# prtk1729/Paligemma-MultiModal-System

Hardware: AMD Instinct MI355X
Metric: image→text tokens/sec + prefill ms, PaliGemma-3B-224 at 1/2/4/8 MI355X (higher is better)
Workload: dtype bf16; 1 GPU; PaliGemma-3B-pt-224 image->text, batch 1, prefill L=264, 128 greedy tokens (BASELINE.json configs[1]); global_batch=1, seq_len=392, parallelism=dp1, decode=hipgraph, prefill=eager

## Files before the change

include/pghip.h:

```cpp
#ifndef PGHIP_H
#define PGHIP_H
#include <stdint.h>
#include <hip/hip_runtime_api.h>

#ifdef __cplusplus
extern "C" {
#endif

int pg_abi_version(void);
int pg_source_hash(char* out, int n);

enum {
  PG_EPI_BF16 = 0,
  PG_EPI_BF16_GELU = 1,
  PG_EPI_BF16_GELU_MUL = 2,
  PG_EPI_F32 = 3,
  PG_EPI_F32_POS = 4,
  PG_EPI_BF16_VT = 5,
  PG_EPI_QKV_ROPE = 6,
  PG_EPI_F32_FIN = 7,
  PG_EPI_F32_ADD = 8,
  PG_EPI_FX_ADD = 9,
  PG_EPI_F32_RES = 10
};

typedef struct PgFusedArgs {
  int pro_mode;
  const float* resid_in;
  float* resid_out;
  const float* partials;
  int nsplit;
  const float* norm_w;
  float eps;
  const float* part_o;
  const float* part_ml;
  int asplit, head_dim, dtw, q_per_kv, kv_heads;
  const float* cos_t;
  const float* sin_t;
  const int* pos;
  int rows_per_batch;
  const int* slot_dev;
  int slot_base;
  void* kc;
  void* vtc;
  int smax;
  int q_heads;
  int* fin_cnt;
  float* fin_resid;
  float* ss_out;
  const float* ss_in;
  int ss_ld, ss_n;
  void* fin_x;
  int akeys;
  const float* a_scale;
  const float* w_scale;
  int slab_rows;
  void* kd;
  void* vd;
  unsigned* amax_out;
  const unsigned* amax_in;
  int amax_ld;
  unsigned* amax_zero;
  int amax_zero_n;
  int64_t* fx;
  uint8_t* mx_out;
  const uint8_t* mx_in;
  int* status;
} PgFusedArgs;

#define PG_W_FRAG 0x100
#define PG_FP8 0x200
#define PG_TILE_M1 0x400
#define PG_TILE_N64 0x800

int pg_gemm(const void* A, int lda, const void* W, int ldw, const float* bias, void* C, int ldc,
            int M, int N, int K, int epi, int ksplit, const float* aux, int aux_rows, void* aux_out,
            int aux_ld, int aux_n, hipStream_t stream);

int pg_gemm_finalize(const float* part, int nsplit, void* C, int ldc, int M, int N, int epi, void* aux_out,
                     int aux_ld, int aux_n, const PgFusedArgs* fused, hipStream_t stream);

int pg_gemm_fused(const void* A, int lda, const void* W, int ldw, const float* bias, void* C, int ldc,
                  int M, int N, int K, int epi, int ksplit, const PgFusedArgs* fused, hipStream_t stream);

int pg_norm_residual(float* resid, const float* partials, int nsplit, int M_part, const float* w,
                     const float* b, void* out, int ldo, float* out_f32, const int* row_map, int M_out,
                     int H, int mode, float eps, int write_resid, hipStream_t stream);

int pg_attention(const void* q, long q_rs, void* o, long o_rs, const void* k, long k_bs, long k_hs,
                 long k_rs, const void* vt, long vt_bs, long vt_hs, long vt_ds, const float* mask,
                 long mask_bs, long mask_rs, int B, int Lq, int Lkv, const int* lkv_dev, int Hq, int Hkv,
                 int D, float scale, int split_keys, int nsplit, float* part_o, float* part_ml,
                 int kcap, const void* kd, const void* vd, hipStream_t stream);
int pg_attn_combine(const float* part_o, const float* part_ml, int B, int Hq, int Hkv, int D, int nsplit,
                    void* o, long o_rs, hipStream_t stream);

int pg_attn_probs(const void* q, long q_rs, const void* k, long k_bs, long k_hs, long k_rs, const float* mask,
                  long mask_bs, long mask_rs, int B, int Lq, int Lkv, int Hq, int Hkv, int D, float scale,
                  int probs, float* out, hipStream_t stream);

#define PG_ATTN_PIPE 0x100
int pg_attn_decode(const void* q, long q_rs, void* o, long o_rs, const void* kd, const void* vd, int B, int Lkv,
                   const int* lkv_dev, int Hq, int Hkv, int D, float scale, int kcap, int nsplit, int nw, int nb,
                   float* part_o, float* part_ml, int* counters, void* q8, float* q8_scale, long q8_ld,
                   hipStream_t stream);

int pg_rope_kv_write(void* qkv, int ldq, const int* pos, int T, int L, int Hq, int Hkv, int D,
                     const float* cosT, const float* sinT, void* kc, void* vtc, int Smax, int slot_base,
                     const int* slot_dev, hipStream_t stream);

int pg_patch_im2col(const float* px, int B, int C, int H, int W, int p, void* out, int ldk, hipStream_t stream);

int pg_image_rank(const int64_t* ids, int n, long image_id, int* rank, hipStream_t stream);

int pg_embed_merge(const int64_t* ids, const int* rank, int n, const void* embed, int V, const float* feat,
                   int n_feat, int H, long image_id, long pad_id, float img_scale, float normalizer,
                   float* out, hipStream_t stream);

int pg_argmax(const float* logits, long ld, int B, int V, void* workspace, int64_t* out_ids,
              int64_t* hist, int hist_rows, int* step, int* pos, int* kv_len, hipStream_t stream);
int pg_argmax_embed(const float* logits, long ld, int B, int V, void* workspace, int64_t* out_ids,
                    int64_t* hist, int hist_rows, int* step, int* pos, int* kv_len, const void* embed, int V_embed,
                    const float* feat, int n_feat, int H, long image_id, long pad_id, float img_scale,
                    float normalizer, float* res, hipStream_t stream);

int pg_argmax_pairs(const float* logits, long ld, int B, int V, int vocab_offset, void* workspace,
                    float* pairs, hipStream_t stream);
int pg_argmax_merge(const float* pairs, int world, int B, int64_t* out_ids, int64_t* hist, int hist_rows,
                    int* step, int* pos, int* kv_len, hipStream_t stream);

int pg_topp_sample(const float* logits, long ld, int B, int V, float temperature, float top_p,
                   const float* uniforms, int64_t* out_ids, int64_t* hist, int hist_rows, int* step, int* pos,
                   int* kv_len, float* probs_out, hipStream_t stream);

int pg_image_preprocess(const uint8_t* src, int H, int W, int S, const int* hb, const int* hk, int hks,
                        const int* vb, const int* vk, int vks, int y0, int rows, const float* lut, uint8_t* tmp,
                        float* out, hipStream_t stream);
int pg_image_preprocess_modes(const uint8_t* src, int H, int W, int C, int alpha, int S, const int* hb,
                              const int* hk, int hks, const int* vb, const int* vk, int vks, int y0, int rows,
                              const float* lut, uint8_t* tmp, float* out, hipStream_t stream);
int pg_image_palette(const uint8_t* src, int H, int W, int S, const int* xtab, const int* ytab,
                     const float* pal_lut, float* out, hipStream_t stream);

int pg_synth_fill(void* out, long n, unsigned int seedmix, float a, float mean, int out_kind,
                  hipStream_t stream);

int pg_quant_fp8(const void* x, int ldx, int M, int K, void* q, int ldq, float* scale, hipStream_t stream);
int pg_norm_residual_fp8(float* resid, const float* partials, int nsplit, int M_part, const float* w,
                         const float* b, void* q, int ldq, float* scale, const int* row_map, int M_out,
                         int H, int mode, float eps, int write_resid, hipStream_t stream);
int pg_norm_residual_mx(float* resid, const float* partials, int nsplit, int M_part, const float* w, void* q,
                        int ldq, void* qs, float* ss, int ss_ld, int M, int H, int write_resid, hipStream_t stream);

int pg_xgmi_buffer_bytes(int world, long cap, long* bytes);
int pg_xgmi_alloc(long bytes, void** out);
int pg_xgmi_free(void* p);
int pg_xgmi_ipc_handle(void* p, void* handle64);
int pg_xgmi_ipc_open(const void* handle64, void** out);
int pg_xgmi_ipc_close(void* p);
int pg_allreduce_xgmi(float* data, long n, int rank, int world, void* const* peers, long cap,
                      unsigned* epochs, int* err, hipStream_t stream);
int pg_allreduce_xgmi_slabs(float* data, long n, int nslab, long slab_stride, int rank, int world,
                            void* const* peers, long cap, unsigned* epochs, int* err, hipStream_t stream);
int pg_allgather_xgmi(const float* in, long n, float* out, int rank, int world, void* const* peers, long cap,
                      unsigned* epochs, int* err, hipStream_t stream);
int pg_xgmi_rs_buffer_bytes(int world, long rs_cap, long* bytes);
int pg_allreduce_xgmi_rs(float* data, long n, int nslab, long slab_stride, int rank, int world, void* const* peers,
                         long rs_cap, int nwg, unsigned* epochs, int* err, hipStream_t stream);

#ifdef __cplusplus
}
#endif
#endif
```

paligemma-multimodal-system_amd/csrc/common.h:

```cpp
#pragma once
#include <hip/hip_runtime.h>
#include <stdint.h>

typedef uint16_t bf16_t;
typedef __attribute__((ext_vector_type(8))) __bf16 bf16x8;
typedef __attribute__((ext_vector_type(4))) float f32x4;
typedef __attribute__((ext_vector_type(2))) float f32x2;
typedef __attribute__((ext_vector_type(4))) uint32_t u32x4;
typedef __attribute__((ext_vector_type(2))) uint32_t u32x2;

#define LDS_AS __attribute__((address_space(3)))

__device__ __forceinline__ float bf2f(bf16_t v) { return __uint_as_float(((uint32_t)v) << 16); }

__device__ __forceinline__ bf16_t f2bf(float f) {
  __bf16 b = (__bf16)f;
  return __builtin_bit_cast(bf16_t, b);
}
typedef __bf16 pg_bf16x2_t __attribute__((ext_vector_type(2)));
typedef float pg_f32x2_t __attribute__((ext_vector_type(2)));
__device__ __forceinline__ uint32_t pack_bf2(float lo, float hi) {
  return __builtin_bit_cast(uint32_t, __builtin_convertvector(pg_f32x2_t{lo, hi}, pg_bf16x2_t));
}

__device__ __forceinline__ float bf_lo(uint32_t v) { return __uint_as_float(v << 16); }
__device__ __forceinline__ float bf_hi(uint32_t v) { return __uint_as_float(v & 0xffff0000u); }
__device__ __forceinline__ uint32_t pack_fp8x4(float a, float b, float c, float d) {
  int w = __builtin_amdgcn_cvt_pk_fp8_f32(fminf(fmaxf(a, -448.f), 448.f), fminf(fmaxf(b, -448.f), 448.f), 0, false);
  w = __builtin_amdgcn_cvt_pk_fp8_f32(fminf(fmaxf(c, -448.f), 448.f), fminf(fmaxf(d, -448.f), 448.f), w, true);
  return (uint32_t)w;
}

__device__ __forceinline__ float max_xor16(float v) {
  const auto r = __builtin_amdgcn_permlane16_swap(__float_as_uint(v), __float_as_uint(v), false, false);
  return fmaxf(__uint_as_float(r[0]), __uint_as_float(r[1]));
}
__device__ __forceinline__ float max_xor32(float v) {
  const auto r = __builtin_amdgcn_permlane32_swap(__float_as_uint(v), __float_as_uint(v), false, false);
  return fmaxf(__uint_as_float(r[0]), __uint_as_float(r[1]));
}
__device__ __forceinline__ float sum_xor16(float v) {
  const auto r = __builtin_amdgcn_permlane16_swap(__float_as_uint(v), __float_as_uint(v), false, false);
  return __uint_as_float(r[0]) + __uint_as_float(r[1]);
}
__device__ __forceinline__ float sum_xor32(float v) {
  const auto r = __builtin_amdgcn_permlane32_swap(__float_as_uint(v), __float_as_uint(v), false, false);
  return __uint_as_float(r[0]) + __uint_as_float(r[1]);
}

__device__ __forceinline__ float xchg_xor32(float v) {
  const auto r = __builtin_amdgcn_permlane32_swap(__float_as_uint(v), __float_as_uint(v), false, false);
  return __uint_as_float((threadIdx.x & 32) ? r[0] : r[1]);
}

__device__ __forceinline__ float gelu_tanh(float x) {
  const float u = 0.7978845608028654f * (x + 0.044715f * x * x * x);
  return x * __builtin_amdgcn_rcpf(1.0f + __builtin_amdgcn_exp2f(-2.8853900817779268f * u));
}

__device__ __forceinline__ f32x4 mfma16(const bf16x8& a, const bf16x8& b, const f32x4& c) {
  return __builtin_amdgcn_mfma_f32_16x16x32_bf16(a, b, c, 0, 0, 0);
}

typedef __attribute__((ext_vector_type(8))) int i32x8;
typedef __attribute__((ext_vector_type(4))) int i32x4;

__device__ __forceinline__ f32x4 mfma8(const bf16x8& a0, const bf16x8& a1, const bf16x8& b0, const bf16x8& b1,
                                       const f32x4& c) {
  const i32x4 x0 = __builtin_bit_cast(i32x4, a0), x1 = __builtin_bit_cast(i32x4, a1);
  const i32x4 y0 = __builtin_bit_cast(i32x4, b0), y1 = __builtin_bit_cast(i32x4, b1);
  const i32x8 a = __builtin_shufflevector(x0, x1, 0, 1, 2, 3, 4, 5, 6, 7);
  const i32x8 b = __builtin_shufflevector(y0, y1, 0, 1, 2, 3, 4, 5, 6, 7);
  return __builtin_amdgcn_mfma_scale_f32_16x16x128_f8f6f4(a, b, c, 0, 0, 0, 127, 0, 127);
}
__device__ __forceinline__ f32x4 mfma8s(const bf16x8& a0, const bf16x8& a1, const bf16x8& b0, const bf16x8& b1,
                                        const f32x4& c, int sb) {
  const i32x4 x0 = __builtin_bit_cast(i32x4, a0), x1 = __builtin_bit_cast(i32x4, a1);
  const i32x4 y0 = __builtin_bit_cast(i32x4, b0), y1 = __builtin_bit_cast(i32x4, b1);
  const i32x8 a = __builtin_shufflevector(x0, x1, 0, 1, 2, 3, 4, 5, 6, 7);
  const i32x8 b = __builtin_shufflevector(y0, y1, 0, 1, 2, 3, 4, 5, 6, 7);
  return __builtin_amdgcn_mfma_scale_f32_16x16x128_f8f6f4(a, b, c, 0, 0, 0, 127, 0, sb);
}
template <int N>
__device__ __forceinline__ void mfma_fence(f32x4 (&a)[N]) {
#ifdef PG_NO_MFMA_FENCE
  return;
#endif
  __builtin_amdgcn_sched_barrier(0);
  asm volatile("s_nop 7\n\ts_nop 7");
  __builtin_amdgcn_sched_barrier(0);
#pragma unroll
  for (int i = 0; i < N; ++i) asm volatile("" : "+v"(a[i]));
  __builtin_amdgcn_sched_barrier(0);
}
__device__ __forceinline__ int mx_exp(float amax) {
  if (!(amax > 0.f)) return 0;
  int k;
  const float f = frexpf(amax, &k);
  const int e = k - 9 + (f * 512.f > 448.f ? 1 : 0);
  return min(max(e, -127), 127);
}
__device__ __forceinline__ f32x4 mfma8(const i32x8& a, const i32x8& b, const f32x4& c) {
  return __builtin_amdgcn_mfma_scale_f32_16x16x128_f8f6f4(a, b, c, 0, 0, 0, 127, 0, 127);
}
template <int SEL>
__device__ __forceinline__ f32x4 mfma8s_sel(const bf16x8& a0, const bf16x8& a1, const bf16x8& b0, const bf16x8& b1,
                                            const f32x4& c, int sb) {
  const i32x4 x0 = __builtin_bit_cast(i32x4, a0), x1 = __builtin_bit_cast(i32x4, a1);
  const i32x4 y0 = __builtin_bit_cast(i32x4, b0), y1 = __builtin_bit_cast(i32x4, b1);
  const i32x8 a = __builtin_shufflevector(x0, x1, 0, 1, 2, 3, 4, 5, 6, 7);
  const i32x8 b = __builtin_shufflevector(y0, y1, 0, 1, 2, 3, 4, 5, 6, 7);
  return __builtin_amdgcn_mfma_scale_f32_16x16x128_f8f6f4(a, b, c, 0, 0, 0, 127, SEL, sb);
}
__device__ __forceinline__ i32x8 cat8(const bf16x8& lo, const bf16x8& hi) {
  return __builtin_shufflevector(__builtin_bit_cast(i32x4, lo), __builtin_bit_cast(i32x4, hi), 0, 1, 2, 3, 4, 5, 6, 7);
}

__device__ __forceinline__ float wave_sum(float v) {
#pragma unroll
  for (int o = 32; o > 0; o >>= 1) v += __shfl_xor(v, o, 64);
  return v;
}
__device__ __forceinline__ float wave_max(float v) {
#pragma unroll
  for (int o = 32; o > 0; o >>= 1) v = fmaxf(v, __shfl_xor(v, o, 64));
  return v;
}

__device__ __forceinline__ float block_sum(float v, float* red ) {
  const int lane = threadIdx.x & 63, w = threadIdx.x >> 6, nw = blockDim.x >> 6;
  v = wave_sum(v);
  __syncthreads();
  if (lane == 0) red[w] = v;
  __syncthreads();
  float s = 0.f;
  for (int i = 0; i < nw; ++i) s += red[i];
  return s;
}

static __device__ int pg_zero_word = 0;

#define PG_VMC(k) case k: asm volatile("s_waitcnt vmcnt(" #k ")" ::: "memory"); break;
__device__ __forceinline__ void wait_vm_n(int n) {
  switch (n) {
    PG_VMC(1) PG_VMC(2) PG_VMC(3) PG_VMC(4) PG_VMC(5) PG_VMC(6) PG_VMC(7) PG_VMC(8) PG_VMC(9) PG_VMC(10)
    PG_VMC(11) PG_VMC(12) PG_VMC(13) PG_VMC(14) PG_VMC(15) PG_VMC(16) PG_VMC(17) PG_VMC(18) PG_VMC(19) PG_VMC(20)
    PG_VMC(21) PG_VMC(22) PG_VMC(23) PG_VMC(24) PG_VMC(25) PG_VMC(26) PG_VMC(27) PG_VMC(28) PG_VMC(29) PG_VMC(30)
    PG_VMC(31) PG_VMC(32) PG_VMC(33) PG_VMC(34) PG_VMC(35) PG_VMC(36) PG_VMC(37) PG_VMC(38) PG_VMC(39) PG_VMC(40)
    default: asm volatile("s_waitcnt vmcnt(0)" ::: "memory"); break;
  }
}
#undef PG_VMC

#define PG_LAUNCH_CHECK() do { hipError_t _e = hipGetLastError(); if (_e != hipSuccess) return (int)_e; } while (0)
#define PG_REQUIRE(cond) do { if (!(cond)) return (int)hipErrorInvalidValue; } while (0)
```

paligemma-multimodal-system_amd/csrc/gemm.hip:

```cpp
#include "gemm_common.h"

static int gemm_impl(const void* A, int lda, const void* W, int ldw, const float* bias, void* C, int ldc,
                     int M, int N, int K, int epi_flags, int ksplit, const float* aux, int aux_rows, void* aux_out,
                     int aux_ld, int aux_n, const PgFusedArgs* fa, hipStream_t stream) {
  const bool frag = (epi_flags & PG_W_FRAG) != 0;
  const bool fp8 = (epi_flags & PG_FP8) != 0;
  const bool m1 = (epi_flags & PG_TILE_M1) != 0;
  const bool n64 = (epi_flags & PG_TILE_N64) != 0;
  const int epi = epi_flags & 0xFF;
  PG_REQUIRE((epi_flags & ~(0xFF | PG_W_FRAG | PG_FP8 | PG_TILE_M1 | PG_TILE_N64)) == 0 && epi <= PG_EPI_F32_RES);
  if (m1) PG_REQUIRE(!fp8 && !n64 && M >= 256 && M <= 288 && (fa == nullptr || fa->pro_mode == 0));
  if (n64) PG_REQUIRE(M > 16);
  PG_REQUIRE(M > 0 && N > 0 && K > 0 && ksplit >= 1 && W != nullptr && C != nullptr);
  PG_REQUIRE(K % 32 == 0 && ldw >= K && (N % 4) == 0);
  if (frag && !fp8) PG_REQUIRE(N % 16 == 0 && K % 64 == 0 && ldw == K &&
                       (epi == PG_EPI_BF16 || epi == PG_EPI_BF16_GELU_MUL || epi == PG_EPI_F32 ||
                        epi == PG_EPI_QKV_ROPE || epi == PG_EPI_F32_FIN || epi == PG_EPI_F32_ADD ||
                        epi == PG_EPI_FX_ADD || epi == PG_EPI_F32_RES));
  PgFusedArgs f{};
  if (fa) f = *fa;
  EpiArgs e{bias, C, ldc, M, N, aux, aux_rows, (bf16_t*)aux_out, aux_ld, aux_n, f};
  PG_REQUIRE(f.pro_mode >= 0 && f.pro_mode <= 5);
  if (f.pro_mode == 5)
    PG_REQUIRE(fp8 && frag && epi == PG_EPI_F32 && M <= 32 && f.amax_in && f.amax_ld >= 1 && A != nullptr &&
               lda >= K && lda % 8 == 0 && ((uintptr_t)A & 15) == 0 && K % 128 == 0 && (K / 128) % ksplit == 0 &&
               (K / 128 / ksplit == 8 || K / 128 / ksplit == 16));
  if (f.amax_out) PG_REQUIRE(fp8 && frag && epi == PG_EPI_BF16_GELU_MUL && M <= 32 && f.amax_ld >= 1 &&
                             ((K >> 7) + ksplit - 1) / ksplit * 128 <= 4096 && PG_GEMV8_WIDE);
  if (f.amax_zero) PG_REQUIRE(frag && f.amax_zero_n >= 0 &&
                              (fp8 ? f.amax_zero_n <= 4096
                                   : (M <= 16 && f.amax_zero_n <= 16384 && f.amax_zero_n % 4 == 0 &&
                                      ((uintptr_t)f.amax_zero & 15) == 0)));
  if (f.pro_mode == 0 || f.pro_mode == 4) PG_REQUIRE(A != nullptr && lda >= K);
  if (f.pro_mode == 4) PG_REQUIRE(ksplit == 1 && f.ss_in && f.ss_n > 0 && f.ss_ld >= f.ss_n &&
                                  ((M <= 2 && f.ss_n <= 256 && (M == 1 || f.ss_n <= 128)) ||
                                   (M > 4 && M <= 16 && f.ss_n <= 64)));
  if (f.pro_mode != 0 && f.pro_mode != 5) PG_REQUIRE(M <= 16);
  if (f.pro_mode == 1) PG_REQUIRE(ksplit == 1 && (f.resid_in || f.fx) && f.norm_w && (f.nsplit == 0 || f.partials) &&
                                  K % 4 == 0);
  if (f.pro_mode == 2)
    PG_REQUIRE(f.part_o && f.part_ml && f.head_dim > 0 && (K / ksplit) % f.head_dim == 0 && f.asplit > 0 &&
               f.q_per_kv > 0 && f.kv_heads > 0);
  if (epi == PG_EPI_QKV_ROPE) PG_REQUIRE(f.head_dim % 16 == 0 && f.cos_t && f.sin_t && f.pos && f.kc && f.vtc &&
                                         f.rows_per_batch > 0 && f.smax > 0 && ksplit == 1 &&
                                         N == (f.q_heads + 2 * f.kv_heads) * f.head_dim);
  if (f.pro_mode == 3) PG_REQUIRE(ksplit == 1 && f.resid_in && f.norm_w && f.ss_in && f.ss_n > 0 &&
                                  f.ss_ld >= f.ss_n && K % 4 == 0);
  if (epi == PG_EPI_F32_FIN) PG_REQUIRE(M <= 16 && ksplit <= 8 && (f.fin_x == nullptr || f.norm_w != nullptr) && f.fin_cnt && f.fin_resid && f.ss_out && f.ss_ld >= (N + 15) / 16 &&
                                        ldc == N);
  if (epi == PG_EPI_F32_ADD) PG_REQUIRE((M <= 16 || (fp8 && frag && M <= 32)) && (f.pro_mode == 0 || f.pro_mode == 2) &&
                                        ldc >= N);
  if (epi == PG_EPI_F32_RES) PG_REQUIRE(M > 16 && ksplit == 1 && f.pro_mode == 0 && ldc >= N && ldc % 4 == 0 &&
                                        ((uintptr_t)C & 15) == 0 && !f.mx_out);
  if (epi == PG_EPI_FX_ADD) PG_REQUIRE(M <= 16 && !fp8 && (f.pro_mode == 0 || f.pro_mode == 2) && ldc >= N &&
                                       ((uintptr_t)C & 15) == 0 && ldc % 2 == 0);
  if (f.mx_in && frag) PG_REQUIRE(fp8 && epi != PG_EPI_F32_ADD && M <= 32 && f.pro_mode == 0 && K % 128 == 0 &&
                                   A != nullptr && ((uintptr_t)f.mx_in & 15) == 0 &&
                                   (!f.ss_in || (f.ss_n > 0 && f.ss_n <= 4 && f.ss_ld >= f.ss_n && K == 1024 * f.ss_n)));
  if (f.mx_in && !frag) PG_REQUIRE(fp8 && (epi == PG_EPI_F32 || epi == PG_EPI_F32_RES) && M > 32 && f.pro_mode == 0 && K % 128 == 0 &&
                                   A != nullptr && ((uintptr_t)f.mx_in & 3) == 0 && !f.ss_in &&
                                   (size_t)M * (size_t)(K / 32) < (1ull << 32) &&
                                   (size_t)M * (size_t)lda < (1ull << 32) && (size_t)N * (size_t)ldw < (1ull << 32));
  if (f.mx_out && frag) PG_REQUIRE(fp8 && epi == PG_EPI_BF16_GELU_MUL && M <= 32 && f.pro_mode == 0 && !f.amax_out &&
                                    ksplit == 1 && (N / 2) % 128 == 0 && PG_GEMV8_WIDE && (K >> 7) * 128 <= 4096 &&
                                    (!f.mx_in || (K >> 7) == 8 || (K >> 7) == 16));
  if (f.mx_out && !frag) PG_REQUIRE(fp8 && epi == PG_EPI_BF16_GELU_MUL && M > 32 && f.pro_mode == 0 && !f.mx_in &&
                                    ksplit == 1 && N % 128 == 0 && ldc >= N / 2);
  if (f.fx) PG_REQUIRE(((uintptr_t)f.fx & 15) == 0 && (f.pro_mode == 1) != (epi == PG_EPI_F32_FIN) && !fp8 &&
                       M <= 16);
  if (ksplit > 1) PG_REQUIRE(epi == PG_EPI_F32 || epi == PG_EPI_F32_FIN || epi == PG_EPI_F32_ADD || epi == PG_EPI_FX_ADD);
  if (epi == PG_EPI_BF16_GELU_MUL) PG_REQUIRE(N % 32 == 0);
  if (epi == PG_EPI_F32_POS) PG_REQUIRE(aux != nullptr && aux_rows > 0 && bias != nullptr);
  if (epi == PG_EPI_BF16_VT) PG_REQUIRE(aux_out != nullptr && aux_n % 4 == 0);
  if (M <= 16) PG_REQUIRE(K % 64 == 0);
  else PG_REQUIRE(K % TBK == 0 && (f.pro_mode == 0 || f.pro_mode == 5) && epi != PG_EPI_F32_FIN);
  const bf16_t* a = (const bf16_t*)A;
  const bf16_t* w = (const bf16_t*)W;
  if (fp8 && frag) {
    PG_REQUIRE(M <= 32 && (f.pro_mode == 0 || f.pro_mode == 5) && (f.a_scale || f.pro_mode == 5 || f.mx_in) && f.w_scale &&
               K % 128 == 0 && N % 16 == 0 && ldw == K && lda >= K && (lda % 16 == 0 || f.pro_mode == 5) &&
               ((uintptr_t)A & 15) == 0 && ((uintptr_t)W & 15) == 0 && epi != PG_EPI_F32_FIN);
    const int rc = pg_dispatch_gemv8(epi, (const uint8_t*)A, lda, (const uint8_t*)W, K, ksplit, e, stream);
    if (rc) return rc;
    PG_LAUNCH_CHECK();
    return 0;
  }
  if (fp8) {
    PG_REQUIRE(!frag && M > 16 && f.pro_mode == 0 && (f.a_scale || f.mx_in) && f.w_scale && K % 128 == 0 && lda % 16 == 0 &&
               ldw % 16 == 0 && ((uintptr_t)A & 15) == 0 && ((uintptr_t)W & 15) == 0);
    const int rc = pg_dispatch_tile(epi, false, true, a, lda / 2, w, ldw / 2, K / 2, ksplit, e, stream, false, n64);
    if (rc) return rc;
    PG_LAUNCH_CHECK();
    return 0;
  }
  const int rc = M <= 16 ? pg_dispatch_gemv(epi, frag, a, lda, w, ldw, K, ksplit, e, stream)
                         : pg_dispatch_tile(epi, frag, false, a, lda, w, ldw, K, ksplit, e, stream, m1, n64);
  if (rc) return rc;
  PG_LAUNCH_CHECK();
  return 0;
}

extern "C" int pg_gemm(const void* A, int lda, const void* W, int ldw, const float* bias, void* C, int ldc,
                       int M, int N, int K, int epi, int ksplit, const float* aux, int aux_rows, void* aux_out,
                       int aux_ld, int aux_n, hipStream_t stream) {
  return gemm_impl(A, lda, W, ldw, bias, C, ldc, M, N, K, epi, ksplit, aux, aux_rows, aux_out, aux_ld, aux_n,
                   nullptr, stream);
}

extern "C" int pg_gemm_fused(const void* A, int lda, const void* W, int ldw, const float* bias, void* C, int ldc,
                             int M, int N, int K, int epi, int ksplit, const PgFusedArgs* fused, hipStream_t stream) {
  return gemm_impl(A, lda, W, ldw, bias, C, ldc, M, N, K, epi, ksplit, nullptr, 0, nullptr, 0, 0, fused, stream);
}
```

paligemma-multimodal-system_amd/csrc/gemm_common.h:

```cpp
#pragma once
#include <cstdlib>
#include <type_traits>

#include "attn_common.h"

#ifndef PG_G256_STAGGER
#define PG_G256_STAGGER 1
#endif
#ifndef PG_G256_F8_BUF
#define PG_G256_F8_BUF 1
#endif
#ifndef PG_G256_PREFETCH
#define PG_G256_PREFETCH 1
#endif

enum {
  PG_EPI_BF16 = 0,
  PG_EPI_BF16_GELU = 1,
  PG_EPI_BF16_GELU_MUL = 2,
  PG_EPI_F32 = 3,
  PG_EPI_F32_POS = 4,
  PG_EPI_BF16_VT = 5,
  PG_EPI_QKV_ROPE = 6,
  PG_EPI_F32_FIN = 7,
  PG_EPI_F32_ADD = 8,
  PG_EPI_FX_ADD = 9,
  PG_EPI_F32_RES = 10,
};

#define PG_FX_SCALE 0x1p32f
#define PG_FX_INV 0x1p-32f
__device__ __forceinline__ long long fx_from_f32(float v) {
  const float t = truncf(v);
  const int hi = (int)t;
  const float r = rintf((v - t) * PG_FX_SCALE);
  const float rh = truncf(r * 0x1p-16f);
  const float rl = fmaf(rh, -65536.f, r);
  return (long long)((unsigned long long)(long long)hi << 32) + ((long long)(int)rh << 16) + (long long)(int)rl;
}
__device__ __forceinline__ long long fx_from_f32_checked(float v, int* status) {
  if (__builtin_expect(!(fabsf(v) < 0x1p31f), 0)) {
    if (status) atomicOr(status, 1);
    return v > 0.f ? (1LL << 62) : (v < 0.f ? -(1LL << 62) : 0LL);
  }
  return fx_from_f32(v);
}
__device__ __forceinline__ float fx_to_f32(long long q) {
  return fmaf((float)(unsigned)(unsigned long long)q, PG_FX_INV, (float)(int)(q >> 32));
}
typedef long long i64x2 __attribute__((ext_vector_type(2)));
__device__ __forceinline__ f32x4 fx_load4(const long long* p) {
  const i64x2 a = *(const i64x2*)p, b = *(const i64x2*)(p + 2);
  return f32x4{fx_to_f32(a[0]), fx_to_f32(a[1]), fx_to_f32(b[0]), fx_to_f32(b[1])};
}

struct PgFusedArgs {
  int pro_mode;
  const float* resid_in;
  float* resid_out;
  const float* partials;
  int nsplit;
  const float* norm_w;
  float eps;
  const float* part_o;
  const float* part_ml;
  int asplit, head_dim, dtw, q_per_kv, kv_heads;
  const float* cos_t;
  const float* sin_t;
  const int* pos;
  int rows_per_batch;
  const int* slot_dev;
  int slot_base;
  bf16_t* kc;
  bf16_t* vtc;
  int smax;
  int q_heads;
  int* fin_cnt;
  float* fin_resid;
  float* ss_out;
  const float* ss_in;
  int ss_ld, ss_n;
  bf16_t* fin_x;
  int akeys;
  const float* a_scale;
  const float* w_scale;
  int slab_rows;
  bf16_t* kd;
  bf16_t* vd;
  unsigned* amax_out;
  const unsigned* amax_in;
  int amax_ld;
  unsigned* amax_zero;
  int amax_zero_n;
  long long* fx;
  uint8_t* mx_out;
  const uint8_t* mx_in;
  int* status;
};

__device__ __forceinline__ f32x4 load4_guard(const float* __restrict__ p, int n0, int N) {
  if (n0 + 3 < N) return *(const f32x4*)(p + n0);
  f32x4 v = {0.f, 0.f, 0.f, 0.f};
#pragma unroll
  for (int j = 0; j < 4; ++j) if (n0 + j < N) v[j] = p[n0 + j];
  return v;
}

#define PG_W_FRAG 0x100
#define PG_TILE_M1 0x400
#define PG_TILE_N64 0x800
#define PG_FP8 0x200

#ifndef PG_GEMV8_WIDE
#define PG_GEMV8_WIDE 1
#endif

#define TBN 128
#define TBK 64

struct EpiArgs {
  const float* bias;
  void* C;
  int ldc;
  int M, N;
  const float* aux;
  int aux_rows;
  bf16_t* aux_out;
  int aux_ld;
  int aux_n;
  PgFusedArgs f;
};

__device__ __forceinline__ void scale_acc(const EpiArgs& e, int m, int n0, f32x4& v) {
  if (m >= e.M || n0 >= e.N) return;
  v *= (e.f.mx_in ? 1.0f : e.f.a_scale[m]) * load4_guard(e.f.w_scale, n0, e.N);
}

struct Fp8RowLoads {
  float v[4];
};
__device__ __forceinline__ Fp8RowLoads fp8_row_load(const EpiArgs& e, int m) {
  Fp8RowLoads r;
  m = min(m, e.M - 1);
  if (!e.f.mx_in) {
    r.v[0] = e.f.a_scale[m];
  } else if (e.f.ss_in) {
    const float* p = e.f.ss_in + (size_t)m * e.f.ss_ld;
#pragma unroll
    for (int i = 0; i < 4; ++i) r.v[i] = p[min(i, e.f.ss_n - 1)];
  }
  return r;
}
__device__ __forceinline__ float fp8_row_finish(const EpiArgs& e, const Fp8RowLoads& r) {
  if (!e.f.mx_in) return r.v[0];
  if (!e.f.ss_in) return 1.0f;
  float s = 0.f;
#pragma unroll
  for (int i = 0; i < 4; ++i) s += i < e.f.ss_n ? r.v[i] : 0.f;
  return rsqrtf(s / (1024.0f * (float)e.f.ss_n) + e.f.eps);
}
__device__ __forceinline__ float fp8_row_factor(const EpiArgs& e, int m) { return fp8_row_finish(e, fp8_row_load(e, m)); }
__device__ __forceinline__ void scale_acc_rf(const EpiArgs& e, int m, int n0, f32x4& v, float rf) {
  if (m >= e.M || n0 >= e.N) return;
  v *= rf * load4_guard(e.f.w_scale, n0, e.N);
}

__device__ __forceinline__ int rope_freq_index(const PgFusedArgs& f, int n0, bool* roped) {
  const int D = f.head_dim, within = n0 % D, jj0 = within & 15;
  *roped = n0 / D < f.q_heads + f.kv_heads;
  return 8 * (within >> 4) + (jj0 & 7);
}
__device__ __forceinline__ void epi_qkv_rope4_core(const EpiArgs& e, int m, int n0, f32x4 v, f32x4 pr, f32x4 cs,
                                                   f32x4 sn, int slot0) {
  if (m >= e.M || n0 >= e.N) return;
  const PgFusedArgs& f = e.f;
  const int D = f.head_dim, half = D >> 1;
  const int blk = n0 / D, within = n0 % D;
  const int t = within >> 4, jj0 = within & 15;
  const bool second = jj0 >= 8;
  const int ii = 8 * t + (jj0 & 7);
  const int d0 = second ? half + ii : ii;
  const int b = m / f.rows_per_batch, i = m % f.rows_per_batch;
  const int slot = slot0 + i;
  const bool in_cache = slot < f.smax;
  const int Hq = f.q_heads, Hkv = f.kv_heads;
  const int KV = Hkv * D;
  if (blk < Hq + Hkv) {
    f32x4 y;
#pragma unroll
    for (int j = 0; j < 4; ++j) {
      y[j] = second ? v[j] * cs[j] + pr[j] * sn[j] : v[j] * cs[j] - pr[j] * sn[j];
    }
    u32x2 pk;
    pk[0] = pack_bf2(y[0], y[1]);
    pk[1] = pack_bf2(y[2], y[3]);
    if (blk < Hq) {
      *(u32x2*)((bf16_t*)e.C + (size_t)m * e.ldc + blk * D + d0) = pk;
    } else if (in_cache) {
      *(u32x2*)(f.kc + ((size_t)b * f.smax + slot) * KV + (blk - Hq) * D + d0) = pk;
      if (f.kd)
        *(u32x2*)(f.kd + ((size_t)b * Hkv + (blk - Hq)) * f.smax * D + dec_koff(slot, d0, D)) = pk;
    }
  } else {
    const int c0 = (blk - Hq - Hkv) * D + d0;
    if (in_cache) {
#pragma unroll
      for (int j = 0; j < 4; ++j) f.vtc[((size_t)b * KV + c0 + j) * f.smax + slot] = f2bf(v[j]);
      if (f.vd) {
        bf16_t* vd = f.vd + ((size_t)b * Hkv + (blk - Hq - Hkv)) * f.smax * D;
#pragma unroll
        for (int j = 0; j < 4; ++j) vd[dec_voff(slot, d0 + j, D)] = f2bf(v[j]);
      }
    }
  }
}

__device__ __forceinline__ void epi_qkv_rope4_pr(const EpiArgs& e, int m, int n0, f32x4 v, f32x4 pr) {
  if (m >= e.M || n0 >= e.N) return;
  const PgFusedArgs& f = e.f;
  bool roped;
  const int ii = rope_freq_index(f, n0, &roped);
  f32x4 cs = {1.f, 1.f, 1.f, 1.f}, sn = {0.f, 0.f, 0.f, 0.f};
  if (roped) {
    const int p = f.pos[m];
    const float* cp = f.cos_t + (long)p * (f.head_dim >> 1) + ii;
    const float* sp = f.sin_t + (long)p * (f.head_dim >> 1) + ii;
#pragma unroll
    for (int j = 0; j < 4; ++j) {
      cs[j] = cp[j];
      sn[j] = sp[j];
    }
  }
  epi_qkv_rope4_core(e, m, n0, v, pr, cs, sn, f.slot_base + (f.slot_dev ? *f.slot_dev : 0));
}

__device__ __forceinline__ void epi_qkv_rope4(const EpiArgs& e, int m, int n0, f32x4 v) {
  if (e.bias && n0 < e.N) v += load4_guard(e.bias, n0, e.N);
  f32x4 pr;
#pragma unroll
  for (int j = 0; j < 4; ++j) pr[j] = xchg_xor32(v[j]);
  epi_qkv_rope4_pr(e, m, n0, v, pr);
}

__device__ __forceinline__ f32x4 res_load4(const EpiArgs& e, int m, int n0) {
  f32x4 r = {0.f, 0.f, 0.f, 0.f};
  if (m >= e.M || n0 >= e.N) return r;
  const float* C = (const float*)e.C + (size_t)m * e.ldc;
  if (n0 + 3 < e.N) return *(const f32x4*)(C + n0);
#pragma unroll
  for (int j = 0; j < 4; ++j) if (n0 + j < e.N) r[j] = C[n0 + j];
  return r;
}
__device__ __forceinline__ void res_store4(const EpiArgs& e, int m, int n0, f32x4 v, f32x4 r) {
  if (m >= e.M || n0 >= e.N) return;
  if (e.bias) v += load4_guard(e.bias, n0, e.N);
  float* C = (float*)e.C + (size_t)m * e.ldc;
  const f32x4 o = r + v;
  if (n0 + 3 < e.N) {
    *(f32x4*)(C + n0) = o;
  } else {
#pragma unroll
    for (int j = 0; j < 4; ++j) if (n0 + j < e.N) C[n0 + j] = o[j];
  }
}

template <int EPI>
__device__ __forceinline__ void epi_store4(const EpiArgs& e, int m, int n0, f32x4 v, int z) {
  if (m >= e.M || n0 >= e.N) return;
  if (e.bias && (EPI != PG_EPI_F32 || z == 0)) v += load4_guard(e.bias, n0, e.N);
  if constexpr (EPI == PG_EPI_F32) {
    const size_t srows = e.f.slab_rows > 0 ? (size_t)e.f.slab_rows : (size_t)e.M;
    float* C = (float*)e.C + ((size_t)z * srows + m) * e.ldc;
    if (n0 + 3 < e.N) {
      *(f32x4*)(C + n0) = v;
    } else {
#pragma unroll
      for (int j = 0; j < 4; ++j) if (n0 + j < e.N) C[n0 + j] = v[j];
    }
  } else if constexpr (EPI == PG_EPI_F32_RES) {
    float* C = (float*)e.C + (size_t)m * e.ldc;
    if (n0 + 3 < e.N) {
      *(f32x4*)(C + n0) = *(const f32x4*)(C + n0) + v;
    } else {
#pragma unroll
      for (int j = 0; j < 4; ++j) if (n0 + j < e.N) C[n0 + j] = C[n0 + j] + v[j];
    }
  } else if constexpr (EPI == PG_EPI_F32_POS) {
    float* C = (float*)e.C + (size_t)m * e.ldc;
    v += load4_guard(e.aux + (size_t)(m % e.aux_rows) * e.ldc, n0, e.N);
    if (n0 + 3 < e.N) {
      *(f32x4*)(C + n0) = v;
    } else {
#pragma unroll
      for (int j = 0; j < 4; ++j) if (n0 + j < e.N) C[n0 + j] = v[j];
    }
  } else {
    if constexpr (EPI == PG_EPI_BF16_GELU) {
#pragma unroll
      for (int j = 0; j < 4; ++j) v[j] = gelu_tanh(v[j]);
    }
    if constexpr (EPI == PG_EPI_BF16_VT) {
      if (n0 >= e.aux_n) {
#pragma unroll
        for (int j = 0; j < 4; ++j)
          if (n0 + j < e.N) e.aux_out[(size_t)(n0 + j - e.aux_n) * e.aux_ld + m] = f2bf(v[j]);
        return;
      }
    }
    bf16_t* C = (bf16_t*)e.C + (size_t)m * e.ldc;
    if (n0 + 3 < e.N) {
      u32x2 p;
      p[0] = pack_bf2(v[0], v[1]);
      p[1] = pack_bf2(v[2], v[3]);
      *(u32x2*)(C + n0) = p;
    } else {
#pragma unroll
      for (int j = 0; j < 4; ++j) if (n0 + j < e.N) C[n0 + j] = f2bf(v[j]);
    }
  }
}

__device__ __forceinline__ void epi_add4(const EpiArgs& e, int m, int n0, f32x4 v, int z) {
  if (m >= e.M || n0 >= e.N) return;
  if (e.bias && z == 0) v += load4_guard(e.bias, n0, e.N);
  float* dst = (float*)e.C + (size_t)m * e.ldc + n0;
#pragma unroll
  for (int j = 0; j < 4; ++j)
    if (n0 + j < e.N) unsafeAtomicAdd(dst + j, v[j]);
}

__device__ __forceinline__ void epi_gelu_mul4(const EpiArgs& e, int m, int gb, int q, f32x4 g, f32x4 u) {
  if (m >= e.M) return;
  const int oc = (gb >> 1) + q;
  if (oc + 3 >= (e.N >> 1)) return;
  u32x2 p;
  p[0] = pack_bf2(gelu_tanh(g[0]) * u[0], gelu_tanh(g[1]) * u[1]);
  p[1] = pack_bf2(gelu_tanh(g[2]) * u[2], gelu_tanh(g[3]) * u[3]);
  *(u32x2*)((bf16_t*)e.C + (size_t)m * e.ldc + oc) = p;
}

__device__ __forceinline__ float epi_gelu_mul4_amax(const EpiArgs& e, int m, int gb, int q, f32x4 g, f32x4 u) {
  if (m >= e.M) return 0.f;
  const int oc = (gb >> 1) + q;
  if (oc + 3 >= (e.N >> 1)) return 0.f;
  u32x2 p;
  p[0] = pack_bf2(gelu_tanh(g[0]) * u[0], gelu_tanh(g[1]) * u[1]);
  p[1] = pack_bf2(gelu_tanh(g[2]) * u[2], gelu_tanh(g[3]) * u[3]);
  *(u32x2*)((bf16_t*)e.C + (size_t)m * e.ldc + oc) = p;
  return fmaxf(fmaxf(fabsf(bf_lo(p[0])), fabsf(bf_hi(p[0]))), fmaxf(fabsf(bf_lo(p[1])), fabsf(bf_hi(p[1]))));
}

__device__ __forceinline__ void amax_clear(const EpiArgs& e) {
  if (e.f.amax_zero && blockIdx.x == 0 && blockIdx.y == 0)
    for (int i = threadIdx.x; i < e.f.amax_zero_n; i += blockDim.x) e.f.amax_zero[i] = 0u;
}

int pg_dispatch_tile(int epi, bool frag, bool f8, const bf16_t* A, int lda, const bf16_t* W, int ldw, int K, int ksplit,
                     const EpiArgs& e, hipStream_t st, bool m1, bool n64);
int pg_dispatch_gemv(int epi, bool frag, const bf16_t* A, int lda, const bf16_t* W, int ldw, int K, int ksplit,
                     const EpiArgs& e, hipStream_t st);
int pg_dispatch_gemv8(int epi, const uint8_t* X, int ldx, const uint8_t* W, int K, int ksplit, const EpiArgs& e,
                      hipStream_t st);
```

paligemma-multimodal-system_amd/csrc/gemm_gemv.hip:

```cpp
#include "gemm_common.h"

#define XPAD 8

#ifndef PG_GEMV_PREW
#define PG_GEMV_PREW 1
#endif
#ifndef PG_GEMV_NT
#define PG_GEMV_NT 0
#endif
#ifndef PG_GEMV_CONTIG
#define PG_GEMV_CONTIG 0
#endif
#ifndef PG_GEMV_QKV_NT1
#define PG_GEMV_QKV_NT1 1
#endif
#ifndef PG_GEMV_D2
#define PG_GEMV_D2 4
#endif
#ifndef PG_GEMV_LM_NT
#define PG_GEMV_LM_NT 2
#endif
#ifndef PG_GEMV_LM_D
#define PG_GEMV_LM_D 6
#endif
// ... 336 lines not shown
    } else {
      const int off = (c0 + wave + j * 4) * CH + LANE_OFF;
#pragma unroll
      for (int t = 0; t < NT; ++t)
#pragma unroll
        for (int s = 0; s < U; ++s) {
#if PG_GEMV_NT
          wv[t][s] = __builtin_nontemporal_load((const u32x4*)(wrow[t] + off + S_STRIDE * s));
#else
          wv[t][s] = *(const u32x4*)(wrow[t] + off + S_STRIDE * s);
#endif
        }
    }
  };
  auto loadx = [&](int j, u32x4 (&xv)[U]) {
    const int koff = (wave + j * 4) * CH + LANE_OFF;
    if constexpr ((PRO == 0 || PRO == 4) && !PG_GEMV_XLDS) {
#pragma unroll
      for (int s = 0; s < U; ++s)
        xv[s] = *(const u32x4*)(xrow + c0 * CH + koff + S_STRIDE * s);
    } else {
#pragma unroll
      for (int s = 0; s < U; ++s) xv[s] = *(const u32x4*)(xlds + koff + S_STRIDE * s);
    }
  };
  constexpr bool STAGED = (PRO != 0 && PRO != 4) || PG_GEMV_XLDS;
  const bool early = PRO == 1 && (PG_GEMV_PRO_EARLY == 1 || (PG_GEMV_PRO_EARLY == 2 && EPI == PG_EPI_QKV_ROPE)) &&
                     M == 1 && (K >> 2) <= 512 && e.f.nsplit == 0 &&
                     e.f.resid_out == nullptr;
  Pro1Row p1;
  if constexpr (PRO == 1 && PG_GEMV_PRO_EARLY) {
    if (early) pro1_row_load(e.f, K, p1);
    __builtin_amdgcn_sched_barrier(0);
  }
  constexpr bool prew = STAGED && PG_GEMV_PREW;
  if (prew) {
#pragma unroll
    for (int d = 0; d < DEPTH; ++d)
      if (CPW > 0 ? d < CPW : d < mine) loadw(d, wb[d]);
  }
  if constexpr (STAGED) {
    float* scratch = (float*)(dyn_smem + (((size_t)M * (Kr + XPAD) * 2 + 15) & ~(size_t)15));
    if (PRO == 1 && PG_GEMV_PRO_EARLY && early)
      pro1_row_finish(e.f, K, p1, xs, scratch);
    else
      gemv_prologue<PRO>(e, M, K, c0 * CH, nch * CH, xs, scratch, A, lda, gi);
  }
#pragma unroll
  for (int d = 0; d < DEPTH; ++d)
    if (CPW > 0 ? d < CPW : d < mine) {
      if (!prew) loadw(d, wb[d]);
      loadx(d, xb[d]);
    }
  f32x4 fin_r[NT], fin_w[NT];
  i64x2 fin_fa[NT], fin_fb[NT];
  if constexpr (EPI == PG_EPI_F32_FIN) {
#pragma unroll
    for (int t = 0; t < NT; ++t) {
      const int n0 = min((tile0 + t) * 16, e.N - 16) + 4 * g;
      const size_t ro = (size_t)(r < M ? r : M - 1) * e.N + n0;
      fin_r[t] = *(const f32x4*)(e.f.fin_resid + ro);
      const long long* p = e.f.fx ? e.f.fx + ro : (const long long*)e.f.fin_resid;
      fin_fa[t] = *(const i64x2*)p;
      fin_fb[t] = *(const i64x2*)(p + 2);
      fin_w[t] = *(const f32x4*)((e.f.norm_w ? e.f.norm_w : e.f.fin_resid) + n0);
    }
  }
  f32x4 rope_cs[NT], rope_sn[NT];
  if constexpr (EPI == PG_EPI_QKV_ROPE) {
#pragma unroll
    for (int t = 0; t < NT; ++t) {
      bool roped;
      const int ii = rope_freq_index(e.f, min((tile0 + t) * 16, e.N - 16) + 4 * g, &roped);
      const long off = (long)rope_p * (e.f.head_dim >> 1) + ii;
      rope_cs[t] = *(const f32x4*)(e.f.cos_t + off);
      rope_sn[t] = *(const f32x4*)(e.f.sin_t + off);
    }
  }
  if constexpr (CPW > 0) {
    __builtin_amdgcn_sched_barrier(0);
#pragma unroll
    for (int j = 0; j < CPW; ++j) {
      const int d = j % DEPTH;
#pragma unroll
      for (int s = 0; s < U; ++s) {
        const bf16x8 xv = __builtin_bit_cast(bf16x8, xb[d][s]);
#pragma unroll
        for (int t = 0; t < NT; ++t) acc[t] = mfma16(__builtin_bit_cast(bf16x8, wb[d][t][s]), xv, acc[t]);
      }
      if (j + DEPTH < CPW) {
        loadw(j + DEPTH, wb[d]);
        loadx(j + DEPTH, xb[d]);
      }
      __builtin_amdgcn_sched_barrier(0);
    }
  } else {
    for (int base = 0; base < mine; base += DEPTH) {
#pragma unroll
      for (int d = 0; d < DEPTH; ++d) {
        const int j = base + d;
        if (j < mine) {
#pragma unroll
          for (int s = 0; s < U; ++s) {
            const bf16x8 xv = __builtin_bit_cast(bf16x8, xb[d][s]);
#pragma unroll
            for (int t = 0; t < NT; ++t) acc[t] = mfma16(__builtin_bit_cast(bf16x8, wb[d][t][s]), xv, acc[t]);
          }
          if (j + DEPTH < mine) {
            loadw(j + DEPTH, wb[d]);
            loadx(j + DEPTH, xb[d]);
          }
        }
      }
    }
  }

  __shared__ f32x4 red[4][NT][64];
#pragma unroll
  for (int t = 0; t < NT; ++t) red[wave][t][lane] = acc[t];
  __syncthreads();
  if (e.f.amax_zero && gi.bx == 0 && gi.by == 0)
    for (int i = 4 * (int)threadIdx.x; i < e.f.amax_zero_n; i += 1024) *(u32x4*)(e.f.amax_zero + i) = u32x4{0u, 0u, 0u, 0u};
  if (wave != 0) return;
#pragma unroll
  for (int t = 0; t < NT; ++t) acc[t] = red[0][t][lane] + red[1][t][lane] + red[2][t][lane] + red[3][t][lane];
  const int m = r;
  const int q = 4 * g;
  if constexpr (PRO == 3) {
    const float* scratch = (const float*)(dyn_smem + (((size_t)M * (Kr + XPAD) * 2 + 15) & ~(size_t)15));
    const float rs = scratch[64 + (m < M ? m : 0)];
#pragma unroll
    for (int t = 0; t < NT; ++t) acc[t] *= rs;
  }
  if constexpr (PRO == 4) {
    float ss = 0.f;
    if (SS16 && M > 2) {
#pragma unroll
      for (int k = 0; k < SSL; ++k) ss += g + 4 * k < e.f.ss_n ? ssv[k] : 0.f;
    } else {
      const int lpr = M == 1 ? 64 : 32;
#pragma unroll
      for (int k = 0; k < 4; ++k) ss += lane % lpr + k * lpr < e.f.ss_n ? ssv[k] : 0.f;
    }
    if (SS16 && M > 2) {
      ss = sum_xor16(ss);
      ss = sum_xor32(ss);
    } else {
      const int lpr = M == 1 ? 64 : 32;
      for (int o = 1; o < lpr; o <<= 1) ss += __shfl_xor(ss, o, 64);
      ss = __shfl(ss, (m < M ? m : 0) * lpr, 64);
    }
    const float rs = rsqrtf(ss / (float)K + e.f.eps);
#pragma unroll
    for (int t = 0; t < NT; ++t) acc[t] *= rs;
  }
  if constexpr (EPI == PG_EPI_F32_FIN) {
    const PgFusedArgs& f = e.f;
    typedef __attribute__((address_space(1))) unsigned long long gu64;
    constexpr int SE = NT >= 2 ? NT / 2 : 1;
    auto finish = [&](int t, int n0, f32x4 v, float& ssl) {
      *(f32x4*)(f.fin_resid + (size_t)m * e.N + n0) = v;
      ssl += v[0] * v[0] + v[1] * v[1] + v[2] * v[2] + v[3] * v[3];
      if (f.fin_x) {
        const f32x4 w = fin_w[t];
        u32x2 pk;
        pk[0] = pack_bf2(v[0] * (1.0f + w[0]), v[1] * (1.0f + w[1]));
        pk[1] = pack_bf2(v[2] * (1.0f + w[2]), v[3] * (1.0f + w[3]));
        *(u32x2*)(f.fin_x + (size_t)m * e.N + n0) = pk;
      }
    };
    auto fin_base = [&](int t) {
      return f.fx ? f32x4{fx_to_f32(fin_fa[t][0]), fx_to_f32(fin_fa[t][1]), fx_to_f32(fin_fb[t][0]),
                          fx_to_f32(fin_fb[t][1])}
                  : fin_r[t];
    };
    auto fx_clear = [&](int n0) {
      if (f.fx) {
        long long* p = f.fx + (size_t)m * e.N + n0;
        *(i64x2*)p = i64x2{0, 0};
        *(i64x2*)(p + 2) = i64x2{0, 0};
      }
    };
    auto put_ss = [&](float (&ssl)[SE]) {
#pragma unroll
      for (int p = 0; p < SE; ++p) {
        const float v = sum_xor32(sum_xor16(ssl[p]));
        if (g == 0 && m < M) f.ss_out[(size_t)m * f.ss_ld + gi.bx * SE + p] = v;
      }
    };
    if (gi.ny == 1) {
      float ssl[SE];
#pragma unroll
      for (int p = 0; p < SE; ++p) ssl[p] = 0.f;
#pragma unroll
      for (int t = 0; t < NT; ++t) {
        const int n0 = (tile0 + t) * 16 + q;
        if (m < M && n0 < e.N) {
          f32x4 v = acc[t];
          if (e.bias) v += load4_guard(e.bias, n0, e.N);
          finish(t, n0, fin_base(t) + v, ssl[t / 2 < SE ? t / 2 : 0]);
          fx_clear(n0);
        }
      }
      put_ss(ssl);
      return;
    }
#pragma unroll
    for (int t = 0; t < NT; ++t) {
      const int n0 = (tile0 + t) * 16 + q;
      if (m < M && n0 < e.N) {
        f32x4 v = acc[t];
        if (e.bias && z == 0) v += load4_guard(e.bias, n0, e.N);
        gu64* dst = (gu64*)((float*)e.C + ((size_t)z * M + m) * e.ldc + n0);
        __hip_atomic_store(dst, __builtin_bit_cast(unsigned long long, u32x2{__float_as_uint(v[0]),
                           __float_as_uint(v[1])}), __ATOMIC_RELAXED, __HIP_MEMORY_SCOPE_AGENT);
        __hip_atomic_store(dst + 1, __builtin_bit_cast(unsigned long long, u32x2{__float_as_uint(v[2]),
                           __float_as_uint(v[3])}), __ATOMIC_RELAXED, __HIP_MEMORY_SCOPE_AGENT);
      }
    }
    asm volatile("s_waitcnt vmcnt(0)" ::: "memory");
    int old = 0;
    if (lane == 0) old = __hip_atomic_fetch_add(f.fin_cnt + gi.bx, 1, __ATOMIC_RELAXED, __HIP_MEMORY_SCOPE_AGENT);
    old = __shfl(old, 0, 64);
    if (old != gi.ny - 1) return;
    __builtin_amdgcn_fence(__ATOMIC_ACQUIRE, "wavefront");
    float ssl[SE];
#pragma unroll
    for (int p = 0; p < SE; ++p) ssl[p] = 0.f;
#pragma unroll
    for (int t = 0; t < NT; ++t) {
      const int n0 = (tile0 + t) * 16 + q;
      if (m < M && n0 < e.N) {
        f32x4 v = fin_base(t);
        const int Z = gi.ny;
        u32x2 sa[8], sb[8];
#pragma unroll
        for (int zz = 0; zz < 8; ++zz) {
          gu64* src = (gu64*)((float*)e.C + ((size_t)(zz < Z ? zz : Z - 1) * M + m) * e.ldc + n0);
          sa[zz] = __builtin_bit_cast(u32x2, __hip_atomic_load(src, __ATOMIC_RELAXED, __HIP_MEMORY_SCOPE_AGENT));
          sb[zz] = __builtin_bit_cast(u32x2, __hip_atomic_load(src + 1, __ATOMIC_RELAXED, __HIP_MEMORY_SCOPE_AGENT));
        }
#pragma unroll
        for (int zz = 0; zz < 8; ++zz) {
          const f32x4 sv = {__uint_as_float(sa[zz][0]), __uint_as_float(sa[zz][1]), __uint_as_float(sb[zz][0]),
                            __uint_as_float(sb[zz][1])};
          v += zz < Z ? sv : f32x4{0.f, 0.f, 0.f, 0.f};
        }
        finish(t, n0, v, ssl[t / 2 < SE ? t / 2 : 0]);
        fx_clear(n0);
      }
    }
    put_ss(ssl);
    if (lane == 0) __hip_atomic_store(f.fin_cnt + gi.bx, 0, __ATOMIC_RELAXED, __HIP_MEMORY_SCOPE_AGENT);
    return;
  }
  if constexpr (EPI == PG_EPI_F32_ADD) {
    if (m < M) {
#pragma unroll
      for (int t = 0; t < NT; ++t) {
        const int n0 = (tile0 + t) * 16 + q;
        if (n0 < e.N) {
          f32x4 v = acc[t];
          if (e.bias && z == 0) v += load4_guard(e.bias, n0, e.N);
          float* dst = (float*)e.C + (size_t)m * e.ldc + n0;
#pragma unroll
          for (int j = 0; j < 4; ++j) unsafeAtomicAdd(dst + j, v[j]);
        }
      }
    }
    return;
  }
  if constexpr (EPI == PG_EPI_FX_ADD) {
    if (m < M) {
#pragma unroll
      for (int t = 0; t < NT; ++t) {
        const int n0 = (tile0 + t) * 16 + q;
        if (n0 < e.N) {
          f32x4 v = acc[t];
          if (e.bias && z == 0) v += load4_guard(e.bias, n0, e.N);
          if (e.f.resid_in && z == 0) v += load4_guard(e.f.resid_in + (size_t)m * e.N, n0, e.N);
          unsigned long long* dst = (unsigned long long*)e.C + (size_t)m * e.ldc + n0;
#pragma unroll
          for (int j = 0; j < 4; ++j) atomicAdd(dst + j, (unsigned long long)fx_from_f32_checked(v[j], e.f.status));
        }
      }
    }
    return;
  }
  if constexpr (EPI == PG_EPI_BF16_GELU_MUL) {
#pragma unroll
    for (int t = 0; t < NT; t += 2) epi_gelu_mul4(e, m, (tile0 + t) * 16, q, acc[t], acc[t + 1]);
  } else if constexpr (EPI == PG_EPI_QKV_ROPE) {
#pragma unroll
    for (int t = 0; t < NT; ++t) {
      f32x4 v = acc[t];
      const int n0 = (tile0 + t) * 16 + q;
      if (e.bias && n0 < e.N) v += load4_guard(e.bias, n0, e.N);
      f32x4 pr;
#pragma unroll
      for (int j = 0; j < 4; ++j) pr[j] = xchg_xor32(v[j]);
      epi_qkv_rope4_core(e, m, n0, v, pr, rope_cs[t], rope_sn[t], e.f.slot_base + rope_slot_raw);
    }
  } else {
#pragma unroll
    for (int t = 0; t < NT; ++t) epi_store4<EPI>(e, m, (tile0 + t) * 16 + q, acc[t], z);
  }
}

template <int EPI, int NT, int U, int DEPTH, int PRO, bool FRAG, int CPW = 0>
__global__ __launch_bounds__(256) void gemv_kernel(const bf16_t* __restrict__ A, int lda,
                                                   const bf16_t* __restrict__ W, int ldw, int K, EpiArgs e) {
  gemv_body<EPI, NT, U, DEPTH, PRO, FRAG, CPW>(A, lda, W, ldw, K, e,
                                               GemvIdx{(int)blockIdx.x, (int)blockIdx.y, (int)gridDim.x, (int)gridDim.y});
}

template <int EPI, int NT, int DEPTH, int PRO, bool FRAG>
static void launch_gemv_cpw(dim3 grid, size_t lds, hipStream_t st, const bf16_t* A, int lda, const bf16_t* W, int ldw,
                            int K, int ksplit, const EpiArgs& e) {
  const int nch = K / 64;
  const int cpw = (nch % ksplit == 0 && (nch / ksplit) % 4 == 0) ? nch / ksplit / 4 : 0;
  switch (PG_GEMV_CPW ? cpw : 0) {
    case 4: hipLaunchKernelGGL((gemv_kernel<EPI, NT, 2, DEPTH, PRO, FRAG, 4>), grid, dim3(256), lds, st, A, lda, W, ldw, K, e); break;
    case 8: hipLaunchKernelGGL((gemv_kernel<EPI, NT, 2, DEPTH, PRO, FRAG, 8>), grid, dim3(256), lds, st, A, lda, W, ldw, K, e); break;
    case 16: hipLaunchKernelGGL((gemv_kernel<EPI, NT, 2, DEPTH, PRO, FRAG, 16>), grid, dim3(256), lds, st, A, lda, W, ldw, K, e); break;
    default: hipLaunchKernelGGL((gemv_kernel<EPI, NT, 2, DEPTH, PRO, FRAG, 0>), grid, dim3(256), lds, st, A, lda, W, ldw, K, e); break;
  }
}

template <int EPI, int PRO, bool FRAG>
static void launch_gemv_pro(const bf16_t* A, int lda, const bf16_t* W, int ldw, int K, int ksplit, const EpiArgs& e,
                            hipStream_t st) {
  const int ntiles = (e.N + 15) / 16;
  const int CH = 64;
  const int per_z = (K / CH + ksplit - 1) / ksplit;
  size_t lds = 0;
  if ((PRO != 0 && PRO != 4) || PG_GEMV_XLDS) {
    lds = (size_t)e.M * (per_z * CH + XPAD) * 2;
    lds = (lds + 15) & ~(size_t)15;
    if (PRO == 1) lds += 64 * sizeof(float);
    if (PRO == 3) lds += 80 * sizeof(float);
  }
  if constexpr (PG_GEMV_QKV_NT1 && EPI == PG_EPI_QKV_ROPE) {
    if (e.M > 4) {
      launch_gemv_cpw<EPI, 1, PG_GEMV_D2, PRO, FRAG>(dim3(ntiles, ksplit), lds, st, A, lda, W, ldw, K, ksplit, e);
      return;
    }
  }
  if constexpr (PG_GEMV_LM_NT == 2 && EPI == PG_EPI_F32) {
    if (e.M <= 4 && ntiles >= 8192 && ksplit == 1) {
      launch_gemv_cpw<EPI, 2, PG_GEMV_LM_D, PRO, FRAG>(dim3((ntiles + 1) / 2, 1), lds, st, A, lda, W, ldw, K, 1, e);
      return;
    }
  }
  if constexpr (PG_GEMV_FIN_NT == 4 && EPI == PG_EPI_F32_FIN) {
    if (e.M > 4 && ntiles % 4 == 0) {
      launch_gemv_cpw<EPI, 4, PG_GEMV_D2, PRO, FRAG>(dim3(ntiles / 4, ksplit), lds, st, A, lda, W, ldw, K, ksplit, e);
      return;
    }
  }
  if (EPI == PG_EPI_BF16_GELU_MUL || e.M > 4) {
    launch_gemv_cpw<EPI, 2, PG_GEMV_D2, PRO, FRAG>(dim3((ntiles + 1) / 2, ksplit), lds, st, A, lda, W, ldw, K, ksplit, e);
  } else {
    launch_gemv_cpw<EPI, 1, PG_GEMV_D1, PRO, FRAG>(dim3(ntiles, ksplit), lds, st, A, lda, W, ldw, K, ksplit, e);
  }
}

template <int EPI, bool FRAG>
static void launch_gemv(const bf16_t* A, int lda, const bf16_t* W, int ldw, int K, int ksplit, const EpiArgs& e,
                        hipStream_t st) {
  if constexpr (EPI == PG_EPI_F32_ADD || EPI == PG_EPI_FX_ADD) {
    if (e.f.pro_mode == 2)
      launch_gemv_pro<EPI, 2, FRAG>(A, lda, W, ldw, K, ksplit, e, st);
    else
      launch_gemv_pro<EPI, 0, FRAG>(A, lda, W, ldw, K, ksplit, e, st);
    return;
  }
  switch (e.f.pro_mode) {
    case 1: launch_gemv_pro<EPI, 1, FRAG>(A, lda, W, ldw, K, ksplit, e, st); break;
    case 2: launch_gemv_pro<EPI, 2, FRAG>(A, lda, W, ldw, K, ksplit, e, st); break;
    case 3: launch_gemv_pro<EPI, 3, FRAG>(A, lda, W, ldw, K, ksplit, e, st); break;
    case 4: launch_gemv_pro<EPI, 4, FRAG>(A, lda, W, ldw, K, ksplit, e, st); break;
    default: launch_gemv_pro<EPI, 0, FRAG>(A, lda, W, ldw, K, ksplit, e, st); break;
  }
}

int pg_dispatch_gemv(int epi, bool frag, const bf16_t* A, int lda, const bf16_t* W, int ldw, int K, int ksplit,
                     const EpiArgs& e, hipStream_t st) {
#define PG_CASE(E)                                                                             \
  case E:                                                                                      \
    if (frag) launch_gemv<E, true>(A, lda, W, ldw, K, ksplit, e, st);                          \
    else launch_gemv<E, false>(A, lda, W, ldw, K, ksplit, e, st);                              \
    return 0;
#define PG_CASE_ROWMAJOR(E)                                                                    \
  case E: launch_gemv<E, false>(A, lda, W, ldw, K, ksplit, e, st); return 0;
  switch (epi) {
    PG_CASE(PG_EPI_BF16)
    PG_CASE(PG_EPI_BF16_GELU_MUL)
    PG_CASE(PG_EPI_F32)
    PG_CASE(PG_EPI_QKV_ROPE)
    PG_CASE(PG_EPI_F32_FIN)
    PG_CASE(PG_EPI_F32_ADD)
    PG_CASE(PG_EPI_FX_ADD)
    PG_CASE_ROWMAJOR(PG_EPI_BF16_GELU)
    PG_CASE_ROWMAJOR(PG_EPI_F32_POS)
    PG_CASE_ROWMAJOR(PG_EPI_BF16_VT)
    default: return (int)hipErrorInvalidValue;
  }
#undef PG_CASE
#undef PG_CASE_ROWMAJOR
}
```

paligemma-multimodal-system_amd/csrc/misc.hip:

```cpp
#include <cstdlib>

#include "common.h"

__global__ void im2col_kernel(const float* __restrict__ px, int B, int C, int H, int W, int p, int nh, int nw,
                              bf16_t* __restrict__ out, int ldk) {
  const long total = (long)B * nh * nw * ldk;
  for (long i = blockIdx.x * (long)blockDim.x + threadIdx.x; i < total; i += (long)gridDim.x * blockDim.x) {
    const int col = (int)(i % ldk);
    const long row = i / ldk;
    const int pw = (int)(row % nw);
    const int ph = (int)((row / nw) % nh);
    const int b = (int)(row / ((long)nw * nh));
    float v = 0.f;
    if (col < C * p * p) {
      const int c = col / (p * p), kh = (col / p) % p, kw = col % p;
      v = px[(((long)b * C + c) * H + ph * p + kh) * W + pw * p + kw];
    }
    out[i] = f2bf(v);
  }
}

extern "C" int pg_patch_im2col(const float* px, int B, int C, int H, int W, int p, void* out, int ldk,
                               hipStream_t stream) {
  PG_REQUIRE(px && out && B > 0 && C > 0 && p > 0 && ldk >= C * p * p && H >= p && W >= p);
  const int nh = H / p, nw = W / p;
  const long total = (long)B * nh * nw * ldk;
  const int grid = (int)min((total + 255) / 256, (long)8192);
  hipLaunchKernelGGL(im2col_kernel, dim3(grid), dim3(256), 0, stream, px, B, C, H, W, p, nh, nw, (bf16_t*)out, ldk);
  PG_LAUNCH_CHECK();
  return 0;
}

__global__ __launch_bounds__(1024) void image_rank_kernel(const int64_t* __restrict__ ids, int n, int64_t image_id,
                                                          int* __restrict__ rank) {
  __shared__ int part[1024];
  const int t = threadIdx.x;
  const int per = (n + 1023) / 1024;
  const int s = min(n, t * per), e = min(n, s + per);
  int cnt = 0;
  for (int i = s; i < e; ++i) cnt += ids[i] == image_id;
  part[t] = cnt;
  __syncthreads();
  for (int off = 1; off < 1024; off <<= 1) {
    int v = t >= off ? part[t - off] : 0;
    __syncthreads();
    part[t] += v;
    __syncthreads();
  }
  int run = part[t] - cnt;
  for (int i = s; i < e; ++i) {
    rank[i] = run;
    run += ids[i] == image_id;
  }
}

extern "C" int pg_image_rank(const int64_t* ids, int n, long image_id, int* rank, hipStream_t stream) {
  PG_REQUIRE(ids && rank && n > 0);
  hipLaunchKernelGGL(image_rank_kernel, dim3(1), dim3(1024), 0, stream, ids, n, (int64_t)image_id, rank);
  PG_LAUNCH_CHECK();
  return 0;
}

__device__ __forceinline__ void embed_row(float* __restrict__ o, int64_t id, int rk, int t, int nt,
                                          const bf16_t* __restrict__ embed, int V, const float* __restrict__ feat,
                                          int n_feat, int H, int64_t image_id, int64_t pad_id, float img_scale,
                                          float normalizer) {
  if (id == pad_id) {
    for (int c = t * 4; c < H; c += 4 * nt) *(f32x4*)(o + c) = f32x4{0.f, 0.f, 0.f, 0.f};
    return;
  }
  if (id == image_id) {
    const bool ok = rk < n_feat;
    const float* f = feat + (long)(ok ? rk : 0) * H;
    for (int c = t * 4; c < H; c += 4 * nt) {
      f32x4 v = ok ? *(const f32x4*)(f + c) : f32x4{0.f, 0.f, 0.f, 0.f};
#pragma unroll
      for (int j = 0; j < 4; ++j) v[j] = (v[j] * img_scale) * normalizer;
      *(f32x4*)(o + c) = v;
    }
    return;
  }
  const int64_t tid = id < 0 ? 0 : (id >= V ? V - 1 : id);
  const bf16_t* e = embed + tid * (long)H;
  for (int c = t * 4; c < H; c += 4 * nt) {
    const u32x2 w = *(const u32x2*)(e + c);
    f32x4 v;
    v[0] = bf2f((bf16_t)(w[0] & 0xFFFF)) * normalizer;
    v[1] = bf2f((bf16_t)(w[0] >> 16)) * normalizer;
    v[2] = bf2f((bf16_t)(w[1] & 0xFFFF)) * normalizer;
    v[3] = bf2f((bf16_t)(w[1] >> 16)) * normalizer;
    *(f32x4*)(o + c) = v;
  }
}

__global__ __launch_bounds__(256) void embed_merge_kernel(const int64_t* __restrict__ ids, const int* __restrict__ rank,
                                                          int n, const bf16_t* __restrict__ embed, int V,
                                                          const float* __restrict__ feat, int n_feat, int H,
                                                          int64_t image_id, int64_t pad_id, float img_scale,
                                                          float normalizer, float* __restrict__ out) {
  const int row = blockIdx.x;
  const int64_t id = ids[row];
  int rk = 0;
  if (id == image_id) {
    if (rank) {
      rk = rank[row];
    } else {
      for (int i = 0; i < row; ++i) rk += ids[i] == image_id;
    }
  }
  embed_row(out + (long)row * H, id, rk, threadIdx.x, blockDim.x, embed, V, feat, n_feat, H, image_id, pad_id,
            img_scale, normalizer);
}

extern "C" int pg_embed_merge(const int64_t* ids, const int* rank, int n, const void* embed, int V, const float* feat,
                              int n_feat, int H, long image_id, long pad_id, float img_scale, float normalizer,
                              float* out, hipStream_t stream) {
  PG_REQUIRE(ids && embed && out && n > 0 && V > 0 && H > 0 && H % 4 == 0 && (n_feat == 0 || feat));
  hipLaunchKernelGGL(embed_merge_kernel, dim3(n), dim3(256), 0, stream, ids, rank, n, (const bf16_t*)embed, V, feat,
                     n_feat, H, (int64_t)image_id, (int64_t)pad_id, img_scale, normalizer, out);
  PG_LAUNCH_CHECK();
  return 0;
}

__global__ __launch_bounds__(256) void rope_kv_kernel(bf16_t* __restrict__ qkv, int ldq, const int* __restrict__ pos,
                                                      int L, int Hq, int Hkv, int D, const float* __restrict__ cosT,
                                                      const float* __restrict__ sinT, bf16_t* __restrict__ kc,
                                                      bf16_t* __restrict__ vtc, int Smax, int slot_base,
                                                      const int* __restrict__ slot_dev) {
  const int t = blockIdx.x;
  const int b = t / L, i = t % L;
  const int slot = slot_base + (slot_dev ? *slot_dev : 0) + i;
  const int p = pos[t];
  const int half = D / 2;
  const float* cs = cosT + (long)p * half;
  const float* sn = sinT + (long)p * half;
  bf16_t* row = qkv + (long)t * ldq;
  const int KV = Hkv * D;
  for (int idx = threadIdx.x; idx < (Hq + Hkv) * half; idx += blockDim.x) {
    const int h = idx / half, j = idx % half;
    bf16_t* x = row + h * D;
    const float x1 = bf2f(x[j]), x2 = bf2f(x[j + half]);
    const float c = cs[j], s = sn[j];
    const float y1 = x1 * c - x2 * s;
    const float y2 = x2 * c + x1 * s;
    if (h < Hq) {
      x[j] = f2bf(y1);
      x[j + half] = f2bf(y2);
    } else {
      const int hk = h - Hq;
      bf16_t* kr = kc + ((long)b * Smax + slot) * KV + hk * D;
      kr[j] = f2bf(y1);
      kr[j + half] = f2bf(y2);
    }
  }
  const bf16_t* v = row + (Hq + Hkv) * D;
  for (int cidx = threadIdx.x; cidx < KV; cidx += blockDim.x)
    vtc[((long)b * KV + cidx) * Smax + slot] = v[cidx];
}

extern "C" int pg_rope_kv_write(void* qkv, int ldq, const int* pos, int T, int L, int Hq, int Hkv, int D,
                                const float* cosT, const float* sinT, void* kc, void* vtc, int Smax, int slot_base,
                                const int* slot_dev, hipStream_t stream) {
  PG_REQUIRE(qkv && pos && cosT && sinT && kc && vtc && T > 0 && L > 0 && T % L == 0 && D % 2 == 0);
  hipLaunchKernelGGL(rope_kv_kernel, dim3(T), dim3(256), 0, stream, (bf16_t*)qkv, ldq, pos, L, Hq, Hkv, D, cosT, sinT,
                     (bf16_t*)kc, (bf16_t*)vtc, Smax, slot_base, slot_dev);
  PG_LAUNCH_CHECK();
  return 0;
}

#define AM_CHUNKS 64
__device__ __forceinline__ void am_better(float& bv, int& bi, float v, int i) {
  if (v > bv || (v == bv && i < bi)) { bv = v; bi = i; }
}
__device__ __forceinline__ void am_block(float& bv, int& bi, float* sv, int* si) {
  const int lane = threadIdx.x & 63, w = threadIdx.x >> 6;
#pragma unroll
  for (int o = 32; o > 0; o >>= 1) {
    float ov = __shfl_xor(bv, o, 64);
    int oi = __shfl_xor(bi, o, 64);
    am_better(bv, bi, ov, oi);
  }
  if (lane == 0) { sv[w] = bv; si[w] = bi; }
  __syncthreads();
  bv = sv[0]; bi = si[0];
  for (int i = 1; i < (int)(blockDim.x >> 6); ++i) am_better(bv, bi, sv[i], si[i]);
}

__global__ __launch_bounds__(256) void argmax_partial_kernel(const float* __restrict__ x, long ld, int V,
                                                             float* __restrict__ pv, int* __restrict__ pi) {
  __shared__ float sv[4];
  __shared__ int si[4];
  const int b = blockIdx.y, ch = blockIdx.x;
  const int per = ((V + AM_CHUNKS - 1) / AM_CHUNKS + 3) & ~3;
  const int s = ch * per, e = min(V, s + per);
  const float* row = x + (long)b * ld;
  float bv = -INFINITY;
  int bi = 0x7FFFFFFF;
  for (int i = s + threadIdx.x * 4; i < e; i += 1024) {
    if (i + 3 < e) {
      const f32x4 v = *(const f32x4*)(row + i);
#pragma unroll
      for (int j = 0; j < 4; ++j) am_better(bv, bi, v[j], i + j);
    } else {
      for (int j = 0; j < 4 && i + j < e; ++j) am_better(bv, bi, row[i + j], i + j);
    }
  }
  am_block(bv, bi, sv, si);
  if (threadIdx.x == 0) { pv[b * AM_CHUNKS + ch] = bv; pi[b * AM_CHUNKS + ch] = bi; }
}

__global__ __launch_bounds__(1024) void argmax_final_kernel(const float* __restrict__ pv, const int* __restrict__ pi,
                                                            int B, int64_t* __restrict__ out_ids, int64_t* __restrict__ hist,
                                                            int hist_rows, int* __restrict__ step, int* __restrict__ pos,
                                                            int* __restrict__ kv_len) {
  const int lane = threadIdx.x & 63, wave = threadIdx.x >> 6, nw = blockDim.x >> 6;
  const int st = step ? *step : 0;
  __syncthreads();
  for (int b = wave; b < B; b += nw) {
    float bv = pv[b * AM_CHUNKS + lane];
    int bi = pi[b * AM_CHUNKS + lane];
#pragma unroll
    for (int o = 32; o > 0; o >>= 1) {
      float ov = __shfl_xor(bv, o, 64);
      int oi = __shfl_xor(bi, o, 64);
      am_better(bv, bi, ov, oi);
    }
    if (lane == 0) {
      out_ids[b] = bi;
      if (hist && st < hist_rows) hist[(long)st * B + b] = bi;
      if (pos) pos[b] += 1;
    }
  }
  if (threadIdx.x == 0) {
    if (kv_len) *kv_len += 1;
    if (step) *step = st + 1;
  }
}

#define AM_EMB_MAX_B 1024
struct AmEmbArgs {
  const bf16_t* embed;
  int V, n_feat, H;
  const float* feat;
  int64_t image_id, pad_id;
  float img_scale, normalizer;
  float* res;
};
__global__ __launch_bounds__(1024) void argmax_final_embed_kernel(const float* __restrict__ pv, const int* __restrict__ pi,
                                                                  int B, int64_t* __restrict__ out_ids,
                                                                  int64_t* __restrict__ hist, int hist_rows,
                                                                  int* __restrict__ step, int* __restrict__ pos,
                                                                  int* __restrict__ kv_len, AmEmbArgs ea) {
  __shared__ int win[AM_EMB_MAX_B];
  const int lane = threadIdx.x & 63, wave = threadIdx.x >> 6, nw = blockDim.x >> 6;
  const int st = step ? *step : 0;
  for (int b = wave; b < B; b += nw) {
    float bv = pv[b * AM_CHUNKS + lane];
    int bi = pi[b * AM_CHUNKS + lane];
#pragma unroll
    for (int o = 32; o > 0; o >>= 1) {
      float ov = __shfl_xor(bv, o, 64);
      int oi = __shfl_xor(bi, o, 64);
      am_better(bv, bi, ov, oi);
    }
    if (lane == 0) {
      win[b] = bi;
      out_ids[b] = bi;
      if (hist && st < hist_rows) hist[(long)st * B + b] = bi;
      if (pos) pos[b] += 1;
    }
  }
  __syncthreads();
  if (threadIdx.x == 0) {
    if (kv_len) *kv_len += 1;
    if (step) *step = st + 1;
  }
  for (int b = wave; b < B; b += nw) {
    const int64_t id = win[b];
    int rk = 0;
    if (id == ea.image_id)
      for (int i = 0; i < b; ++i) rk += win[i] == ea.image_id;
    embed_row(ea.res + (long)b * ea.H, id, rk, lane, 64, ea.embed, ea.V, ea.feat, ea.n_feat, ea.H, ea.image_id,
              ea.pad_id, ea.img_scale, ea.normalizer);
  }
}

static inline int am_waves(int B) { return B < 1 ? 1 : (B > 16 ? 16 : B); }

__global__ __launch_bounds__(1024) void argmax_pairs_kernel(const float* __restrict__ pv, const int* __restrict__ pi,
                                                            int B, int vocab_offset, float* __restrict__ pairs) {
  const int lane = threadIdx.x & 63, wave = threadIdx.x >> 6, nw = blockDim.x >> 6;
  for (int b = wave; b < B; b += nw) {
    float bv = pv[b * AM_CHUNKS + lane];
    int bi = pi[b * AM_CHUNKS + lane];
#pragma unroll
    for (int o = 32; o > 0; o >>= 1) {
      float ov = __shfl_xor(bv, o, 64);
      int oi = __shfl_xor(bi, o, 64);
      am_better(bv, bi, ov, oi);
    }
    if (lane == 0) { pairs[2 * b] = bv; pairs[2 * b + 1] = (float)(bi + vocab_offset); }
  }
}

__global__ void argmax_merge_kernel(const float* __restrict__ pairs, int world, int B, int64_t* __restrict__ out_ids,
                                    int64_t* __restrict__ hist, int hist_rows, int* __restrict__ step, int* __restrict__ pos,
                                    int* __restrict__ kv_len) {
  if (threadIdx.x != 0) return;
  const int st = step ? *step : 0;
  for (int b = 0; b < B; ++b) {
    float bv = -INFINITY;
    int bi = 0x7FFFFFFF;
    for (int r = 0; r < world; ++r) am_better(bv, bi, pairs[(r * B + b) * 2], (int)pairs[(r * B + b) * 2 + 1]);
    out_ids[b] = bi;
    if (hist && st < hist_rows) hist[(long)st * B + b] = bi;
    if (pos) pos[b] += 1;
  }
  if (kv_len) *kv_len += 1;
  if (step) *step = st + 1;
}

extern "C" int pg_argmax_pairs(const float* logits, long ld, int B, int V, int vocab_offset, void* workspace,
                               float* pairs, hipStream_t stream) {
  PG_REQUIRE(logits && workspace && pairs && B > 0 && V > 0 && ld % 4 == 0 && vocab_offset >= 0 &&
             vocab_offset + V < (1 << 24));
  float* pv = (float*)workspace;
  int* pi = (int*)(pv + B * AM_CHUNKS);
  hipLaunchKernelGGL(argmax_partial_kernel, dim3(AM_CHUNKS, B), dim3(256), 0, stream, logits, ld, V, pv, pi);
  hipLaunchKernelGGL(argmax_pairs_kernel, dim3(1), dim3(64 * am_waves(B)), 0, stream, pv, pi, B, vocab_offset, pairs);
  PG_LAUNCH_CHECK();
  return 0;
}

extern "C" int pg_argmax_merge(const float* pairs, int world, int B, int64_t* out_ids, int64_t* hist, int hist_rows,
                               int* step, int* pos, int* kv_len, hipStream_t stream) {
  PG_REQUIRE(pairs && out_ids && world > 0 && B > 0 && (hist == nullptr || hist_rows > 0));
  hipLaunchKernelGGL(argmax_merge_kernel, dim3(1), dim3(64), 0, stream, pairs, world, B, out_ids, hist, hist_rows,
                     step, pos, kv_len);
  PG_LAUNCH_CHECK();
  return 0;
}

extern "C" int pg_argmax(const float* logits, long ld, int B, int V, void* workspace, int64_t* out_ids,
                         int64_t* hist, int hist_rows, int* step, int* pos, int* kv_len, hipStream_t stream) {
  PG_REQUIRE(logits && workspace && out_ids && B > 0 && V > 0 && ld % 4 == 0 && (hist == nullptr || hist_rows > 0));
  float* pv = (float*)workspace;
  int* pi = (int*)(pv + B * AM_CHUNKS);
  hipLaunchKernelGGL(argmax_partial_kernel, dim3(AM_CHUNKS, B), dim3(256), 0, stream, logits, ld, V, pv, pi);
  hipLaunchKernelGGL(argmax_final_kernel, dim3(1), dim3(64 * am_waves(B)), 0, stream, pv, pi, B, out_ids, hist, hist_rows, step, pos,
                     kv_len);
  PG_LAUNCH_CHECK();
  return 0;
}

extern "C" int pg_argmax_embed(const float* logits, long ld, int B, int V, void* workspace, int64_t* out_ids,
                               int64_t* hist, int hist_rows, int* step, int* pos, int* kv_len, const void* embed,
                               int V_embed, const float* feat, int n_feat, int H, long image_id, long pad_id,
                               float img_scale, float normalizer, float* res, hipStream_t stream) {
  PG_REQUIRE(logits && workspace && out_ids && B > 0 && B <= AM_EMB_MAX_B && V > 0 && ld % 4 == 0 &&
             (hist == nullptr || hist_rows > 0));
  PG_REQUIRE(embed != nullptr && res != nullptr && V_embed > 0 && H > 0 && H % 4 == 0 && (n_feat == 0 || feat));
  float* pv = (float*)workspace;
  int* pi = (int*)(pv + B * AM_CHUNKS);
  const AmEmbArgs ea{(const bf16_t*)embed, V_embed, n_feat, H, feat, (int64_t)image_id, (int64_t)pad_id,
                     img_scale, normalizer, res};
  hipLaunchKernelGGL(argmax_partial_kernel, dim3(AM_CHUNKS, B), dim3(256), 0, stream, logits, ld, V, pv, pi);
  hipLaunchKernelGGL(argmax_final_embed_kernel, dim3(1), dim3(64 * am_waves(B)), 0, stream, pv, pi, B, out_ids, hist,
                     hist_rows, step, pos, kv_len, ea);
  PG_LAUNCH_CHECK();
  return 0;
}

__global__ __launch_bounds__(1024) void topp_kernel(const float* __restrict__ logits, long ld, int V, float inv_temp,
                                                    float top_p, const float* __restrict__ uniforms,
                                                    int64_t* __restrict__ out_ids, int64_t* __restrict__ hist, int hist_rows,
                                                    int* __restrict__ step, int* __restrict__ pos, int B,
                                                    int* __restrict__ kv_len, float* __restrict__ probs_out) {
  __shared__ float red[16];
  __shared__ float hist_mass[256];
  __shared__ float scan[1024];
  __shared__ int sel;
  __shared__ float sel_above;
  const int b = blockIdx.x;
  const float* x = logits + (long)b * ld;
  const int tid = threadIdx.x;
  float mx = -INFINITY;
  for (int i = tid; i < V; i += 1024) mx = fmaxf(mx, x[i] * inv_temp);
  mx = wave_max(mx);
  if ((tid & 63) == 0) red[tid >> 6] = mx;
  __syncthreads();
  mx = red[0];
  for (int i = 1; i < 16; ++i) mx = fmaxf(mx, red[i]);
  __syncthreads();
  float z = 0.f;
  for (int i = tid; i < V; i += 1024) z += __expf(x[i] * inv_temp - mx);
  z = block_sum(z, red);
  const float target = top_p * z;
  uint32_t prefix = 0;
  float above = 0.f;
  for (int digit = 3; digit >= 0; --digit) {
    const int shift = digit * 8;
    const uint32_t hi_mask = digit == 3 ? 0u : (0xFFFFFFFFu << (shift + 8));
    for (int i = tid; i < 256; i += 1024) hist_mass[i] = 0.f;
    __syncthreads();
    for (int i = tid; i < V; i += 1024) {
      const float e = __expf(x[i] * inv_temp - mx);
      const uint32_t u = __float_as_uint(e);
      if ((u & hi_mask) == (prefix & hi_mask)) atomicAdd(&hist_mass[(u >> shift) & 255], e);
    }
    __syncthreads();
    if (tid == 0) {
      float acc = above;
      int k = 255;
      for (; k >= 0; --k) {
        if (acc + hist_mass[k] > target && hist_mass[k] > 0.f) break;
        acc += hist_mass[k];
      }
      if (k < 0) {
        acc = above;
        for (k = 0; k < 256 && hist_mass[k] == 0.f; ++k) {}
        for (int j = 255; j > k; --j) acc += hist_mass[j];
      }
      sel = k;
      sel_above = acc;
    }
    __syncthreads();
    prefix |= ((uint32_t)sel) << shift;
    above = sel_above;
    __syncthreads();
  }
  const float t0 = __uint_as_float(prefix);
  const int per = (V + 1023) / 1024;
  const int s = min(V, tid * per), e = min(V, s + per);
  float mine = 0.f;
  for (int i = s; i < e; ++i) {
    const float v = __expf(x[i] * inv_temp - mx);
    if (v >= t0) mine += v;
  }
  scan[tid] = mine;
  __syncthreads();
  for (int off = 1; off < 1024; off <<= 1) {
    float v = tid >= off ? scan[tid - off] : 0.f;
    __syncthreads();
    scan[tid] += v;
    __syncthreads();
  }
  const float kept = scan[1023];
  if (probs_out) {
    for (int i = s; i < e; ++i) {
      const float v = __expf(x[i] * inv_temp - mx);
      probs_out[(long)b * V + i] = v >= t0 ? v / kept : 0.f;
    }
  }
  const long srow = step ? (long)min(*step, hist_rows - 1) : 0;
  const float u = uniforms[srow * B + b] * kept;
  const float lo = scan[tid] - mine;
  __shared__ int chosen;
  if (tid == 0) chosen = -1;
  __syncthreads();
  if (mine > 0.f && u >= lo && u < scan[tid]) {
    float run = lo;
    int pick = -1, last = -1;
    for (int i = s; i < e; ++i) {
      const float v = __expf(x[i] * inv_temp - mx);
      if (v >= t0) {
        last = i;
        run += v;
        if (run > u) { pick = i; break; }
      }
    }
    atomicMax(&chosen, pick >= 0 ? pick : last);
  }
  __syncthreads();
  if (tid == 0) {
    int c = chosen;
    if (c < 0) {
      for (int i = V - 1; i >= 0; --i) if (__expf(x[i] * inv_temp - mx) >= t0) { c = i; break; }
    }
    out_ids[b] = c;
    if (hist && (!step || *step < hist_rows)) hist[srow * B + b] = c;
    if (pos) pos[b] += 1;
  }
}

__global__ void advance_kernel(int* step, int* kv_len) {
  if (kv_len) *kv_len += 1;
  if (step) *step += 1;
}

extern "C" int pg_topp_sample(const float* logits, long ld, int B, int V, float temperature, float top_p,
                              const float* uniforms, int64_t* out_ids, int64_t* hist, int hist_rows, int* step, int* pos,
                              int* kv_len, float* probs_out, hipStream_t stream) {
  PG_REQUIRE(logits && uniforms && out_ids && B > 0 && V > 0 && temperature > 0.f && hist_rows > 0);
  hipLaunchKernelGGL(topp_kernel, dim3(B), dim3(1024), 0, stream, logits, ld, V, 1.0f / temperature, top_p, uniforms,
                     out_ids, hist, hist_rows, step, pos, B, kv_len, probs_out);
  hipLaunchKernelGGL(advance_kernel, dim3(1), dim3(1), 0, stream, step, kv_len);
  PG_LAUNCH_CHECK();
  return 0;
}

__device__ __forceinline__ uint32_t fmix32(uint32_t h) {
  h ^= h >> 16; h *= 0x85EBCA6Bu; h ^= h >> 13; h *= 0xC2B2AE35u; h ^= h >> 16;
  return h;
}
__device__ __forceinline__ uint32_t bf16_rne_bits(float v) {
  const uint32_t u = __float_as_uint(v);
  return (u + 0x7FFFu + ((u >> 16) & 1u)) >> 16;
}
__global__ void synth_kernel(void* out, long n, uint32_t seedmix, float a, float mean, int out_kind) {
  for (long i = blockIdx.x * (long)blockDim.x + threadIdx.x; i < n; i += (long)gridDim.x * blockDim.x) {
    const uint32_t h = fmix32((uint32_t)i * 0x9E3779B1u + seedmix);
    float v = __fmul_rn((float)(h >> 8), 5.9604644775390625e-08f);
    v = __fsub_rn(__fmul_rn(v, 2.0f), 1.0f);
    v = __fmul_rn(v, a);
    if (mean != 0.0f) v = __fadd_rn(v, mean);
    const uint32_t bits = bf16_rne_bits(v);
    if (out_kind == 0) ((bf16_t*)out)[i] = (bf16_t)bits;
    else ((float*)out)[i] = __uint_as_float(bits << 16);
  }
}

extern "C" int pg_synth_fill(void* out, long n, unsigned int seedmix, float a, float mean, int out_kind,
                             hipStream_t stream) {
  PG_REQUIRE(out && n > 0 && n <= 0xFFFFFFFFl && (out_kind == 0 || out_kind == 1));
  const int grid = (int)min((n + 255) / 256, (long)16384);
  hipLaunchKernelGGL(synth_kernel, dim3(grid), dim3(256), 0, stream, out, n, (uint32_t)seedmix, a, mean, out_kind);
  PG_LAUNCH_CHECK();
  return 0;
}

extern "C" int pg_abi_version(void) { return 13; }

#ifndef PG_SOURCE_HASH
#define PG_SOURCE_HASH "unknown"
#endif
__attribute__((used)) static const char pg_source_hash_str[] = "PGHIP_SOURCE_HASH=" PG_SOURCE_HASH;
extern "C" int pg_source_hash(char* out, int n) {
  const char* h = pg_source_hash_str + 18;
  PG_REQUIRE(n <= 0 || out != nullptr);
  int i = 0;
  for (; h[i] && i + 1 < n; ++i) out[i] = h[i];
  if (n > 0) out[i] = 0;
  return h[i] ? (int)hipErrorInvalidValue : 0;
}

__device__ __forceinline__ uint8_t clip8_22(int acc) {
  const int v = acc >> 22;
  return (uint8_t)(v < 0 ? 0 : (v > 255 ? 255 : v));
}

__global__ __launch_bounds__(256) void resize_h_kernel(const uint8_t* __restrict__ src, int W, int y0, int rows,
                                                       int S, const int* __restrict__ hb, const int* __restrict__ hk,
                                                       int hks, uint8_t* __restrict__ tmp) {
  const long total = (long)rows * S * 3;
  for (long i = blockIdx.x * (long)blockDim.x + threadIdx.x; i < total; i += (long)gridDim.x * blockDim.x) {
    const int c = (int)(i % 3), xx = (int)((i / 3) % S);
    const long r = i / (3L * S);
    const int xmin = hb[2 * xx], n = hb[2 * xx + 1];
    const int* k = hk + (long)xx * hks;
    const uint8_t* p = src + ((long)(y0 + r) * W + xmin) * 3 + c;
    int acc = 1 << 21;
    for (int x = 0; x < n; ++x) acc += (int)p[3 * x] * k[x];
    tmp[i] = clip8_22(acc);
  }
}

__global__ __launch_bounds__(256) void resize_v_kernel(const uint8_t* __restrict__ in, int Win, int yshift, int S,
                                                       const int* __restrict__ vb, const int* __restrict__ vk,
                                                       int vks, const float* __restrict__ lut,
                                                       float* __restrict__ out) {
  const long total = 3L * S * S;
  for (long i = blockIdx.x * (long)blockDim.x + threadIdx.x; i < total; i += (long)gridDim.x * blockDim.x) {
    const int xx = (int)(i % S), yy = (int)((i / S) % S), c = (int)(i / ((long)S * S));
    int v;
    if (vb) {
      const int ymin = vb[2 * yy] - yshift, n = vb[2 * yy + 1];
      const int* k = vk + (long)yy * vks;
      const uint8_t* p = in + ((long)ymin * Win + xx) * 3 + c;
      int acc = 1 << 21;
      for (int y = 0; y < n; ++y) acc += (int)p[(long)y * Win * 3] * k[y];
      v = clip8_22(acc);
    } else {
      v = in[((long)yy * Win + xx) * 3 + c];
    }
    out[i] = lut[v];
  }
}

extern "C" int pg_image_preprocess(const uint8_t* src, int H, int W, int S, const int* hb, const int* hk, int hks,
                                   const int* vb, const int* vk, int vks, int y0, int rows, const float* lut,
                                   uint8_t* tmp, float* out, hipStream_t stream) {
  PG_REQUIRE(H > 0 && W > 0 && S > 0 && lut && out && src);
  PG_REQUIRE(hb ? (hk && hks > 0 && tmp && rows > 0 && y0 >= 0 && y0 + rows <= H) : W == S);
  PG_REQUIRE(vb ? (vk && vks > 0) : (hb ? rows == S : H == S));
  const uint8_t* in = src;
  int win = W, yshift = 0;
  if (hb) {
    const long n = (long)rows * S * 3;
    hipLaunchKernelGGL(resize_h_kernel, dim3((int)min((n + 255) / 256, 4096L)), dim3(256), 0, stream, src, W, y0,
                       rows, S, hb, hk, hks, tmp);
    in = tmp;
    win = S;
    yshift = y0;
  }
  const long n = 3L * S * S;
  hipLaunchKernelGGL(resize_v_kernel, dim3((int)min((n + 255) / 256, 4096L)), dim3(256), 0, stream, in, win, yshift,
                     S, vb, vk, vks, lut, out);
  PG_LAUNCH_CHECK();
  return 0;
}

__device__ __forceinline__ int clip8_22_px(int acc) {
  const int hi = (256 << 22) - 1;
  return (int)((uint32_t)(acc < 0 ? 0 : (acc > hi ? hi : acc)) >> 22);
}

template <int C>
__device__ __forceinline__ void load_px(const uint8_t* __restrict__ p, int (&v)[C]) {
  if constexpr (C == 4) {
    const uint32_t w = *reinterpret_cast<const uint32_t*>(p);
    v[0] = (int)(w & 255u), v[1] = (int)((w >> 8) & 255u), v[2] = (int)((w >> 16) & 255u), v[3] = (int)(w >> 24);
  } else if constexpr (C == 2) {
    const uint32_t w = *reinterpret_cast<const uint16_t*>(p);
    v[0] = (int)(w & 255u), v[1] = (int)(w >> 8);
  } else {
#pragma unroll
    for (int c = 0; c < C; ++c) v[c] = p[c];
  }
}

template <int C>
__device__ __forceinline__ void store_px(uint8_t* __restrict__ p, const int (&v)[C]) {
  if constexpr (C == 4) {
    *reinterpret_cast<uint32_t*>(p) =
        (uint32_t)v[0] | ((uint32_t)v[1] << 8) | ((uint32_t)v[2] << 16) | ((uint32_t)v[3] << 24);
  } else if constexpr (C == 2) {
    *reinterpret_cast<uint16_t*>(p) = (uint16_t)(v[0] | (v[1] << 8));
  } else {
#pragma unroll
    for (int c = 0; c < C; ++c) p[c] = (uint8_t)v[c];
  }
}

template <int C>
__device__ __forceinline__ void premultiply_px(int (&v)[C]) {
#pragma unroll
  for (int c = 0; c < C - 1; ++c) {
    const int t = v[c] * v[C - 1] + 128;
    v[c] = ((t >> 8) + t) >> 8;
  }
}

template <int C, bool ALPHA>
__global__ __launch_bounds__(256) void resize_h_px_kernel(const uint8_t* __restrict__ src, int W, int y0, int rows,
                                                          int S, const int* __restrict__ hb,
                                                          const int* __restrict__ hk, int hks,
                                                          uint8_t* __restrict__ tmp) {
  const long total = (long)rows * S;
  for (long i = blockIdx.x * (long)blockDim.x + threadIdx.x; i < total; i += (long)gridDim.x * blockDim.x) {
    const int xx = (int)(i % S);
    const long r = i / S;
    const int xmin = hb[2 * xx], n = hb[2 * xx + 1];
    const int* k = hk + (long)xx * hks;
    const uint8_t* p = src + ((long)(y0 + r) * W + xmin) * C;
    int acc[C];
#pragma unroll
    for (int c = 0; c < C; ++c) acc[c] = 1 << 21;
    for (int x = 0; x < n; ++x) {
      int v[C];
      load_px<C>(p + (long)x * C, v);
      if constexpr (ALPHA) premultiply_px<C>(v);
      const int kx = k[x];
#pragma unroll
      for (int c = 0; c < C; ++c) acc[c] += v[c] * kx;
    }
// ... 115 lines not shown
```

paligemma-multimodal-system_amd/pghip/_lib.py:

```python
from __future__ import annotations

import ctypes as C
import os

_HERE = os.path.dirname(os.path.abspath(__file__))
LIB_PATH = os.environ.get("PGHIP_LIB") or os.path.join(_HERE, "libpghip.so")

vp, i32, i64, f32, u32 = C.c_void_p, C.c_int, C.c_long, C.c_float, C.c_uint

class PgFusedArgs(C.Structure):
    _fields_ = [("pro_mode", C.c_int), ("resid_in", C.c_void_p), ("resid_out", C.c_void_p),
                ("partials", C.c_void_p), ("nsplit", C.c_int), ("norm_w", C.c_void_p), ("eps", C.c_float),
                ("part_o", C.c_void_p), ("part_ml", C.c_void_p), ("asplit", C.c_int), ("head_dim", C.c_int),
                ("dtw", C.c_int), ("q_per_kv", C.c_int), ("kv_heads", C.c_int), ("cos_t", C.c_void_p),
                ("sin_t", C.c_void_p), ("pos", C.c_void_p), ("rows_per_batch", C.c_int), ("slot_dev", C.c_void_p),
                ("slot_base", C.c_int), ("kc", C.c_void_p), ("vtc", C.c_void_p), ("smax", C.c_int),
                ("q_heads", C.c_int), ("fin_cnt", C.c_void_p), ("fin_resid", C.c_void_p), ("ss_out", C.c_void_p),
                ("ss_in", C.c_void_p), ("ss_ld", C.c_int), ("ss_n", C.c_int), ("fin_x", C.c_void_p),
                ("akeys", C.c_int), ("a_scale", C.c_void_p), ("w_scale", C.c_void_p),
                ("slab_rows", C.c_int), ("kd", C.c_void_p), ("vd", C.c_void_p),
                ("amax_out", C.c_void_p), ("amax_in", C.c_void_p), ("amax_ld", C.c_int), ("amax_zero", C.c_void_p),
                ("amax_zero_n", C.c_int), ("fx", C.c_void_p),
                ("mx_out", C.c_void_p), ("mx_in", C.c_void_p), ("status", C.c_void_p)]


SIGNATURES = {
    "pg_abi_version": [],
    "pg_source_hash": [C.c_char_p, i32],
    "pg_gemm": [vp, i32, vp, i32, vp, vp, i32, i32, i32, i32, i32, i32, vp, i32, vp, i32, i32, vp],
    "pg_gemm_fused": [vp, i32, vp, i32, vp, vp, i32, i32, i32, i32, i32, i32, C.POINTER(PgFusedArgs), vp],
    "pg_gemm_finalize": [vp, i32, vp, i32, i32, i32, i32, vp, i32, i32, C.POINTER(PgFusedArgs), vp],
    "pg_norm_residual": [vp, vp, i32, i32, vp, vp, vp, i32, vp, vp, i32, i32, i32, f32, i32, vp],
    "pg_attention": [vp, i64, vp, i64, vp, i64, i64, i64, vp, i64, i64, i64, vp, i64, i64,
                     i32, i32, i32, vp, i32, i32, i32, f32, i32, i32, vp, vp, i32, vp, vp, vp],
    "pg_attn_combine": [vp, vp, i32, i32, i32, i32, i32, vp, i64, vp],
    "pg_attn_probs": [vp, i64, vp, i64, i64, i64, vp, i64, i64, i32, i32, i32, i32, i32, i32, f32, i32, vp, vp],
    "pg_attn_decode": [vp, i64, vp, i64, vp, vp, i32, i32, vp, i32, i32, i32, f32, i32, i32, i32, i32, vp, vp, vp,
                       vp, vp, i64, vp],
    "pg_rope_kv_write": [vp, i32, vp, i32, i32, i32, i32, i32, vp, vp, vp, vp, i32, i32, vp, vp],
    "pg_patch_im2col": [vp, i32, i32, i32, i32, i32, vp, i32, vp],
    "pg_image_rank": [vp, i32, i64, vp, vp],
    "pg_embed_merge": [vp, vp, i32, vp, i32, vp, i32, i32, i64, i64, f32, f32, vp, vp],
    "pg_argmax": [vp, i64, i32, i32, vp, vp, vp, i32, vp, vp, vp, vp],
    "pg_argmax_embed": [vp, i64, i32, i32, vp, vp, vp, i32, vp, vp, vp, vp, i32, vp, i32, i32, i64, i64, f32, f32, vp,
                        vp],
    "pg_argmax_pairs": [vp, i64, i32, i32, i32, vp, vp, vp],
    "pg_argmax_merge": [vp, i32, i32, vp, vp, i32, vp, vp, vp, vp],
    "pg_topp_sample": [vp, i64, i32, i32, f32, f32, vp, vp, vp, i32, vp, vp, vp, vp, vp],
    "pg_image_preprocess": [vp, i32, i32, i32, vp, vp, i32, vp, vp, i32, i32, i32, vp, vp, vp, vp],
    "pg_image_preprocess_modes": [vp, i32, i32, i32, i32, i32, vp, vp, i32, vp, vp, i32, i32, i32, vp, vp, vp, vp],
    "pg_image_palette": [vp, i32, i32, i32, vp, vp, vp, vp, vp],
    "pg_synth_fill": [vp, i64, u32, f32, f32, i32, vp],
    "pg_quant_fp8": [vp, i32, i32, i32, vp, i32, vp, vp],
    "pg_norm_residual_fp8": [vp, vp, i32, i32, vp, vp, vp, i32, vp, vp, i32, i32, i32, f32, i32, vp],
    "pg_norm_residual_mx": [vp, vp, i32, i32, vp, vp, i32, vp, vp, i32, i32, i32, i32, vp],
    "pg_xgmi_buffer_bytes": [i32, i64, C.POINTER(C.c_long)],
    "pg_xgmi_alloc": [i64, C.POINTER(C.c_void_p)],
    "pg_xgmi_free": [vp],
    "pg_xgmi_ipc_handle": [vp, C.c_char_p],
    "pg_xgmi_ipc_open": [C.c_char_p, C.POINTER(C.c_void_p)],
    "pg_xgmi_ipc_close": [vp],
    "pg_allreduce_xgmi": [vp, i64, i32, i32, C.POINTER(C.c_void_p), i64, vp, vp, vp],
    "pg_allreduce_xgmi_slabs": [vp, i64, i32, i64, i32, i32, C.POINTER(C.c_void_p), i64, vp, vp, vp],
    "pg_allgather_xgmi": [vp, i64, vp, i32, i32, C.POINTER(C.c_void_p), i64, vp, vp, vp],
    "pg_xgmi_rs_buffer_bytes": [i32, i64, C.POINTER(C.c_long)],
    "pg_allreduce_xgmi_rs": [vp, i64, i32, i64, i32, i32, C.POINTER(C.c_void_p), i64, i32, vp, vp, vp],
}

_lib = None
_hip = None


class PgHipError(RuntimeError):
    pass


ABI_VERSION = 13


def source_hash(lib=None) -> str:
    lib = load() if lib is None else lib
    buf = C.create_string_buffer(80)
    if lib.pg_source_hash(buf, 80) != 0:
        raise PgHipError("pg_source_hash: buffer too small")
    return buf.value.decode()


def load(path: str = LIB_PATH) -> C.CDLL:
    global _lib
    if _lib is not None:
        return _lib
    if not os.path.exists(path):
        raise PgHipError(f"libpghip.so not found at {path}: build it with `python -m pghip.build` "
                         "(or __graft_entry__.build()); there is no CPU fallback.")
    lib = C.CDLL(path, mode=C.RTLD_GLOBAL)
    for name, argtypes in SIGNATURES.items():
        fn = getattr(lib, name)
        fn.argtypes = argtypes
        fn.restype = C.c_int
    if lib.pg_abi_version() != ABI_VERSION:
        raise PgHipError(f"{path}: ABI {lib.pg_abi_version()}, this package expects {ABI_VERSION}; rebuild it")
    if not os.environ.get("PGHIP_LIB"):
        from . import build
        if os.path.isdir(build.CSRC):
            want, got = build.source_hash(), source_hash(lib)
            if want != got:
                raise PgHipError(f"{path} was built from other sources (hash {got[:16]}, tree {want[:16]}): "
                                 "rebuild it with `python -m pghip.build`")
    _lib = lib
    return lib


def _err_string(code: int) -> str:
    global _hip
    try:
        if _hip is None:
            _hip = C.CDLL("libamdhip64.so.7")
            _hip.hipGetErrorString.restype = C.c_char_p
            _hip.hipGetErrorString.argtypes = [C.c_int]
        return _hip.hipGetErrorString(code).decode()
    except Exception:
        return "?"


def call(name: str, *args) -> None:
    rc = getattr(load(), name)(*args)
    if rc != 0:
        raise PgHipError(f"{name} failed: hip error {rc} ({_err_string(rc)})")
```

paligemma-multimodal-system_amd/pghip/engine.py:

```python
from __future__ import annotations

import math
import os
from types import SimpleNamespace
from typing import Optional

import torch

from . import ops
from .tp import CaptureUnsupported, SoloComm
from .weights import PackedWeights


def _rup(x: int, m: int) -> int:
    return (x + m - 1) // m * m


def rope_tables(dim: int, n_pos: int, base: float, device):
    inv = 1.0 / (base ** (torch.arange(0, dim, 2, dtype=torch.int64).float() / dim))
    pos = torch.arange(n_pos, dtype=torch.int64).float()
    freqs = inv[None, :] * pos[:, None]
    return freqs.cos().to(device).contiguous(), freqs.sin().to(device).contiguous()


class KVStore:

    def __init__(self, layers: int, B: int, Smax: int, kv_dim: int, device, kv_heads: int = 1):
        if kv_dim % kv_heads:
            raise ValueError(f"kv_dim {kv_dim} does not split into {kv_heads} kv heads")
        self.B, self.Smax, self.kv_dim, self.kv_heads = B, Smax, kv_dim, kv_heads
        self.k = torch.zeros(layers, B, Smax, kv_dim, dtype=torch.bfloat16, device=device)
        self.vt = torch.zeros(layers, B, kv_dim, Smax, dtype=torch.bfloat16, device=device)
        self.kd = torch.zeros(layers, B * Smax * kv_dim, dtype=torch.bfloat16, device=device)
        self.vd = torch.zeros(layers, B * Smax * kv_dim, dtype=torch.bfloat16, device=device)
        self.length = 0

    def copy_prefix_from(self, old: "KVStore", n: int):
        nl = old.k.shape[0]
        self.k[:nl, :, :n] = old.k[:, :, :n]
        self.vt[:nl, :, :, :n] = old.vt[:, :, :, :n]
        if (old.B, old.kv_dim, old.kv_heads) != (self.B, self.kv_dim, self.kv_heads):
            raise ValueError("copy_prefix_from: the stores differ in batch or kv-head layout")
        nb = -(-n // 32) * 32
        hk, hd = self.kv_heads, self.kv_dim // self.kv_heads
        for t_new, t_old in ((self.kd, old.kd), (self.vd, old.vd)):
            t_new.view(-1, self.B, hk, self.Smax, hd)[:nl, :, :, :nb] = t_old.view(nl, old.B, hk, old.Smax, hd)[:, :, :, :nb]


class PaliGemmaEngine:
    DECODE_SPLIT_O = 2
    DECODE_SPLIT_O_SMALL = 2
    DECODE_SPLIT_O_FIN16, DECODE_SPLIT_DOWN_FIN16 = 1, 4
    DECODE_SPLIT_DOWN = 8
    DECODE_SPLIT_KEYS = 32
    DECODE_SPLIT_KEYS_SMALL = int(os.environ.get("PG_SK_SMALL", "32"))
    PREFILL_ROWMAJOR_MIN_M = int(os.environ.get("PG_ROWMAJOR_MIN_M", "256"))
    ROW_BLOCKS = os.environ.get("PG_ROW_BLOCKS", "1") != "0"
    TAIL_SPLIT = os.environ.get("PG_TAIL_SPLIT", "1") != "0"
    HEAD_KSPLIT = os.environ.get("PG_HEAD_KSPLIT", "1") != "0"
    ROW_BLOCKS_GU = os.environ.get("PG_ROW_BLOCKS_GU", "1") != "0"
    TILE_M1 = os.environ.get("PG_TILE_M1", "1") != "0"
    TILE_M1_SPLIT = {"gu": 1, "down": int(os.environ.get("PG_M1_DOWN", "16"))}
    FUSE_MAX_B = 2
    DECODE_SPLIT_TARGET = 1024
    FIN_MIN_B = 5
    USE_FIN = True
    VISION_DP = os.environ.get("PG_VISION_DP", "1") != "0"
    AR_CHUNK_ROWS = int(os.environ.get("PG_AR_CHUNK_ROWS", "4096"))
    CHAIN_EMBED = os.environ.get("PG_CHAIN_EMBED", "1") != "0"
    MX_H = os.environ.get("PG_MX_H", "1") != "0"
    MX_NORM = os.environ.get("PG_MX_NORM", "1") != "0"
    MX_PREFILL = os.environ.get("PG_MX_PREFILL", "1") != "0"
    PREFILL_RES = os.environ.get("PG_PREFILL_RES", "1") != "0"
    PREFILL_RES_MIN_M = int(os.environ.get("PG_PREFILL_RES_MIN_M", "65536"))

    DECODE_FUSED_ATTN = os.environ.get("PG_DECODE_FUSED", "1") != "0"
    FUSED_MIN_ROUNDS = int(os.environ.get("PG_FUSED_MIN_ROUNDS", "2"))
    ATTN_FP8_OUT = os.environ.get("PG_ATTN_FP8_OUT", "1") != "0"
    DECODE_ADD = os.environ.get("PG_DECODE_ADD", "fx")
    FP8_GEMV = os.environ.get("PG_FP8_GEMV", "1") != "0"

    def __init__(self, cfg: dict, weights: PackedWeights, device="cuda", comm=None):
        self.cfg = cfg
        self.w = weights
        self.comm = comm if comm is not None else SoloComm()
        self.fp8 = bool(getattr(weights, "fp8", False))
        self.tp = getattr(weights, "tp_world", 1)
        if self.comm.world != self.tp:
            raise ValueError(f"weights packed for tp_world={self.tp}, communicator has world {self.comm.world}")
        self.split_o = self.DECODE_SPLIT_O if self.tp == 1 else 1
        self.split_down = self.DECODE_SPLIT_DOWN if self.tp == 1 else max(1, self.DECODE_SPLIT_DOWN // self.tp)
        env_o, env_d = os.environ.get("PG_SPLIT_O"), os.environ.get("PG_SPLIT_DOWN")
        if env_o:
            self.split_o = int(env_o)
        if env_d:
            self.split_down = int(env_d)
        self._split_fixed = (bool(env_o), bool(env_d))
        self._validate_splits()
        self.device = torch.device(device)
        self.image_token_id = cfg.get("image_token_index", 256000)
        pad = cfg.get("pad_token_id")
        self.pad_id = -1 if pad is None else pad
        self.n_img = weights.n_img
        self._rope = None
        self._rope_n = 0
        self._ws = {}
        self.graphs = {}

    def _validate_splits(self):
        w = self.w
        if not hasattr(w, "heads"):
            return
        checks = [("o_proj (PG_SPLIT_O)", self.split_o, w.heads * w.head_dim, 8),
                  ("o_proj at batch <= 2", self.DECODE_SPLIT_O_SMALL, w.heads * w.head_dim, 8),
                  ("down_proj (PG_SPLIT_DOWN)", self.split_down, w.inter, 8)]
        if self.TILE_M1:
            checks.append(("batch-1 prefill down_proj (PG_M1_DOWN)", self.TILE_M1_SPLIT["down"], 64 * 64, 64))
        for what, ks, K, hi in checks:
            if not 1 <= ks <= hi:
                raise ValueError(f"split-K {ks} for {what}: needs 1 <= split <= {hi} (K = {K})")

    def _buf(self, name, shape, dtype):
        t = self._ws.get(name)
        n = math.prod(shape)
        if t is None or t.numel() < n or t.dtype != dtype:
            t = torch.empty(max(n, 1), dtype=dtype, device=self.device)
            self._ws[name] = t
        return t[:n].view(*shape)

    def rope(self, n_pos: int):
        if self._rope is None or self._rope_n < n_pos:
            n = _rup(max(n_pos, 1024), 1024)
            self._rope = rope_tables(self.w.head_dim, n, self.w.rope_theta, self.device)
            self._rope_n = n
        return self._rope

    def new_cache(self, B: int, Smax: int) -> KVStore:
        w = self.w
        return KVStore(w.t_layers, B, _rup(Smax, 64), w.kv_heads * w.head_dim, self.device, kv_heads=w.kv_heads)

    def vision(self, pixel_values: torch.Tensor, want_hidden: bool = False, taps: Optional[list] = None,
               _split_batch: Optional[int] = None):
        w = self.w
        px = pixel_values.to(device=self.device, dtype=torch.float32).contiguous()
        B = px.shape[0]
        if (_split_batch is None and self.tp > 1 and self.VISION_DP and B >= self.tp and B % self.tp == 0
                and not want_hidden and taps is None and w.proj_w is not None):
            Bl = B // self.tp
            mine = self.vision(px[self.comm.rank * Bl:(self.comm.rank + 1) * Bl], _split_batch=B)
            feats = torch.empty(B * w.n_img, w.proj_dim, dtype=torch.float32, device=self.device)
            self.comm.all_gather(feats, mine)
            return feats
        N, hv, nh, hd = w.n_img, w.v_hidden, w.v_heads, w.v_head_dim
        M = B * N
        patches = self._buf("v_patches", (M, w.patch_k), torch.bfloat16)
        ops.patch_im2col(px, w.patch, patches)
        resid = self._buf("v_resid", (M, hv), torch.float32)
        ops.gemm(patches, w.patch_w, resid, epi=ops.EPI_F32_POS, bias=w.patch_b, aux=w.pos_emb, aux_rows=N)
        if taps is not None:
            taps.append(resid.clone())
        xn = self._buf("v_xn", (M, hv), torch.bfloat16)
        qkv = self._buf("v_qkv", (M, 3 * hv), torch.bfloat16)
        vt = self._buf("v_vt", (hv, M + 32), torch.bfloat16)
        attn = self._buf("v_attn", (M, hv), torch.bfloat16)
        h = self._buf("v_h", (M, w.v_inter), torch.bfloat16)
        Bs = _split_batch or B
        s_o = ops.gemm_ksplit(Bs * N, hv, hv)
        s_2 = ops.gemm_ksplit(Bs * N, hv, w.v_inter)
        ks_v = self._key_split_args("v", Bs, N, N, nh, nh, hd)
        part = self._buf("v_part", (max(s_o, s_2), M, hv), torch.float32)
        res = self.PREFILL_RES and M >= max(17, self.PREFILL_RES_MIN_M)
        res_o, res_2 = res and s_o == 1, res and s_2 == 1
        ns = 0
        for L in w.vl:
            ops.norm_residual(resid, L["ln1_w"], b=L["ln1_b"], mode=ops.NORM_LAYER, eps=w.v_eps, partials=part,
                              nsplit=ns, out=xn, write_resid=ns > 0)
            ops.gemm(xn, L["qkv_w"], qkv, epi=ops.EPI_BF16_VT, bias=L["qkv_b"], aux_out=vt, aux_ld=M + 32,
                     aux_n=2 * hv, split_m=Bs * N)
            ops.attention(qkv, 3 * hv, attn, hv, qkv[:, hv:], N * 3 * hv, hd, 3 * hv, vt, N, hd * (M + 32), M + 32,
                          B=B, Lq=N, Lkv=N, Hq=nh, Hkv=nh, D=hd, scale=1.0 / (hd ** 0.5), **ks_v)
            if res_o:
                ops.gemm(attn, L["o_w"], resid, epi=ops.EPI_F32_RES, bias=L["o_b"])
            else:
                ops.gemm(attn, L["o_w"], part, epi=ops.EPI_F32, bias=L["o_b"], ksplit=s_o)
            ops.norm_residual(resid, L["ln2_w"], b=L["ln2_b"], mode=ops.NORM_LAYER, eps=w.v_eps, partials=part,
                              nsplit=0 if res_o else s_o, out=xn, write_resid=not res_o)
            ops.gemm(xn, L["fc1_w"], h, epi=ops.EPI_BF16_GELU, bias=L["fc1_b"], split_m=Bs * N)
            if res_2:
                ops.gemm(h, L["fc2_w"], resid, epi=ops.EPI_F32_RES, bias=L["fc2_b"])
                ns = 0
            else:
                ops.gemm(h, L["fc2_w"], part, epi=ops.EPI_F32, bias=L["fc2_b"], ksplit=s_2)
                ns = s_2
            if taps is not None:
                taps.append((resid + part[:ns].sum(0)).clone())
        hid = torch.empty(M, hv, dtype=torch.float32, device=self.device) if want_hidden else None
        ops.norm_residual(resid, w.post_w, b=w.post_b, mode=ops.NORM_LAYER, eps=w.v_eps, partials=part, nsplit=ns,
                          out=xn, out_f32=hid)
        feats = torch.empty(M, max(w.proj_dim, 1), dtype=torch.float32, device=self.device)
        if w.proj_w is None:
            return (None, hid) if want_hidden else None
        ops.gemm(xn, w.proj_w, feats, epi=ops.EPI_F32)
        return (feats, hid) if want_hidden else feats

    def _embed_kw(self) -> dict:
        return dict(image_id=self.image_token_id, pad_id=self.pad_id, img_scale=float(self.w.proj_dim ** -0.5),
                    normalizer=float(self.w.hidden ** 0.5))

    def embed_merge(self, input_ids: torch.Tensor, feats: torch.Tensor, out: torch.Tensor, rank=None):
        ids = input_ids.reshape(-1)
        n = ids.numel()
        if rank is None and n > 64:
            rank = self._buf("rank", (n,), torch.int32)
            ops.image_rank(ids, self.image_token_id, rank)
        ops.embed_merge(ids, rank, self.w.embed, feats, feats.shape[0] if feats is not None else 0, out,
                        **self._embed_kw())

    def gemma_prefill(self, x_resid: torch.Tensor, positions: torch.Tensor, cache: KVStore, B: int, L: int,
                      logits_rows: Optional[torch.Tensor] = None, mask: Optional[torch.Tensor] = None,
                      want_hidden: bool = False, want_logits: bool = True, taps: Optional[list] = None):
        w = self.w
        T = B * L
        H, I, nh, nkv, hd = w.hidden, w.inter, w.heads, w.kv_heads, w.head_dim
        cos_t, sin_t = self.rope(L + 2)
        xn = self._buf("t_xn", (T, H), torch.bfloat16)
        qb = self._buf("t_q", (T, nh * hd), torch.bfloat16)
        attn = self._buf("t_attn", (T, nh * hd), torch.bfloat16)
        h = self._buf("t_h", (T, I), torch.bfloat16)
        s_o = self._ksplit(T, H, nh * hd) if T > 16 else self.DECODE_SPLIT_O
        s_d = self._ksplit(T, H, I) if T > 16 else self.DECODE_SPLIT_DOWN
        part = self._buf("t_part", (max(s_o, s_d), T, H), torch.float32)
        pos = positions.to(device=self.device, dtype=torch.int32).reshape(-1).contiguous()
        ks_t = self._key_split_args("t", B, L, L, nh, nkv, hd) if mask is None else {}
        ns = 0
        if taps is not None:
            taps.append(x_resid.clone())
        kvd = nkv * hd
        for i, Lw in enumerate(w.tl):
            xin = self._norm(x_resid, Lw["in_w"], part, ns, xn, T)
            fa = ops.fused_args(head_dim=hd, cos_t=cos_t, sin_t=sin_t, pos=pos, rows_per_batch=L, slot_base=0,
                                kc=cache.k[i], vtc=cache.vt[i], smax=cache.Smax, q_heads=nh, kv_heads=nkv,
                                kd=cache.kd[i], vd=cache.vd[i])
            self._lin(xin, Lw, "qkv", qb, ops.EPI_QKV_ROPE, T, fa=fa)
            ops.attention(qb, nh * hd, attn, attn.stride(0), cache.k[i], cache.Smax * kvd, hd, kvd,
                          cache.vt[i], kvd * cache.Smax, hd * cache.Smax, cache.Smax,
                          B=B, Lq=L, Lkv=L, Hq=nh, Hkv=nkv, D=hd, scale=1.0 / math.sqrt(hd),
                          mask=mask, mask_bs=(mask.stride(0) if mask is not None else 0),
                          mask_rs=(mask.stride(-2) if mask is not None else 0), **ks_t)
            n_o = self._row_parallel(attn, Lw, "o", part, T, s_o, resid=x_resid)
            xin = self._norm(x_resid, Lw["post_w"], part, n_o, xn, T)
            if self._mx_prefill(T):
                h8 = self._buf("t_h8", (T, I), torch.uint8)
                hs = self._buf("t_hs", (T, I // 32), torch.uint8)
                x8, xs = xin
                ops.gemm8(x8, xs, Lw["gu_w8"], Lw["gu_s8"], h8, epi=ops.EPI_BF16_GELU_MUL, M=T, mx_out=hs)
                ns = self._row_parallel(("mx", h8, hs), Lw, "down", part, T, s_d, resid=x_resid)
            else:
                self._lin(xin, Lw, "gu", h, ops.EPI_BF16_GELU_MUL, T)
                ns = self._row_parallel(h, Lw, "down", part, T, s_d, resid=x_resid)
            if taps is not None:
                taps.append((x_resid + part[:ns].sum(0)).clone())
        cache.length = L
        rows = logits_rows.numel() if logits_rows is not None else T
        xf = self._buf("t_xf", (rows, H), torch.bfloat16)
        hid = torch.empty(rows, H, dtype=torch.float32, device=self.device) if want_hidden else None
        ops.norm_residual(x_resid, w.final_w, mode=ops.NORM_RMS, partials=part, nsplit=ns, out=xf, out_f32=hid,
                          row_map=logits_rows, write_resid=False)
        logits = self.lm_head(xf, rows, fresh=True) if want_logits else None
        return logits, hid

    def _key_split_args(self, tag: str, B: int, Lq: int, Lkv: int, Hq: int, Hkv: int, D: int) -> dict:
        nks = ops.prefill_key_splits(B, Lq, Lkv, Hq, Hkv)
        if nks <= 1:
            return {}
        no, nml = ops.prefill_split_workspace(B, Lq, Hq, Hkv, D, nks)
        return dict(nsplit=nks, part_o=self._buf(f"pf_po_{tag}", (no,), torch.float32),
                    part_ml=self._buf(f"pf_pml_{tag}", (nml,), torch.float32))

    def _fp8_rows(self, M: int) -> bool:
        return self.fp8 and M > 16

    def _mx_prefill(self, M: int) -> bool:
        L0 = self.w.tl[0]
        chunks_ok = self.tp == 1 or M < 2 * self.AR_CHUNK_ROWS or self.AR_CHUNK_ROWS >= 64
        return (self.MX_PREFILL and self._fp8_rows(M) and M > 32 and "gu_w8" in L0 and "down_w8" in L0
                and self.w.inter % 128 == 0 and chunks_ok)

    def _mx_decode(self, B: int) -> tuple:
        w = self.w
        L0 = w.tl[0]
        mx_h = (self.FP8_GEMV and self._fp8_rows(B) and B <= 32 and self.MX_H and "gu_w8f" in L0
                and "down_w8f" in L0 and w.inter % 128 == 0 and w.hidden <= 4096)
        mx_n = (mx_h and self.MX_NORM and "qkv_w8f" in L0 and w.hidden % 1024 == 0
                and getattr(w, "lm_w8f", None) is not None)
        return mx_h, mx_n

    def _ksplit(self, M: int, N: int, K: int) -> int:
        if self._fp8_rows(M):
            return ops.gemm_ksplit(M, N, K // 2)
        m1 = self._tile_m1(M, "down" if K == self.w.inter else "o")
        if m1:
            return m1
        Mh = M // 256 * 256
        if self.ROW_BLOCKS and self.HEAD_KSPLIT and 0 < Mh < M:
            s = ops.gemm_ksplit(Mh, N, K)
            if self._row_head(M, N, s):
                return s
        return ops.gemm_ksplit(M, N, K)

    def _tile_m1(self, M: int, name: str) -> int:
        if (not self.TILE_M1 or self.fp8 or self.tp != 1 or not 256 <= M <= 288
                or M < self.PREFILL_ROWMAJOR_MIN_M):
            return 0
        ks = self.TILE_M1_SPLIT.get(name, 0)
        K = self.w.inter if name == "down" else self.w.hidden
        return ks if ks * 64 <= K else 0

    def _lin(self, x: torch.Tensor, Lw: dict, name: str, out: torch.Tensor, epi: int, M: int, ksplit: int = 1,
             fa=None):
        if isinstance(x, tuple) and x[0] == "mx":
            return ops.gemm8(x[1], None, Lw[name + "_w8"], Lw[name + "_s8"], out, epi=epi, M=M, ksplit=ksplit, fa=fa,
                             mx_in=x[2])
        if not isinstance(x, tuple) and self._fp8_rows(M):
            x8, xs = self._x8(M, x.shape[1])
            ops.quant_fp8(x, x8, xs, M=M)
            x = (x8, xs)
        if isinstance(x, tuple):
            x8, xs = x
            if self.FP8_GEMV and M <= 32 and name + "_w8f" in Lw:
                return ops.gemm8(x8, xs, Lw[name + "_w8f"], Lw[name + "_s8"], out, epi=epi, M=M, ksplit=ksplit,
                                 fa=fa, frag=True)
            return ops.gemm8(x8, xs, Lw[name + "_w8"], Lw[name + "_s8"], out, epi=epi, M=M, ksplit=ksplit, fa=fa)
        W, flag = Lw[name + "_w"], self.w.wflag
        if M >= self.PREFILL_ROWMAJOR_MIN_M and name + "_wr" in Lw:
            W, flag = Lw[name + "_wr"], 0
            if fa is None and self._tile_m1(M, name) == ksplit:
                return ops.gemm(x, W, out, epi=epi | ops.TILE_M1, ksplit=ksplit)
        if fa is not None:
            return ops.gemm_fused(x, W, out, fa, epi=epi | flag, M=M)
        if epi == ops.EPI_F32 and self.ROW_BLOCKS:
            Mh = self._row_head(M, W.shape[0], ksplit)
            if Mh:
                return self._lin_row_blocks(x, W, out, epi | flag, M, Mh, ksplit)
        if epi == ops.EPI_BF16_GELU_MUL and self.ROW_BLOCKS and self.ROW_BLOCKS_GU:
            Mh = self._row_head(M, W.shape[0], 1)
            if Mh:
                ops.gemm(x[:Mh], W, out[:Mh], epi=epi | flag)
                return ops.gemm(x[Mh:M], W, out[Mh:M], epi=epi | flag)
        return ops.gemm(x, W, out, epi=epi | flag, ksplit=ksplit)

    def _lin_row_blocks(self, x: torch.Tensor, W: torch.Tensor, out: torch.Tensor, epi: int, M: int, Mh: int,
                        ksplit: int):
        fr = ops.fused_args(slab_rows=M)
        ops.gemm_fused(x[:Mh], W, out, fr, epi=epi, M=Mh, ksplit=ksplit, ldc=out.stride(-2))
        N, K, Mt = W.shape[0], W.shape[1], M - Mh
        st = max(ksplit, ops.split_for(math.ceil(Mt / 64) * math.ceil(N / 128), K // 64, max_split=8))
        if st > ksplit and self.TAIL_SPLIT:
            tp = self._buf("row_tail", (st, Mt, N), torch.float32)
            ops.gemm(x[Mh:M], W, tp, epi=epi, ksplit=st)
            ops.slab_sum(tp, out[0, Mh:M])
            if ksplit > 1:
                out[1:ksplit, Mh:M].zero_()
            return out
        tail = out.view(-1)[Mh * out.stride(-2):]
        return ops.gemm_fused(x[Mh:M], W, tail, fr, epi=epi, M=Mt, ksplit=ksplit, ldc=out.stride(-2))

    def _x8(self, M: int, K: int) -> tuple:
        return self._buf(f"x8_{K}", (M, K), torch.uint8), self._buf(f"xs_{K}", (M,), torch.float32)

    @staticmethod
    def _row_head(M: int, N: int, ksplit: int, cus: int = ops.CUS) -> int:
        Mh = M // 256 * 256
        tn = (N + 255) // 256
        if Mh == M or Mh == 0 or (M + 255) // 256 * tn * ksplit < cus:
            return 0
        rounds = lambda tiles: (tiles + cus - 1) // cus
        return Mh if rounds(Mh // 256 * tn * ksplit) < rounds((M + 255) // 256 * tn * ksplit) else 0

    def _norm(self, resid: torch.Tensor, norm_w: torch.Tensor, part, nsplit: int, xn: torch.Tensor, M: int):
        if self._fp8_rows(M):
            x8, xs = self._x8(M, resid.shape[-1])
            return ops.norm_residual_fp8(resid, norm_w, x8, xs, mode=ops.NORM_RMS, partials=part, nsplit=nsplit,
                                         write_resid=nsplit > 0)
        ops.norm_residual(resid, norm_w, mode=ops.NORM_RMS, partials=part, nsplit=nsplit, out=xn,
                          write_resid=nsplit > 0)
        return xn

    def _allreduce_slabs(self, part: torch.Tensor, ns: int) -> int:
        if self.tp == 1:
            return ns
        return self.comm.all_reduce_slabs(part[:ns], ns)

    def _row_parallel(self, x: torch.Tensor, Lw: dict, name: str, part: torch.Tensor, T: int, ks: int,
                      resid: Optional[torch.Tensor] = None) -> int:
        if self.tp == 1:
            row_blocks = (not self._fp8_rows(T) and self.ROW_BLOCKS and
                          self._row_head(T, self.w.hidden, 1) > 0)
            if (resid is not None and self.PREFILL_RES and ks == 1 and T >= max(17, self.PREFILL_RES_MIN_M)
                    and not row_blocks):
                self._lin(x, Lw, name, resid, ops.EPI_F32_RES, T)
                return 0
            self._lin(x, Lw, name, part, ops.EPI_F32, T, ksplit=ks)
            return ks
        C = -(-T // self.AR_CHUNK_ROWS) if T >= 2 * self.AR_CHUNK_ROWS else 1
        if C <= 1:
            self._lin(x, Lw, name, part, ops.EPI_F32, T, ksplit=ks)
            return self.comm.all_reduce_slabs(part[:ks], ks)
        bounds = [T * c // C for c in range(C + 1)]
        works = []
        for r0, r1 in zip(bounds[:-1], bounds[1:]):
            xc = ("mx", x[1][r0:r1], x[2][r0:r1]) if isinstance(x, tuple) else x[r0:r1]
            self._lin(xc, Lw, name, part[0, r0:r1], ops.EPI_F32, r1 - r0, ksplit=1)
            works.append(self.comm.all_reduce_async(part[0, r0:r1]))
        for wk in works:
            wk.wait()
        return 1

    def lm_head(self, xf: torch.Tensor, rows: int, fresh: bool = False, name: str = "lm"):
        w = self.w
        alloc = (lambda shape: torch.empty(*shape, dtype=torch.float32, device=self.device)) if fresh else \
            (lambda shape: self._buf(name, shape, torch.float32))
        if self.tp == 1:
            logits = alloc((rows, w.vocab_local_pad))
            self._lm_gemm(xf, rows, logits)
            return logits[:, :w.vocab]
        vl, vlp = w.vocab_local, w.vocab_local_pad
        loc = self._buf(name + "_loc", (rows, vlp), torch.float32)
        self._lm_gemm(xf, rows, loc)
        g = self._buf(name + "_gather", (self.tp, rows, vlp), torch.float32)
        self.comm.all_gather(g, loc)
        out = alloc((rows, w.vocab))
        out.view(rows, self.tp, vl).copy_(g[:, :, :vl].permute(1, 0, 2))
        return out

    def _lm_gemm(self, xf: torch.Tensor, rows: int, out: torch.Tensor):
        w = self.w
        if isinstance(xf, tuple):
            _, x8, xs, ss = xf
            return ops.gemm8(x8, None, w.lm_w8f, w.lm_s8, out, epi=ops.EPI_F32, M=rows, bias=w.lm_bias, frag=True,
                             mx_in=xs, ss_in=ss)
        if self.FP8_GEMV and self._fp8_rows(rows) and rows <= 32 and getattr(w, "lm_w8f", None) is not None:
            x8, xs = self._x8(rows, xf.shape[1])
            ops.quant_fp8(xf, x8, xs, M=rows)
            return ops.gemm8(x8, xs, w.lm_w8f, w.lm_s8, out, epi=ops.EPI_F32, M=rows, bias=w.lm_bias, frag=True)
        return ops.gemm(xf, w.lm_w, out, epi=ops.EPI_F32 | w.wflag, bias=w.lm_bias)

    def _chain_ok(self, sampler) -> bool:
        return self.CHAIN_EMBED and self.tp == 1 and sampler is not None and not sampler.get("do_sample")

    def decode_state(self, B: int, cache: KVStore, positions_next: torch.Tensor, max_steps: int, sampler=None):
        st = {
            "ids": torch.zeros(B, dtype=torch.int64, device=self.device),
            "pos": positions_next.to(device=self.device, dtype=torch.int32).reshape(B).contiguous().clone(),
            "kv_len": torch.full((1,), cache.length, dtype=torch.int32, device=self.device),
            "step": torch.zeros(1, dtype=torch.int32, device=self.device),
            "hist": torch.zeros(max_steps + 1, B, dtype=torch.int64, device=self.device),
            "ws": torch.empty(B * 64 * 2, dtype=torch.float32, device=self.device),
            "chain": self._chain_ok(sampler),
        }
        return st

    def _decode_route(self, B: int) -> str:
        fin_rows = B <= self.FUSE_MAX_B or self.FIN_MIN_B <= B <= 16
        if self.tp == 1 and self.USE_FIN and fin_rows and not self._fp8_rows(B):
            return "fin"
        return "unfused" if B > self.FUSE_MAX_B else "fused"

    def _decode_splits(self, B: int, route: str) -> tuple:
        so, sd = self.split_o, self.split_down
        fixed_o, fixed_d = self._split_fixed
        if route == "fin" and B > self.FUSE_MAX_B:
            so = so if fixed_o else self.DECODE_SPLIT_O_FIN16
            sd = sd if fixed_d else self.DECODE_SPLIT_DOWN_FIN16
        elif self.tp == 1 and B <= self.FUSE_MAX_B and not fixed_o:
            so = self.DECODE_SPLIT_O_SMALL
        return so, sd

    def _decode_ws(self, B: int, cache: KVStore) -> SimpleNamespace:
        w = self.w
        H, nh, nkv, hd = w.hidden, w.heads, w.kv_heads, w.head_dim
        route = self._decode_route(B)
        so, sd = self._decode_splits(B, route)
        cos_t, sin_t = self.rope(cache.Smax + 2)
        SK = self._split_keys(B, cache.Smax)
        nsplit = _rup((cache.Smax + SK - 1) // SK, 4)
        dt = (hd + 15) // 16 * 16
        ns_ws = max(nsplit, ops.decode_plan(B, nkv, cache.Smax)[0]) if B > self.FUSE_MAX_B else nsplit
        return SimpleNamespace(
            B=B, route=route, so=so, sd=sd, SK=SK, nsplit=nsplit, dt=dt, cos_t=cos_t, sin_t=sin_t,
            res_a=self._buf("d_res_a", (B, H), torch.float32),
            res_b=self._buf("d_res_b", (B, H), torch.float32),
            xn=self._buf("d_xn", (B, H), torch.bfloat16),
            qb=self._buf("d_q", (B, nh * hd), torch.bfloat16),
            h=self._buf("d_h", (B, w.inter), torch.bfloat16),
            part=self._buf("d_part", (max(so, sd), B, H), torch.float32),
            part_o=self._buf("d_po", (B * nkv * ns_ws * 16 * dt,), torch.float32),
            part_ml=self._buf("d_pml", (B * nkv * ns_ws * 16 * 2,), torch.float32))

    def decode_step(self, st: dict, cache: KVStore, feats: Optional[torch.Tensor], sampler: dict):
        w = self.w
        B = st["ids"].numel()
        ws = self._decode_ws(B, cache)
        chain = bool(st.get("chain")) and self._chain_ok(sampler)
        if not chain:
            ops.embed_merge(st["ids"], None, w.embed, feats, feats.shape[0] if feats is not None else 0, ws.res_a,
                            **self._embed_kw())
        if ws.route == "fin":
            xq, ss, tiles, n_ss = self._decode_layers_fin(st, cache, ws)
            logits = self._buf("d_logits", (B, w.vocab_local_pad), torch.float32)
            fa = ops.fused_args(pro_mode=ops.PRO_X_RSTD, ss_in=ss, ss_ld=tiles, ss_n=n_ss, eps=1e-6)
            ops.gemm_fused(xq, w.lm_w, logits, fa, epi=ops.EPI_F32 | w.wflag, M=B, bias=w.lm_bias)
            logits = logits[:, :w.vocab]
        else:
            layers = self._decode_layers_fused if ws.route == "fused" else self._decode_layers_unfused
            ns = layers(st, cache, ws)
            xn = ws.xn
            if ws.route == "unfused" and self._mx_decode(B)[1]:
                H = w.hidden
                xn = ("mx",) + ops.norm_residual_mx(ws.res_a, w.final_w, self._buf("d_x8n", (B, H), torch.uint8),
                                                    self._buf("d_xsn", (B * H // 32,), torch.uint8),
                                                    self._buf("d_ssn", (B, H // 1024), torch.float32),
                                                    partials=ws.part, nsplit=ns, write_resid=False)
            else:
                ops.norm_residual(ws.res_a, w.final_w, mode=ops.NORM_RMS, partials=ws.part, nsplit=ns, out=xn,
                                  write_resid=False)
            if self.tp > 1 and sampler is not None and not sampler.get("do_sample"):
                return self._tp_greedy(xn, st)
            logits = self.lm_head(xn, B, name="d_logits")
        if sampler is not None:
            self.sample(logits, st, sampler, advance=True, feats=feats)
        return logits

    def _tp_greedy(self, xn, st: dict) -> torch.Tensor:
        w = self.w
        B = st["ids"].numel()
        loc = self._buf("d_logits_loc", (B, w.vocab_local_pad), torch.float32)
        self._lm_gemm(xn, B, loc)
        loc = loc[:, :w.vocab_local]
        Bp = B + (B & 1)
        mine = self._buf("d_pairs_loc", (Bp, 2), torch.float32)
        ops.argmax_pairs(loc, st["ws"], mine, vocab_offset=w.vocab_offset)
        pairs = self._buf("d_pairs", (self.tp, Bp, 2), torch.float32)
        self.comm.all_gather(pairs, mine)
        if Bp != B:
            pairs = self._buf("d_pairs_b", (self.tp, B, 2), torch.float32).copy_(pairs[:, :B])
        ops.argmax_merge(pairs, st["ids"], world=self.tp, hist=st["hist"], step=st["step"], pos=st["pos"],
                         kv_len=st["kv_len"])
        return loc

    def _rope_kw(self, i: int, st: dict, cache: KVStore, ws) -> dict:
        w = self.w
        return dict(head_dim=w.head_dim, cos_t=ws.cos_t, sin_t=ws.sin_t, pos=st["pos"], rows_per_batch=1,
                    slot_dev=st["kv_len"], slot_base=0, kc=cache.k[i], vtc=cache.vt[i], smax=cache.Smax,
                    q_heads=w.heads, kv_heads=w.kv_heads, kd=cache.kd[i], vd=cache.vd[i])

    def _attn_split(self, i: int, st: dict, cache: KVStore, ws):
        w = self.w
        nh, nkv, hd = w.heads, w.kv_heads, w.head_dim
        kvd = nkv * hd
        ops.attention(ws.qb, nh * hd, None, nh * hd, cache.k[i], cache.Smax * kvd, hd, kvd,
                      cache.vt[i], kvd * cache.Smax, hd * cache.Smax, cache.Smax,
                      B=ws.B, Lq=1, Lkv=1, lkv_dev=st["kv_len"], Hq=nh, Hkv=nkv, D=hd,
                      scale=1.0 / math.sqrt(hd), split_keys=ws.SK, nsplit=ws.nsplit, part_o=ws.part_o,
                      part_ml=ws.part_ml, kcap=cache.Smax, kd=cache.kd[i], vd=cache.vd[i])

    def _combine_kw(self, st: dict, ws) -> dict:
        w = self.w
        return dict(pro_mode=ops.PRO_ATTN_COMBINE, part_o=ws.part_o, part_ml=ws.part_ml, asplit=ws.nsplit,
                    head_dim=w.head_dim, dtw=ws.dt, q_per_kv=w.heads // w.kv_heads, kv_heads=w.kv_heads,
                    slot_dev=st["kv_len"], akeys=ws.SK)

    def _decode_attn_merged(self, i: int, st: dict, cache: KVStore, ws, want_fp8: bool = False):
        w = self.w
        B = ws.B
        nh, nkv, hd = w.heads, w.kv_heads, w.head_dim
        attn = self._buf("d_attn", (B, nh * hd), torch.bfloat16)
        plan = ops.decode_plan(B, nkv, cache.Smax)
        if self.DECODE_FUSED_ATTN and hd in (32, 256) and cache.Smax >= 64 and plan[2] >= self.FUSED_MIN_ROUNDS:
            x8 = None
            if want_fp8 and self.ATTN_FP8_OUT and ops.attn_decode_q8_ok(nh, nkv, hd, plan[1]):
                x8 = self._x8(B, nh * hd)
            ops.attn_decode(ws.qb, nh * hd, attn, nh * hd, cache.kd[i], cache.vd[i],
                            B=B, Lkv=1, lkv_dev=st["kv_len"], Hq=nh, Hkv=nkv, D=hd, scale=1.0 / math.sqrt(hd),
                            kcap=cache.Smax, part_o=ws.part_o, part_ml=ws.part_ml,
                            counters=self._zeros("d_dec_cnt", (B * nkv,), torch.int32), plan=plan,
                            q8=x8[0] if x8 else None, q8_scale=x8[1] if x8 else None)
            return x8 or attn
        self._attn_split(i, st, cache, ws)
        ops.attn_combine(ws.part_o, ws.part_ml, attn, nh * hd, B=B, Hq=nh, Hkv=nkv, D=hd, nsplit=ws.nsplit)
        return attn

    def fx_status(self) -> torch.Tensor:
        return self._zeros("d_fx_status", (1,), torch.int32)

    def check_numerics(self):
        t = self._ws.get("d_fx_status")
        if t is not None and int(t.item()):
            t.zero_()
            raise FloatingPointError("decode residual: a non-finite or out-of-range (|v| >= 2^31) value reached the "
                                     "fixed-point accumulator; the generated tokens are invalid")

    def _zeros(self, name, shape, dtype):
        t = self._ws.get(name)
        if t is None or tuple(t.shape) != tuple(shape) or t.dtype != dtype:
            t = torch.zeros(*shape, dtype=dtype, device=self.device)
            self._ws[name] = t
        return t

    def _decode_layers_fused(self, st: dict, cache: KVStore, ws) -> int:
        w = self.w
        B, res_a, res_b, part = ws.B, ws.res_a, ws.res_b, ws.part
        ns = 0
        for i, Lw in enumerate(w.tl):
            fa = ops.fused_args(pro_mode=ops.PRO_RMSNORM, resid_in=res_a, resid_out=res_b, partials=part, nsplit=ns,
                                norm_w=Lw["in_w"], eps=1e-6, **self._rope_kw(i, st, cache, ws))
            ops.gemm_fused(None, Lw["qkv_w"], ws.qb, fa, epi=ops.EPI_QKV_ROPE | w.wflag, M=B)
            self._attn_split(i, st, cache, ws)
            fa = ops.fused_args(**self._combine_kw(st, ws))
            ops.gemm_fused(None, Lw["o_w"], part, fa, epi=ops.EPI_F32 | w.wflag, M=B, ksplit=ws.so)
            n_o = self._allreduce_slabs(part, ws.so)
            fa = ops.fused_args(pro_mode=ops.PRO_RMSNORM, resid_in=res_b, resid_out=res_a, partials=part, nsplit=n_o,
                                norm_w=Lw["post_w"], eps=1e-6)
            ops.gemm_fused(None, Lw["gu_w"], ws.h, fa, epi=ops.EPI_BF16_GELU_MUL | w.wflag, M=B)
            ops.gemm(ws.h, Lw["down_w"], part, epi=ops.EPI_F32 | w.wflag, ksplit=ws.sd)
            ns = self._allreduce_slabs(part, ws.sd)
        return ns

    def _decode_layers_fin(self, st: dict, cache: KVStore, ws):
        w = self.w
        B, res, part = ws.B, ws.res_a, ws.part
        H = w.hidden
        tiles = (H + 15) // 16
        merge_in_gemv = B <= self.FUSE_MAX_B
        fx = self._zeros("d_fx", (B, H), torch.int64) if merge_in_gemv and self.DECODE_ADD == "fx" else None
        f = SimpleNamespace(
            tiles=tiles,
            n_ss=tiles if B <= 4 else (tiles + 1) // 2,
            cnt=self._zeros("d_fin_cnt", (tiles,), torch.int32),
            ss_o=self._buf("d_ss_o", (B, tiles), torch.float32),
            ss_d=self._buf("d_ss_d", (B, tiles), torch.float32),
            xq=self._buf("d_xq", (B, H), torch.bfloat16),
            add_down=merge_in_gemv and self.DECODE_ADD in ("down", "both", "fx"),
            add_o=merge_in_gemv and self.DECODE_ADD in ("both", "fx"),
            fx=fx,
            fx_st=self.fx_status() if fx is not None else None,
            add_epi=ops.EPI_FX_ADD if fx is not None else ops.EPI_F32_ADD,
            add_dst=fx if fx is not None else res)
        fin_o = dict(fin_cnt=f.cnt, fin_resid=res, ss_out=f.ss_o, ss_ld=tiles, fin_x=f.xq)
        for i, Lw in enumerate(w.tl):
            rope = self._rope_kw(i, st, cache, ws)
            if i == 0 or f.add_down:
                fa = ops.fused_args(pro_mode=ops.PRO_RMSNORM, resid_in=res if (i == 0 or fx is None) else None,
                                    fx=fx if i > 0 else None, nsplit=0, norm_w=Lw["in_w"], eps=1e-6, **rope)
                if i == 0 and fx is not None:
                    fa.amax_zero, fa.amax_zero_n = fx.data_ptr(), fx.numel() * 2
                ops.gemm_fused(None, Lw["qkv_w"], ws.qb, fa, epi=ops.EPI_QKV_ROPE | w.wflag, M=B)
            else:
                fa = ops.fused_args(pro_mode=ops.PRO_X_RSTD, ss_in=f.ss_d, ss_ld=tiles, ss_n=f.n_ss, eps=1e-6, **rope)
                ops.gemm_fused(f.xq, Lw["qkv_w"], ws.qb, fa, epi=ops.EPI_QKV_ROPE | w.wflag, M=B)
            if not merge_in_gemv:
                attn = self._decode_attn_merged(i, st, cache, ws)
                fa = ops.fused_args(norm_w=Lw["post_w"], **fin_o)
                ops.gemm_fused(attn, Lw["o_w"], part, fa, epi=ops.EPI_F32_FIN | w.wflag, M=B, ksplit=ws.so)
            else:
                self._attn_split(i, st, cache, ws)
                if f.add_o:
                    fa = ops.fused_args(resid_in=res if (fx is not None and i == 0) else None, status=f.fx_st,
                                        **self._combine_kw(st, ws))
                    ops.gemm_fused(None, Lw["o_w"], f.add_dst, fa, epi=f.add_epi | w.wflag, M=B, ksplit=ws.so)
                else:
                    fa = ops.fused_args(norm_w=Lw["post_w"], **fin_o, **self._combine_kw(st, ws))
                    ops.gemm_fused(None, Lw["o_w"], part, fa, epi=ops.EPI_F32_FIN | w.wflag, M=B, ksplit=ws.so)
            self._mlp_fin(i, ws, f)
        return f.xq, f.ss_d, tiles, f.n_ss

    def _mlp_fin(self, i: int, ws, f):
        w = self.w
        Lw, last = w.tl[i], i + 1 == len(w.tl)
        B, res, fx = ws.B, ws.res_a, f.fx
        if f.add_o:
            fa = ops.fused_args(pro_mode=ops.PRO_RMSNORM, resid_in=res if fx is None else None, fx=fx, nsplit=0,
                                norm_w=Lw["post_w"], eps=1e-6)
            ops.gemm_fused(None, Lw["gu_w"], ws.h, fa, epi=ops.EPI_BF16_GELU_MUL | w.wflag, M=B)
        else:
            fa = ops.fused_args(pro_mode=ops.PRO_X_RSTD, ss_in=f.ss_o, ss_ld=f.tiles, ss_n=f.n_ss, eps=1e-6)
            ops.gemm_fused(f.xq, Lw["gu_w"], ws.h, fa, epi=ops.EPI_BF16_GELU_MUL | w.wflag, M=B)
        if f.add_down and not last:
            ops.gemm_fused(ws.h, Lw["down_w"], f.add_dst, ops.fused_args(status=f.fx_st), epi=f.add_epi | w.wflag,
                           M=B, ksplit=ws.sd)
            return
        nxt_w = w.final_w if last else w.tl[i + 1]["in_w"]
        fa = ops.fused_args(fin_cnt=f.cnt, fin_resid=res, ss_out=f.ss_d, ss_ld=f.tiles, fin_x=f.xq, norm_w=nxt_w, fx=fx)
        ops.gemm_fused(ws.h, Lw["down_w"], ws.part, fa, epi=ops.EPI_F32_FIN | w.wflag, M=B, ksplit=ws.sd)

    def _split_keys(self, B: int, Smax: int) -> int:
        SK = self.DECODE_SPLIT_KEYS
        if B <= self.FUSE_MAX_B:
            return self.DECODE_SPLIT_KEYS_SMALL
        blocks = (Smax + SK - 1) // SK
        mult = max(1, min(8, (B * blocks) // self.DECODE_SPLIT_TARGET))
        return SK * (1 << (mult.bit_length() - 1))

    def _decode_layers_unfused(self, st: dict, cache: KVStore, ws) -> int:
        w = self.w
        B, res, part, h = ws.B, ws.res_a, ws.part, ws.h
        I, H = w.inter, w.hidden
        mx, mxn = self._mx_decode(B)
        if mx:
            h8 = self._buf("d_h8", (B, I), torch.uint8)
            hs = self._buf("d_hs", (B * I // 32,), torch.uint8)
        if mxn:
            x8n = self._buf("d_x8n", (B, H), torch.uint8)
            xsn = self._buf("d_xsn", (B * H // 32,), torch.uint8)
            ssn = self._buf("d_ssn", (B, H // 1024), torch.float32)
        ns = 0
        for i, Lw in enumerate(w.tl):
            fa = ops.fused_args(**self._rope_kw(i, st, cache, ws))
            if mxn:
                ops.norm_residual_mx(res, Lw["in_w"], x8n, xsn, ssn, partials=part, nsplit=ns)
                ops.gemm8(x8n, None, Lw["qkv_w8f"], Lw["qkv_s8"], ws.qb, epi=ops.EPI_QKV_ROPE, M=B, fa=fa, frag=True,
                          mx_in=xsn, ss_in=ssn)
            else:
                xin = self._norm(res, Lw["in_w"], part, ns, ws.xn, B)
                self._lin(xin, Lw, "qkv", ws.qb, ops.EPI_QKV_ROPE, B, fa=fa)
            attn = self._decode_attn_merged(i, st, cache, ws, want_fp8=self._fp8_rows(B))
            self._lin(attn, Lw, "o", part, ops.EPI_F32, B, ksplit=ws.so)
            n_o = self._allreduce_slabs(part, ws.so)
            if mxn:
                ops.norm_residual_mx(res, Lw["post_w"], x8n, xsn, ssn, partials=part, nsplit=n_o)
                ops.gemm8(x8n, None, Lw["gu_w8f"], Lw["gu_s8"], h8, epi=ops.EPI_BF16_GELU_MUL, M=B, frag=True,
                          mx_in=xsn, ss_in=ssn, mx_out=hs)
            else:
                xin = self._norm(res, Lw["post_w"], part, n_o, ws.xn, B)
                if mx:
                    x8, xs = xin
                    ops.gemm8(x8, xs, Lw["gu_w8f"], Lw["gu_s8"], h8, epi=ops.EPI_BF16_GELU_MUL, M=B, frag=True,
                              mx_out=hs)
                else:
                    self._lin(xin, Lw, "gu", h, ops.EPI_BF16_GELU_MUL, B)
            if mx:
                ops.gemm8(h8, None, Lw["down_w8f"], Lw["down_s8"], part, epi=ops.EPI_F32, M=B, ksplit=ws.sd,
                          frag=True, mx_in=hs)
            else:
                self._lin(h, Lw, "down", part, ops.EPI_F32, B, ksplit=ws.sd)
            ns = self._allreduce_slabs(part, ws.sd)
        return ns

    def sample(self, logits: torch.Tensor, st: dict, sampler: dict, advance: bool,
               feats: Optional[torch.Tensor] = None):
        kw = dict(hist=st["hist"], step=st["step"])
        if advance:
            kw.update(pos=st["pos"], kv_len=st["kv_len"])
        if st.get("chain") and self._chain_ok(sampler):
            w = self.w
            B = st["ids"].numel()
            ops.argmax_embed(logits, st["ids"], st["ws"], w.embed, feats, feats.shape[0] if feats is not None else 0,
                             self._buf("d_res_a", (B, w.hidden), torch.float32), **self._embed_kw(), **kw)
        elif sampler.get("do_sample"):
            ops.topp_sample(logits, st["ids"], sampler["uniforms"], temperature=sampler["temperature"],
                            top_p=sampler["top_p"], **kw)
        else:
            ops.argmax(logits, st["ids"], st["ws"], **kw)

    def prefill_request(self, input_ids: torch.Tensor, pixel_values: torch.Tensor, attention_mask: torch.Tensor,
                        max_new_tokens: int, feats: Optional[torch.Tensor] = None):
        B, L = input_ids.shape
        if feats is None:
            feats = self.vision(pixel_values)
        cache = self.new_cache(B, L + max_new_tokens + 1)
        resid = self._buf("p_resid", (B * L, self.w.hidden), torch.float32)
        self.embed_merge(input_ids.to(self.device), feats, resid)
        am = attention_mask.to(self.device)
        pos = am.cumsum(-1).masked_fill(am == 0, 1)
        rows = (torch.arange(B, device=self.device, dtype=torch.int32) * L + (L - 1)).contiguous()
        logits, _ = self.gemma_prefill(resid, pos, cache, B, L, logits_rows=rows)
        nxt = am.sum(-1).to(torch.int32) + 1
        return cache, feats, logits, nxt

    def generate(self, input_ids, pixel_values, attention_mask, max_new_tokens: int, do_sample=False,
                 temperature=0.8, top_p=0.9, uniforms=None, stop_token: Optional[int] = 1, use_graph=True,
                 check_every: Optional[int] = None, pad_token: int = 0, return_list: bool = False):
        B = input_ids.shape[0]
        if check_every is None:
            check_every = 1 if B == 1 else 8
        cache, feats, logits, nxt = self.prefill_request(input_ids, pixel_values, attention_mask, max_new_tokens)
        sampler = dict(do_sample=do_sample, temperature=temperature, top_p=top_p)
        st = self.decode_state(B, cache, nxt, max_new_tokens, sampler=sampler)
        if do_sample:
            if uniforms is None:
                uniforms = torch.rand(max_new_tokens + 1, B)
            sampler["uniforms"] = uniforms.to(device=self.device, dtype=torch.float32).contiguous()
        self.sample(logits, st, sampler, advance=False, feats=feats)
        n = 1
        step_fn = None
        if use_graph and self.comm.capturable:
            try:
                step_fn = self._graph_step(st, cache, feats, sampler)
            except CaptureUnsupported:
                torch.cuda.synchronize()
                step_fn = None
        if step_fn is None:
            step_fn = lambda: self.decode_step(st, cache, feats, sampler)
        while n < max_new_tokens:
            if stop_token is not None and n % check_every == 0:
                if B == 1:
                    if int(st["ids"][0]) == stop_token:
                        break
                elif bool((st["hist"][:n] == stop_token).any(0).all()):
                    break
            step_fn()
            n += 1
        hist = st["hist"][:n].t().contiguous().cpu()
        self.check_numerics()
        if hasattr(self.comm, "check"):
            self.comm.check()
        if stop_token is None:
            return [r.tolist() for r in hist] if return_list else hist
        rows = []
        for r in hist.tolist():
            rows.append(r[: r.index(stop_token) + 1] if stop_token in r else r)
        if return_list:
            return rows
        if B == 1:
            return torch.tensor(rows, dtype=torch.int64)
        out = torch.full((B, max(len(r) for r in rows)), pad_token, dtype=torch.int64)
        for b, r in enumerate(rows):
            out[b, : len(r)] = torch.tensor(r, dtype=torch.int64)
        return out

    def _graph_step(self, st, cache, feats, sampler):
        torch.cuda.synchronize()
        snap = {k: st[k].clone() for k in ("ids", "pos", "kv_len", "step")}
        hist0 = st["hist"].clone()
        res0 = self._ws["d_res_a"][: st["ids"].numel() * self.w.hidden].clone() if st.get("chain") else None
        s = torch.cuda.Stream()
        s.wait_stream(torch.cuda.current_stream())
        try:
            with torch.cuda.stream(s):
                self.decode_step(st, cache, feats, sampler)
            torch.cuda.current_stream().wait_stream(s)
        finally:
            torch.cuda.synchronize()
            for k, v in snap.items():
                st[k].copy_(v)
            st["hist"].copy_(hist0)
            if res0 is not None:
                self._ws["d_res_a"][: res0.numel()].copy_(res0)
        g = torch.cuda.CUDAGraph()
        with torch.cuda.graph(g):
            self.decode_step(st, cache, feats, sampler)
        torch.cuda.synchronize()
        self.graphs["decode"] = g
        return g.replay
```

paligemma-multimodal-system_amd/pghip/ops.py:

```python
from __future__ import annotations

import math
import os
from typing import Optional

import torch

from . import _lib

EPI_BF16, EPI_BF16_GELU, EPI_BF16_GELU_MUL, EPI_F32, EPI_F32_POS, EPI_BF16_VT, EPI_QKV_ROPE, EPI_F32_FIN, \
    EPI_F32_ADD, EPI_FX_ADD, EPI_F32_RES = range(11)
FX_SCALE = 2.0 ** 32
PRO_NONE, PRO_RMSNORM, PRO_ATTN_COMBINE, PRO_RMSNORM_FIN, PRO_X_RSTD = range(5)
NORM_LAYER, NORM_RMS = 0, 1
W_FRAG = 0x100
TILE_M1 = 0x400
TILE_N64 = 0x800


def _p(t: Optional[torch.Tensor]):
    return None if t is None else t.data_ptr()


def _s() -> int:
# ... 49 lines not shown
        _lib.call("pg_gemm", _p(A), A.stride(0), _p(W), W.stride(0), _p(bias), _p(part), N, M, N, K,
                  (flags & ~0xFF) | EPI_F32, s, None, 0, None, 0, 0, _s())
        _lib.call("pg_gemm_finalize", _p(part), s, _p(out), ldc, M, N, epi, _p(aux_out), aux_ld, aux_n, None, _s())
        return out
    _lib.call("pg_gemm", _p(A), A.stride(0), _p(W), W.stride(0), _p(bias), _p(out), ldc, M, N, K, flags, ksplit,
              _p(aux), aux_rows, _p(aux_out), aux_ld, aux_n, _s())
    return out


EPI_FP8 = 0x200


def quant_fp8(x: torch.Tensor, q: Optional[torch.Tensor] = None, scale: Optional[torch.Tensor] = None,
              M: Optional[int] = None):
    _chk(x, torch.bfloat16, "x")
    M = x.shape[0] if M is None else M
    K = x.shape[1]
    if q is None:
        q = torch.empty(M, K, dtype=torch.uint8, device=x.device)
    if scale is None:
        scale = torch.empty(M, dtype=torch.float32, device=x.device)
    if q.dtype != torch.uint8 or q.stride(1) != 1 or x.stride(1) != 1 or q.shape[1] < K or scale.numel() < M:
        raise ValueError("pghip.quant_fp8: bad output buffers")
    _lib.call("pg_quant_fp8", _p(x), x.stride(0), M, K, _p(q), q.stride(0), _p(scale), _s())
    return q, scale


def gemm8(A8: torch.Tensor, a_scale: Optional[torch.Tensor], W8: torch.Tensor, w_scale: torch.Tensor,
          out: torch.Tensor, *, epi: int = EPI_BF16, M: Optional[int] = None, bias: Optional[torch.Tensor] = None,
          ksplit: int = 1, fa=None, frag: bool = False, mx_in: Optional[torch.Tensor] = None,
          mx_out: Optional[torch.Tensor] = None, ss_in: Optional[torch.Tensor] = None,
          eps: float = 1e-6) -> torch.Tensor:
    for t, n in ((A8, "A8"), (W8, "W8")):
        if t.dtype != torch.uint8 or not t.is_cuda or t.stride(1) != 1:
            raise ValueError(f"pghip.gemm8: {n} must be a row-major uint8 (e4m3) HIP tensor")
    if mx_in is None:
        _chk(a_scale, torch.float32, "a_scale")
    _chk(w_scale, torch.float32, "w_scale")
    M = A8.shape[0] if M is None else M
    N, K = W8.shape
    fa = fused_args() if fa is None else fa
    fa.a_scale = a_scale.data_ptr() if a_scale is not None else None
    fa.w_scale = w_scale.data_ptr()
    for t, n, numel in ((mx_in, "mx_in", M * K // 32), (mx_out, "mx_out", M * N // 64)):
        if t is None:
            continue
        if (t.dtype != torch.uint8 or not t.is_cuda or not t.is_contiguous() or t.numel() < numel
                or (not frag and M <= 32)):
            raise ValueError(f"pghip.gemm8: {n} must be a contiguous uint8 HIP tensor of >= {numel} E8M0 scales "
                             "(the fp8 GEMV, or the tile GEMM at M > 32)")
        setattr(fa, n, t.data_ptr())
    if ss_in is not None:
        _chk(ss_in, torch.float32, "ss_in")
        if mx_in is None or ss_in.stride(-1) != 1 or K % 1024 or not 0 < K // 1024 <= 4 or ss_in.shape[-1] < K // 1024:
            raise ValueError("pghip.gemm8: ss_in needs mx_in and fp32 [M][K/1024] sums of squares (K <= 4096)")
        fa.ss_in, fa.ss_ld, fa.ss_n, fa.eps = ss_in.data_ptr(), ss_in.stride(-2), K // 1024, float(eps)
    e = epi & 0xFF
    ldc = out.stride(-2) if out.dim() >= 2 else out.shape[-1]
    if frag:
        if M > 32:
            raise ValueError("pghip.gemm8: the fp8 GEMV takes at most 32 rows")
        _lib.call("pg_gemm_fused", _p(A8), A8.stride(0), _p(W8), W8.stride(0), _p(bias), _p(out), ldc, M, N, K,
                  e | EPI_FP8 | W_FRAG, ksplit, _lib.C.byref(fa), _s())
        return out
    s = finalize_split(M, N, K // 2) if ksplit == 1 and e in _FIN_EPIS and mx_out is None else 1
    if s > 1:
        part = torch.empty(s, M, N, dtype=torch.float32, device=out.device)
        _lib.call("pg_gemm_fused", _p(A8), A8.stride(0), _p(W8), W8.stride(0), _p(bias), _p(part), N, M, N, K,
                  EPI_F32 | EPI_FP8, s, _lib.C.byref(fa), _s())
        _lib.call("pg_gemm_finalize", _p(part), s, _p(out), ldc, M, N, e, None, 0, 0, _lib.C.byref(fa), _s())
        return out
    _lib.call("pg_gemm_fused", _p(A8), A8.stride(0), _p(W8), W8.stride(0), _p(bias), _p(out), ldc, M, N, K,
              e | EPI_FP8, ksplit, _lib.C.byref(fa), _s())
    return out


def gemm8_hx(H: torch.Tensor, amax: torch.Tensor, amax_ld: int, W8: torch.Tensor, w_scale: torch.Tensor,
             out: torch.Tensor, *, M: int, ksplit: int, bias: Optional[torch.Tensor] = None) -> torch.Tensor:
    _chk(H, torch.bfloat16, "H")
    _chk(w_scale, torch.float32, "w_scale")
    if W8.dtype != torch.uint8 or not W8.is_cuda or amax.dtype != torch.int32 or not amax.is_cuda:
        raise ValueError("pghip.gemm8_hx: W8 uint8 (fragment-packed e4m3) and amax int32 HIP tensors")
    N, K = W8.shape
    if M > 32 or (K // 128) % ksplit or (K // 128 // ksplit) not in (8, 16) or amax.numel() < M * amax_ld:
        raise ValueError("pghip.gemm8_hx: M <= 32, K / 128 / ksplit in (8, 16), amax [M * amax_ld]")
    fa = fused_args(pro_mode=5, amax_in=amax, amax_ld=amax_ld, w_scale=w_scale)
    ldc = out.stride(-2) if out.dim() >= 2 else out.shape[-1]
    _lib.call("pg_gemm_fused", _p(H), H.stride(0), _p(W8), W8.stride(0), _p(bias), _p(out), ldc, M, N, K,
              EPI_F32 | EPI_FP8 | W_FRAG, ksplit, _lib.C.byref(fa), _s())
    return out


def fused_args(**kw) -> "_lib.PgFusedArgs":
    fa = _lib.PgFusedArgs()
    for k, v in kw.items():
        setattr(fa, k, v.data_ptr() if isinstance(v, torch.Tensor) else v)
    return fa


def gemm_fused(A: Optional[torch.Tensor], W: torch.Tensor, out: torch.Tensor, fa, *, epi: int = EPI_BF16,
               M: int, bias: Optional[torch.Tensor] = None, ksplit: int = 1, N: Optional[int] = None,
               ldc: Optional[int] = None, keep=None) -> torch.Tensor:
    _chk(W, torch.bfloat16, "W")
    _chk_frag(W, epi)
    if (epi & 0xFF) == EPI_FX_ADD:
        _chk(out, torch.int64, "out (the fixed-point accumulator)")
    N = W.shape[0] if N is None else N
    K = W.shape[1]
    if ldc is None:
        ldc = out.stride(-2) if out.dim() >= 2 else out.shape[-1]
    lda = A.stride(0) if A is not None else K
    s = finalize_split(M, N, K) if (fa.pro_mode == 0 and A is not None and ksplit == 1 and
                                    (epi & 0xFF) in _FIN_EPIS) else 1
    if s > 1:
        part = torch.empty(s, M, N, dtype=torch.float32, device=out.device)
        _lib.call("pg_gemm", _p(A), lda, _p(W), W.stride(0), _p(bias), _p(part), N, M, N, K,
                  (epi & ~0xFF) | EPI_F32, s, None, 0, None, 0, 0, _s())
        _lib.call("pg_gemm_finalize", _p(part), s, _p(out), ldc, M, N, epi & 0xFF, None, 0, 0,
                  _lib.C.byref(fa), _s())
        return out
    _lib.call("pg_gemm_fused", _p(A), lda, _p(W), W.stride(0), _p(bias), _p(out), ldc, M, N, K, epi, ksplit,
              _lib.C.byref(fa), _s())
    return out


def norm_residual(resid: torch.Tensor, w: torch.Tensor, *, b: Optional[torch.Tensor] = None,
                  mode: int = NORM_RMS, eps: float = 1e-6, partials: Optional[torch.Tensor] = None,
                  nsplit: int = 0, out: Optional[torch.Tensor] = None, out_f32: Optional[torch.Tensor] = None,
                  row_map: Optional[torch.Tensor] = None, write_resid: bool = True):
    _chk(resid, torch.float32, "resid")
    M, H = resid.shape[-2], resid.shape[-1]
    M_out = row_map.numel() if row_map is not None else M
    ldo = out.stride(-2) if out is not None else H
    _lib.call("pg_norm_residual", _p(resid), _p(partials), nsplit, M, _p(w), _p(b), _p(out), ldo, _p(out_f32),
              _p(row_map), M_out, H, mode, float(eps), int(write_resid), _s())


def norm_residual_fp8(resid: torch.Tensor, w: torch.Tensor, q: torch.Tensor, scale: torch.Tensor, *,
                      b: Optional[torch.Tensor] = None, mode: int = NORM_RMS, eps: float = 1e-6,
                      partials: Optional[torch.Tensor] = None, nsplit: int = 0, write_resid: bool = True):
    _chk(resid, torch.float32, "resid")
    M, H = resid.shape[-2], resid.shape[-1]
    if q.dtype != torch.uint8 or q.stride(-1) != 1 or q.shape[-1] < H or scale.numel() < M:
        raise ValueError("pghip.norm_residual_fp8: bad output buffers")
    _lib.call("pg_norm_residual_fp8", _p(resid), _p(partials), nsplit, M, _p(w), _p(b), _p(q), q.stride(-2),
              _p(scale), None, M, H, mode, float(eps), int(write_resid), _s())
    return q, scale


def norm_residual_mx(resid: torch.Tensor, w: torch.Tensor, q: torch.Tensor, qs: torch.Tensor, ss: torch.Tensor, *,
                     partials: Optional[torch.Tensor] = None, nsplit: int = 0, write_resid: bool = True):
    _chk(resid, torch.float32, "resid")
    _chk(w, torch.float32, "w")
    M, H = resid.shape[-2], resid.shape[-1]
    if (q.dtype != torch.uint8 or q.stride(-1) != 1 or q.shape[-1] < H or q.shape[0] < M or qs.dtype != torch.uint8
            or not qs.is_contiguous() or qs.numel() < M * H // 32 or ss.dtype != torch.float32
            or ss.stride(-1) != 1 or ss.shape[-1] < H // 1024 or ss.shape[0] < M or H % 1024):
        raise ValueError("pghip.norm_residual_mx: bad output buffers (q uint8 [M][H], qs uint8 [M*H/32], "
                         "ss fp32 [M][H/1024], H % 1024 == 0)")
    if nsplit and (partials is None or partials.dtype != torch.float32):
        raise ValueError("pghip.norm_residual_mx: fp32 partials needed for nsplit > 0")
    _lib.call("pg_norm_residual_mx", _p(resid), _p(partials), nsplit, M, _p(w), _p(q), q.stride(-2), _p(qs), _p(ss),
              ss.stride(-2), M, H, int(write_resid), _s())
    return q, qs, ss


def attention(q, q_rs, o, o_rs, k, k_bs, k_hs, k_rs, vt, vt_bs, vt_hs, vt_ds, *, B, Lq, Lkv, Hq, Hkv, D,
              scale, mask=None, mask_bs=0, mask_rs=0, lkv_dev=None, split_keys=0, nsplit=0, part_o=None,
              part_ml=None, kcap=0, kd=None, vd=None):
    _lib.call("pg_attention", _p(q), q_rs, _p(o), o_rs, _p(k), k_bs, k_hs, k_rs, _p(vt), vt_bs, vt_hs, vt_ds,
              _p(mask), mask_bs, mask_rs, B, Lq, Lkv, _p(lkv_dev), Hq, Hkv, D, float(scale), split_keys, nsplit,
              _p(part_o), _p(part_ml), int(kcap), _p(kd), _p(vd), _s())


def decode_cache_pack(k: torch.Tensor, vt: torch.Tensor, Hkv: int):
    B, S, KV = k.shape
    D = KV // Hkv
    nb = S // 32
    kd = (k.reshape(B, nb, 4, 2, 4, Hkv, D // 8, 8).permute(0, 5, 1, 3, 6, 2, 4, 7)
          .reshape(B, Hkv, S, D).contiguous())
    vd = (vt.reshape(B, Hkv, D // 16, 16, nb, 4, 8).permute(0, 1, 4, 2, 5, 3, 6)
          .reshape(B, Hkv, S, D).contiguous())
    return kd, vd


PF_KEYSPLIT = os.environ.get("PG_PF_KEYSPLIT", "1") != "0"


def prefill_key_splits(B: int, Lq: int, Lkv: int, Hq: int, Hkv: int) -> int:
    wgs = math.ceil(Lq * (Hq // Hkv) / 64) * Hkv * B
    if not PF_KEYSPLIT or wgs >= 128:
        return 1
    return max(1, min(8, 256 // wgs, math.ceil(Lkv / 64)))


def prefill_split_workspace(B: int, Lq: int, Hq: int, Hkv: int, D: int, nks: int):
    rows = B * Hkv * nks * Lq * (Hq // Hkv)
    return rows * ((D + 15) // 16 * 16), rows * 2


def attn_combine(part_o, part_ml, o, o_rs, *, B, Hq, Hkv, D, nsplit):
    _lib.call("pg_attn_combine", _p(part_o), _p(part_ml), B, Hq, Hkv, D, nsplit, _p(o), o_rs, _s())


ATTN_WEIGHTS = os.environ.get("PG_ATTN_WEIGHTS", "0") == "1"


def attn_probs(q, q_rs, k, k_bs, k_hs, k_rs, *, B, Lq, Lkv, Hq, Hkv, D, scale, mask=None, mask_bs=0, mask_rs=0,
               probs=True, out=None) -> torch.Tensor:
    if out is None:
        out = torch.empty(B, Hq, Lq, Lkv, dtype=torch.float32, device=q.device)
    if mask is not None:
        _chk(mask, torch.float32, "mask")
    _lib.call("pg_attn_probs", _p(q), q_rs, _p(k), k_bs, k_hs, k_rs, _p(mask), mask_bs, mask_rs, B, Lq, Lkv, Hq, Hkv,
              D, float(scale), int(bool(probs)), _p(out), _s())
    return out


DECODE_MAX_SPLITS = int(os.environ.get("PG_DECODE_MAX_SPLITS", "8"))


def decode_plan(B: int, Hkv: int, kcap: int):
    nblk = kcap // 32
    nw = 4 if nblk >= 4 else 2
    nsplit = max(1, min(DECODE_MAX_SPLITS, nblk // nw))
    nb = -(-nblk // (nw * nsplit))
    return nsplit, nw, nb


ATTN_PIPE = os.environ.get("PG_ATTN_PIPE", "1") != "0"
_ATTN_PIPE_FLAG = 0x100


def attn_decode(q, q_rs, o, o_rs, kd, vd, *, B, Lkv, lkv_dev, Hq, Hkv, D, scale, kcap, part_o, part_ml, counters,
                plan=None, q8=None, q8_scale=None):
    nsplit, nw, nb = plan or decode_plan(B, Hkv, kcap)
    if q8 is not None:
        _chk(q8, torch.uint8, "q8")
        _chk(q8_scale, torch.float32, "q8_scale")
        if not attn_decode_q8_ok(Hq, Hkv, D, nw) or q8.shape[0] < B or q8_scale.numel() < B:
            raise ValueError("pghip.attn_decode: fp8 row copy needs one kv head, Hq*D/8 <= 64*nw and B rows")
    if part_o.numel() < B * Hkv * nsplit * 16 * D or part_ml.numel() < B * Hkv * nsplit * 16 * 2:
        raise ValueError("pghip.attn_decode: partial workspace too small")
    if counters.dtype != torch.int32 or counters.numel() < B * Hkv:
        raise ValueError("pghip.attn_decode: counters must be int32 [B*Hkv]")
    _lib.call("pg_attn_decode", _p(q), q_rs, _p(o), o_rs, _p(kd), _p(vd), B, Lkv, _p(lkv_dev), Hq, Hkv, D,
              float(scale), kcap, nsplit, nw | (_ATTN_PIPE_FLAG if ATTN_PIPE else 0), nb, _p(part_o), _p(part_ml), _p(counters), _p(q8), _p(q8_scale),
              q8.stride(0) if q8 is not None else 0, _s())


def attn_decode_q8_ok(Hq: int, Hkv: int, D: int, nw: int) -> bool:
    return Hkv == 1 and Hq * (D // 8) <= 64 * nw


def rope_kv_write(qkv, pos, cos_t, sin_t, kc, vtc, *, T, L, Hq, Hkv, D, Smax, slot_base=0, slot_dev=None):
    _chk(qkv, torch.bfloat16, "qkv")
    _chk(pos, torch.int32, "pos")
    _lib.call("pg_rope_kv_write", _p(qkv), qkv.stride(0), _p(pos), T, L, Hq, Hkv, D, _p(cos_t), _p(sin_t), _p(kc),
              _p(vtc), Smax, slot_base, _p(slot_dev), _s())


def patch_im2col(px: torch.Tensor, patch: int, out: torch.Tensor):
    _chk(px, torch.float32, "pixel_values")
    px = px.contiguous()
    B, C, H, W = px.shape
    _lib.call("pg_patch_im2col", _p(px), B, C, H, W, patch, _p(out), out.stride(0), _s())


def image_rank(ids: torch.Tensor, image_id: int, rank: torch.Tensor):
    _chk(ids, torch.int64, "input_ids")
    _lib.call("pg_image_rank", _p(ids), ids.numel(), int(image_id), _p(rank), _s())


def embed_merge(ids, rank, embed, feat, n_feat, out, *, image_id, pad_id, img_scale, normalizer):
    _chk(ids, torch.int64, "input_ids")
    V, H = embed.shape
    _lib.call("pg_embed_merge", _p(ids), _p(rank), ids.numel(), _p(embed), V, _p(feat), n_feat, H, int(image_id),
              int(pad_id), float(img_scale), float(normalizer), _p(out), _s())


def _rows(t: Optional[torch.Tensor], B: int) -> int:
    return 0 if t is None else t.numel() // B


def argmax(logits, out_ids, workspace, *, hist=None, step=None, pos=None, kv_len=None):
    _chk(logits, torch.float32, "logits")
    B, V = logits.shape
    _lib.call("pg_argmax", _p(logits), logits.stride(0), B, V, _p(workspace), _p(out_ids), _p(hist), _rows(hist, B),
              _p(step), _p(pos), _p(kv_len), _s())


def argmax_embed(logits, out_ids, workspace, embed, feat, n_feat, res, *, image_id, pad_id, img_scale, normalizer,
                 hist=None, step=None, pos=None, kv_len=None):
    _chk(logits, torch.float32, "logits")
    _chk(res, torch.float32, "res")
    B, V = logits.shape
    Ve, H = embed.shape
    assert res.is_contiguous() and res.numel() >= B * H
    _lib.call("pg_argmax_embed", _p(logits), logits.stride(0), B, V, _p(workspace), _p(out_ids), _p(hist),
              _rows(hist, B), _p(step), _p(pos), _p(kv_len), _p(embed), Ve, _p(feat), int(n_feat), H, int(image_id),
              int(pad_id), float(img_scale), float(normalizer), _p(res), _s())


def argmax_pairs(logits, workspace, pairs, *, vocab_offset: int):
    _chk(logits, torch.float32, "logits")
    B, V = logits.shape
    _lib.call("pg_argmax_pairs", _p(logits), logits.stride(0), B, V, int(vocab_offset), _p(workspace), _p(pairs), _s())


def argmax_merge(pairs, out_ids, *, world: int, hist=None, step=None, pos=None, kv_len=None):
    B = out_ids.numel()
    _lib.call("pg_argmax_merge", _p(pairs), int(world), B, _p(out_ids), _p(hist), _rows(hist, B), _p(step), _p(pos),
              _p(kv_len), _s())


def topp_sample(logits, out_ids, uniforms, *, temperature, top_p, hist=None, step=None, pos=None, kv_len=None,
                probs_out=None):
    _chk(logits, torch.float32, "logits")
    B, V = logits.shape
    rows = _rows(uniforms, B) if hist is None else min(_rows(uniforms, B), _rows(hist, B))
    _lib.call("pg_topp_sample", _p(logits), logits.stride(0), B, V, float(temperature), float(top_p), _p(uniforms),
              _p(out_ids), _p(hist), rows, _p(step), _p(pos), _p(kv_len), _p(probs_out), _s())


def image_preprocess(src, H, W, S, hb, hk, hks, vb, vk, vks, y0, rows, lut, tmp, out):
    _chk(src, torch.uint8, "image")
    _chk(out, torch.float32, "pixel_values")
    _lib.call("pg_image_preprocess", _p(src), H, W, S, _p(hb), _p(hk), hks, _p(vb), _p(vk), vks, y0, rows, _p(lut),
              _p(tmp), _p(out), _s())


def image_preprocess_modes(src, H, W, C, alpha, S, hb, hk, hks, vb, vk, vks, y0, rows, lut, tmp, out):
    _chk(src, torch.uint8, "image")
    _chk(out, torch.float32, "pixel_values")
    _lib.call("pg_image_preprocess_modes", _p(src), H, W, C, int(bool(alpha)), S, _p(hb), _p(hk), hks, _p(vb), _p(vk),
              vks, y0, rows, _p(lut), _p(tmp), _p(out), _s())


def image_palette(src, H, W, S, xtab, ytab, pal_lut, out):
    _chk(src, torch.uint8, "image")
    _chk(out, torch.float32, "pixel_values")
    _lib.call("pg_image_palette", _p(src), H, W, S, _p(xtab), _p(ytab), _p(pal_lut), _p(out), _s())


def synth_fill(out: torch.Tensor, seedmix: int, a: float, mean: float):
    kind = 0 if out.dtype == torch.bfloat16 else 1
    if kind == 1:
        _chk(out, torch.float32, "out")
    _lib.call("pg_synth_fill", _p(out), out.numel(), seedmix & 0xFFFFFFFF, float(a), float(mean), kind, _s())


_FIN_EPIS = (EPI_BF16, EPI_BF16_GELU, EPI_BF16_GELU_MUL, EPI_BF16_VT, EPI_QKV_ROPE)
FINALIZE_SPLIT = True


def finalize_split(M: int, N: int, K: int) -> int:
    if not FINALIZE_SPLIT or M <= 16 or K % 64:
        return 1
    if math.ceil(M / 256) * math.ceil(N / 256) >= CUS:
        return 1
    tiles = math.ceil(M / 64) * math.ceil(N / 128)
    if tiles > 100:
        return 1
    s = min(2, math.ceil(CUS / tiles), (K // 64) // 6)
    return s if s >= 2 else 1


def slab_sum(part: torch.Tensor, out: torch.Tensor) -> torch.Tensor:
    _chk(part, torch.float32, "part")
    _chk(out, torch.float32, "out")
    S, M, N = part.shape
    if not part.is_contiguous() or out.shape != (M, N) or out.stride(1) != 1:
        raise ValueError("pghip.slab_sum: part must be contiguous [S][M][N] and out [M][N] with unit column stride")
    _lib.call("pg_gemm_finalize", _p(part), S, _p(out), out.stride(0), M, N, EPI_F32, None, 0, 0, None, _s())
    return out


def split_for(tiles: int, k_steps: int, target: int = 256, max_split: int = 4) -> int:
    s = max(1, min(max_split, target // max(tiles, 1), k_steps // 2))
    return s


CUS = 256


def gemm_ksplit(M: int, N: int, K: int) -> int:
    t256 = math.ceil(M / 256) * math.ceil(N / 256)
    if t256 >= CUS:
        kt = K // 64
        best, best_s = -1.0, 1
        for s in (1, 2, 3, 4):
            if s > 1 and kt // s < 8:
                break
            u = t256 * s
            eff = u / (math.ceil(u / CUS) * CUS) - 800.0 / K * (s - 1)
            if eff > best + 1e-9:
                best, best_s = eff, s
        return best_s
    s256 = math.ceil(CUS / t256)
    if s256 <= min(16, (K // 64) // 8):
        return s256
    return split_for(math.ceil(M / 64) * math.ceil(N / 128), K // 64, max_split=6)
```

Measured before the change: 942.8 tokens/s.

## Fuse per-workgroup argmax partials into LM-head GEMV epilogue for greedy decode

The LM-head GEMV epilogue now also computes a per-workgroup (value, index) argmax over its logit tiles using cross-lane permlane swaps, and writes these partials to small buffers. A new single-workgroup final kernel, optionally with the next-token embedding, reduces only those partials instead of rescanning the full vocab-sized logits. The aim is to remove the separate argmax pass over the logits array in each greedy decode step. Logits are still written in full, so the kernel now does a bit more epilogue work, and the Python side tracks tensor versions to confirm the partials still match the logits.

```diff
diff --git a/include/pghip.h b/include/pghip.h
--- a/include/pghip.h
+++ b/include/pghip.h
@@ -124,6 +124,18 @@
                     const float* feat, int n_feat, int H, long image_id, long pad_id, float img_scale,
                     float normalizer, float* res, hipStream_t stream);
 
+int pg_gemm_fused_argmax(const void* A, int lda, const void* W, int ldw, const float* bias, void* C, int ldc, int M,
+                         int N, int K, int epi, const PgFusedArgs* fused, int am_n, float* am_val, int* am_idx,
+                         int am_ld, hipStream_t stream);
+int pg_gemv_argmax_parts(int M, int N, int* n_part);
+int pg_argmax_parts(const float* am_val, const int* am_idx, int am_ld, int n_part, int B, void* workspace,
+                    int64_t* out_ids, int64_t* hist, int hist_rows, int* step, int* pos, int* kv_len,
+                    hipStream_t stream);
+int pg_argmax_parts_embed(const float* am_val, const int* am_idx, int am_ld, int n_part, int B, void* workspace,
+                          int64_t* out_ids, int64_t* hist, int hist_rows, int* step, int* pos, int* kv_len,
+                          const void* embed, int V_embed, const float* feat, int n_feat, int H, long image_id,
+                          long pad_id, float img_scale, float normalizer, float* res, hipStream_t stream);
+
 int pg_argmax_pairs(const float* logits, long ld, int B, int V, int vocab_offset, void* workspace,
                     float* pairs, hipStream_t stream);
 int pg_argmax_merge(const float* pairs, int world, int B, int64_t* out_ids, int64_t* hist, int hist_rows,
diff --git a/paligemma-multimodal-system_amd/csrc/common.h b/paligemma-multimodal-system_amd/csrc/common.h
--- a/paligemma-multimodal-system_amd/csrc/common.h
+++ b/paligemma-multimodal-system_amd/csrc/common.h
@@ -46,6 +46,23 @@
 __device__ __forceinline__ float sum_xor32(float v) {
   const auto r = __builtin_amdgcn_permlane32_swap(__float_as_uint(v), __float_as_uint(v), false, false);
   return __uint_as_float(r[0]) + __uint_as_float(r[1]);
+}
+
+__device__ __forceinline__ void am_better(float& bv, int& bi, float v, int i) {
+  if (v > bv || (v == bv && i < bi)) { bv = v; bi = i; }
+}
+
+__device__ __forceinline__ void am_xor16(float& bv, int& bi) {
+  const auto rv = __builtin_amdgcn_permlane16_swap(__float_as_uint(bv), __float_as_uint(bv), false, false);
+  const auto ri = __builtin_amdgcn_permlane16_swap((uint32_t)bi, (uint32_t)bi, false, false);
+  am_better(bv, bi, __uint_as_float(rv[0]), (int)ri[0]);
+  am_better(bv, bi, __uint_as_float(rv[1]), (int)ri[1]);
+}
+__device__ __forceinline__ void am_xor32(float& bv, int& bi) {
+  const auto rv = __builtin_amdgcn_permlane32_swap(__float_as_uint(bv), __float_as_uint(bv), false, false);
+  const auto ri = __builtin_amdgcn_permlane32_swap((uint32_t)bi, (uint32_t)bi, false, false);
+  am_better(bv, bi, __uint_as_float(rv[0]), (int)ri[0]);
+  am_better(bv, bi, __uint_as_float(rv[1]), (int)ri[1]);
 }
 
 __device__ __forceinline__ float xchg_xor32(float v) {
diff --git a/paligemma-multimodal-system_amd/csrc/gemm.hip b/paligemma-multimodal-system_amd/csrc/gemm.hip
--- a/paligemma-multimodal-system_amd/csrc/gemm.hip
+++ b/paligemma-multimodal-system_amd/csrc/gemm.hip
@@ -2,7 +2,8 @@
 
 static int gemm_impl(const void* A, int lda, const void* W, int ldw, const float* bias, void* C, int ldc,
                      int M, int N, int K, int epi_flags, int ksplit, const float* aux, int aux_rows, void* aux_out,
-                     int aux_ld, int aux_n, const PgFusedArgs* fa, hipStream_t stream) {
+                     int aux_ld, int aux_n, const PgFusedArgs* fa, hipStream_t stream, float* am_val = nullptr,
+                     int* am_idx = nullptr, int am_ld = 0, int am_n = 0) {
   const bool frag = (epi_flags & PG_W_FRAG) != 0;
   const bool fp8 = (epi_flags & PG_FP8) != 0;
   const bool m1 = (epi_flags & PG_TILE_M1) != 0;
@@ -20,6 +21,13 @@
   PgFusedArgs f{};
   if (fa) f = *fa;
   EpiArgs e{bias, C, ldc, M, N, aux, aux_rows, (bf16_t*)aux_out, aux_ld, aux_n, f};
+  if (am_val || am_idx)
+    PG_REQUIRE(am_val && am_idx && epi == PG_EPI_F32 && !fp8 && M <= 16 && ksplit == 1 && am_n > 0 && am_n <= N &&
+               am_ld >= pg_gemv_f32_wgs(M, N));
+  e.am_val = am_val;
+  e.am_idx = am_idx;
+  e.am_ld = am_ld;
+  e.am_n = am_n;
   PG_REQUIRE(f.pro_mode >= 0 && f.pro_mode <= 5);
   if (f.pro_mode == 5)
     PG_REQUIRE(fp8 && frag && epi == PG_EPI_F32 && M <= 32 && f.amax_in && f.amax_ld >= 1 && A != nullptr &&
@@ -111,3 +119,17 @@
                              int M, int N, int K, int epi, int ksplit, const PgFusedArgs* fused, hipStream_t stream) {
   return gemm_impl(A, lda, W, ldw, bias, C, ldc, M, N, K, epi, ksplit, nullptr, 0, nullptr, 0, 0, fused, stream);
 }
+
+extern "C" int pg_gemm_fused_argmax(const void* A, int lda, const void* W, int ldw, const float* bias, void* C, int ldc,
+                                    int M, int N, int K, int epi, const PgFusedArgs* fused, int am_n, float* am_val,
+                                    int* am_idx, int am_ld, hipStream_t stream) {
+  PG_REQUIRE(am_val != nullptr && am_idx != nullptr);
+  return gemm_impl(A, lda, W, ldw, bias, C, ldc, M, N, K, epi, 1, nullptr, 0, nullptr, 0, 0, fused, stream, am_val,
+                   am_idx, am_ld, am_n);
+}
+
+extern "C" int pg_gemv_argmax_parts(int M, int N, int* n_part) {
+  PG_REQUIRE(M > 0 && M <= 16 && N > 0 && n_part != nullptr);
+  *n_part = pg_gemv_f32_wgs(M, N);
+  return 0;
+}
diff --git a/paligemma-multimodal-system_amd/csrc/gemm_common.h b/paligemma-multimodal-system_amd/csrc/gemm_common.h
--- a/paligemma-multimodal-system_amd/csrc/gemm_common.h
+++ b/paligemma-multimodal-system_amd/csrc/gemm_common.h
@@ -129,6 +129,9 @@
   int aux_ld;
   int aux_n;
   PgFusedArgs f;
+  float* am_val;
+  int* am_idx;
+  int am_ld, am_n;
 };
 
 __device__ __forceinline__ void scale_acc(const EpiArgs& e, int m, int n0, f32x4& v) {
@@ -264,19 +267,23 @@
   }
 }
 
+__device__ __forceinline__ void epi_put4_f32(const EpiArgs& e, int m, int n0, f32x4 v, int z) {
+  const size_t srows = e.f.slab_rows > 0 ? (size_t)e.f.slab_rows : (size_t)e.M;
+  float* C = (float*)e.C + ((size_t)z * srows + m) * e.ldc;
+  if (n0 + 3 < e.N) {
+    *(f32x4*)(C + n0) = v;
+  } else {
+#pragma unroll
+    for (int j = 0; j < 4; ++j) if (n0 + j < e.N) C[n0 + j] = v[j];
+  }
+}
+
 template <int EPI>
 __device__ __forceinline__ void epi_store4(const EpiArgs& e, int m, int n0, f32x4 v, int z) {
   if (m >= e.M || n0 >= e.N) return;
   if (e.bias && (EPI != PG_EPI_F32 || z == 0)) v += load4_guard(e.bias, n0, e.N);
   if constexpr (EPI == PG_EPI_F32) {
-    const size_t srows = e.f.slab_rows > 0 ? (size_t)e.f.slab_rows : (size_t)e.M;
-    float* C = (float*)e.C + ((size_t)z * srows + m) * e.ldc;
-    if (n0 + 3 < e.N) {
-      *(f32x4*)(C + n0) = v;
-    } else {
-#pragma unroll
-      for (int j = 0; j < 4; ++j) if (n0 + j < e.N) C[n0 + j] = v[j];
-    }
+    epi_put4_f32(e, m, n0, v, z);
   } else if constexpr (EPI == PG_EPI_F32_RES) {
     float* C = (float*)e.C + (size_t)m * e.ldc;
     if (n0 + 3 < e.N) {
@@ -359,5 +366,6 @@
                      const EpiArgs& e, hipStream_t st, bool m1, bool n64);
 int pg_dispatch_gemv(int epi, bool frag, const bf16_t* A, int lda, const bf16_t* W, int ldw, int K, int ksplit,
                      const EpiArgs& e, hipStream_t st);
+int pg_gemv_f32_wgs(int M, int N);
 int pg_dispatch_gemv8(int epi, const uint8_t* X, int ldx, const uint8_t* W, int K, int ksplit, const EpiArgs& e,
                       hipStream_t st);
diff --git a/paligemma-multimodal-system_amd/csrc/gemm_gemv.hip b/paligemma-multimodal-system_amd/csrc/gemm_gemv.hip
--- a/paligemma-multimodal-system_amd/csrc/gemm_gemv.hip
+++ b/paligemma-multimodal-system_amd/csrc/gemm_gemv.hip
@@ -662,6 +662,31 @@
       epi_qkv_rope4_core(e, m, n0, v, pr, rope_cs[t], rope_sn[t], e.f.slot_base + rope_slot_raw);
     }
   } else {
+    if constexpr (EPI == PG_EPI_F32) {
+      if (e.am_val) {
+        float bv = -INFINITY;
+        int bi = 0x7FFFFFFF;
+#pragma unroll
+        for (int t = 0; t < NT; ++t) {
+          const int n0 = (tile0 + t) * 16 + q;
+          if (m < M && n0 < e.N) {
+            f32x4 v = acc[t];
+            if (e.bias) v += load4_guard(e.bias, n0, e.N);
+            epi_put4_f32(e, m, n0, v, 0);
+#pragma unroll
+            for (int j = 0; j < 4; ++j)
+              if (n0 + j < e.am_n) am_better(bv, bi, v[j], n0 + j);
+          }
+        }
+        am_xor16(bv, bi);
+        am_xor32(bv, bi);
+        if (g == 0 && m < M) {
+          e.am_val[(size_t)m * e.am_ld + gi.bx] = bv;
+          e.am_idx[(size_t)m * e.am_ld + gi.bx] = bi;
+        }
+        return;
+      }
+    }
 #pragma unroll
     for (int t = 0; t < NT; ++t) epi_store4<EPI>(e, m, (tile0 + t) * 16 + q, acc[t], z);
   }
@@ -685,6 +710,14 @@
     case 16: hipLaunchKernelGGL((gemv_kernel<EPI, NT, 2, DEPTH, PRO, FRAG, 16>), grid, dim3(256), lds, st, A, lda, W, ldw, K, e); break;
     default: hipLaunchKernelGGL((gemv_kernel<EPI, NT, 2, DEPTH, PRO, FRAG, 0>), grid, dim3(256), lds, st, A, lda, W, ldw, K, e); break;
   }
+}
+
+static inline bool gemv_lm_two_tiles(int M, int ntiles, int ksplit) {
+  return PG_GEMV_LM_NT == 2 && M <= 4 && ntiles >= 8192 && ksplit == 1;
+}
+int pg_gemv_f32_wgs(int M, int N) {
+  const int ntiles = (N + 15) / 16;
+  return (M > 4 || gemv_lm_two_tiles(M, ntiles, 1)) ? (ntiles + 1) / 2 : ntiles;
 }
 
 template <int EPI, int PRO, bool FRAG>
@@ -707,7 +740,7 @@
     }
   }
   if constexpr (PG_GEMV_LM_NT == 2 && EPI == PG_EPI_F32) {
-    if (e.M <= 4 && ntiles >= 8192 && ksplit == 1) {
+    if (gemv_lm_two_tiles(e.M, ntiles, ksplit)) {
       launch_gemv_cpw<EPI, 2, PG_GEMV_LM_D, PRO, FRAG>(dim3((ntiles + 1) / 2, 1), lds, st, A, lda, W, ldw, K, 1, e);
       return;
     }
diff --git a/paligemma-multimodal-system_amd/csrc/misc.hip b/paligemma-multimodal-system_amd/csrc/misc.hip
--- a/paligemma-multimodal-system_amd/csrc/misc.hip
+++ b/paligemma-multimodal-system_amd/csrc/misc.hip
@@ -169,9 +169,6 @@
 }
 
 #define AM_CHUNKS 64
-__device__ __forceinline__ void am_better(float& bv, int& bi, float v, int i) {
-  if (v > bv || (v == bv && i < bi)) { bv = v; bi = i; }
-}
 __device__ __forceinline__ void am_block(float& bv, int& bi, float* sv, int* si) {
   const int lane = threadIdx.x & 63, w = threadIdx.x >> 6;
 #pragma unroll
@@ -371,6 +368,162 @@
   return 0;
 }
 
+typedef __attribute__((ext_vector_type(4))) int i32x4;
+template <int UN>
+__global__ __launch_bounds__(1024) void argmax_parts_final_kernel(const float* __restrict__ pv, const int* __restrict__ pi,
+                                                                  int ld, int n_part, int B, int tshift,
+                                                                  int64_t* __restrict__ out_ids,
+                                                                  int64_t* __restrict__ hist, int hist_rows,
+                                                                  int* __restrict__ step, int* __restrict__ pos,
+                                                                  int* __restrict__ kv_len, AmEmbArgs ea) {
+  __shared__ float sv[16];
+  __shared__ int si[16];
+  __shared__ int win[16];
+  const int T = 1 << tshift;
+  const int b = threadIdx.x >> tshift, tr = threadIdx.x & (T - 1);
+  const int lane = threadIdx.x & 63, wave = threadIdx.x >> 6;
+  const int st = step ? *step : 0;
+  float bv = -INFINITY;
+  int bi = 0x7FFFFFFF;
+  if (b < B) {
+    const float* rv = pv + (long)b * ld;
+    const int* ri = pi + (long)b * ld;
+    const int last = (n_part - 1) & ~3;
+    for (int i0 = tr * 4; i0 < n_part; i0 += T * 4 * UN) {
+      f32x4 v[UN];
+      i32x4 ix[UN];
+#pragma unroll
+      for (int u = 0; u < UN; ++u) {
+        const int i = min(i0 + u * T * 4, last);
+        v[u] = *(const f32x4*)(rv + i);
+        ix[u] = *(const i32x4*)(ri + i);
+      }
+      __builtin_amdgcn_sched_barrier(0);
+#pragma unroll
+      for (int u = 0; u < UN; ++u) {
+        const int i = i0 + u * T * 4;
+#pragma unroll
+        for (int j = 0; j < 4; ++j)
+          if (i + j < n_part) am_better(bv, bi, v[u][j], ix[u][j]);
+      }
+    }
+  }
+#pragma unroll
+  for (int o = 32; o > 0; o >>= 1) {
+    float ov = __shfl_xor(bv, o, 64);
+    int oi = __shfl_xor(bi, o, 64);
+    am_better(bv, bi, ov, oi);
+  }
+  if (lane == 0) { sv[wave] = bv; si[wave] = bi; }
+  __syncthreads();
+  if (threadIdx.x < B) {
+    const int wpr = T >> 6, row = threadIdx.x;
+    bv = sv[row * wpr];
+    bi = si[row * wpr];
+    for (int i = 1; i < wpr; ++i) am_better(bv, bi, sv[row * wpr + i], si[row * wpr + i]);
+    win[row] = bi;
+    out_ids[row] = bi;
+    if (hist && st < hist_rows) hist[(long)st * B + row] = bi;
+    if (pos) pos[row] += 1;
+  }
+  if (threadIdx.x == 0) {
+    if (kv_len) *kv_len += 1;
+    if (step) *step = st + 1;
+  }
+  if (ea.res == nullptr) return;
+  __syncthreads();
+  if (b < B) {
+    const int64_t id = win[b];
+    int rk = 0;
+    if (id == ea.image_id)
+      for (int i = 0; i < b; ++i) rk += win[i] == ea.image_id;
+    embed_row(ea.res + (long)b * ea.H, id, rk, tr, T, ea.embed, ea.V, ea.feat, ea.n_feat, ea.H, ea.image_id, ea.pad_id,
+              ea.img_scale, ea.normalizer);
+  }
+}
+
+__global__ __launch_bounds__(64) void argmax_parts_chunk_kernel(const float* __restrict__ am_val,
+                                                                const int* __restrict__ am_idx, int ld, int n_part,
+                                                                float* __restrict__ pv, int* __restrict__ pi) {
+  const int b = blockIdx.y, ch = blockIdx.x, lane = threadIdx.x;
+  const int per = ((n_part + AM_CHUNKS - 1) / AM_CHUNKS + 3) & ~3;
+  const int s = ch * per, e = min(n_part, s + per);
+  const float* rv = am_val + (long)b * ld;
+  const int* ri = am_idx + (long)b * ld;
+  float bv = -INFINITY;
+  int bi = 0x7FFFFFFF;
+  for (int i = s + lane * 4; i < e; i += 256) {
+    const f32x4 v = *(const f32x4*)(rv + i);
+    const i32x4 ix = *(const i32x4*)(ri + i);
+#pragma unroll
+    for (int j = 0; j < 4; ++j)
+      if (i + j < e) am_better(bv, bi, v[j], ix[j]);
+  }
+#pragma unroll
+  for (int o = 32; o > 0; o >>= 1) {
+    float ov = __shfl_xor(bv, o, 64);
+    int oi = __shfl_xor(bi, o, 64);
+    am_better(bv, bi, ov, oi);
+  }
+  if (lane == 0) { pv[b * AM_CHUNKS + ch] = bv; pi[b * AM_CHUNKS + ch] = bi; }
+}
+
+#define AMP_ONE_WG_MAX_B 4
+static int argmax_parts_launch(const float* am_val, const int* am_idx, int am_ld, int n_part, int B, void* workspace,
+                               int64_t* out_ids, int64_t* hist, int hist_rows, int* step, int* pos, int* kv_len,
+                               const AmEmbArgs& ea, hipStream_t stream) {
+  PG_REQUIRE(am_val && am_idx && out_ids && B > 0 && B <= 16 && n_part > 0 && n_part <= (1 << 24) &&
+             am_ld >= n_part && am_ld % 4 == 0 && ((uintptr_t)am_val & 15) == 0 && ((uintptr_t)am_idx & 15) == 0 &&
+             (hist == nullptr || hist_rows > 0) && (B <= AMP_ONE_WG_MAX_B || workspace != nullptr));
+  if (B > AMP_ONE_WG_MAX_B) {
+    float* pv = (float*)workspace;
+    int* pi = (int*)(pv + B * AM_CHUNKS);
+    hipLaunchKernelGGL(argmax_parts_chunk_kernel, dim3(AM_CHUNKS, B), dim3(64), 0, stream, am_val, am_idx, am_ld,
+                       n_part, pv, pi);
+    if (ea.res)
+      hipLaunchKernelGGL(argmax_final_embed_kernel, dim3(1), dim3(64 * am_waves(B)), 0, stream, pv, pi, B, out_ids,
+                         hist, hist_rows, step, pos, kv_len, ea);
+    else
+      hipLaunchKernelGGL(argmax_final_kernel, dim3(1), dim3(64 * am_waves(B)), 0, stream, pv, pi, B, out_ids, hist,
+                         hist_rows, step, pos, kv_len);
+    PG_LAUNCH_CHECK();
+    return 0;
+  }
+  int tshift = 10;
+  while ((1024 >> tshift) < B) --tshift;
+  const int groups = (n_part + 3) / 4, T = 1 << tshift;
+  const int un = (groups + T - 1) / T;
+#define PG_AMP(U)                                                                                                  \
+  hipLaunchKernelGGL(argmax_parts_final_kernel<U>, dim3(1), dim3(1024), 0, stream, am_val, am_idx, am_ld, n_part, \
+                     B, tshift, out_ids, hist, hist_rows, step, pos, kv_len, ea)
+  if (un <= 1) PG_AMP(1);
+  else if (un <= 2) PG_AMP(2);
+  else if (un <= 4) PG_AMP(4);
+  else PG_AMP(8);
+#undef PG_AMP
+  PG_LAUNCH_CHECK();
+  return 0;
+}
+
+extern "C" int pg_argmax_parts(const float* am_val, const int* am_idx, int am_ld, int n_part, int B, void* workspace,
+                               int64_t* out_ids, int64_t* hist, int hist_rows, int* step, int* pos, int* kv_len,
+                               hipStream_t stream) {
+  return argmax_parts_launch(am_val, am_idx, am_ld, n_part, B, workspace, out_ids, hist, hist_rows, step, pos, kv_len,
+                             AmEmbArgs{}, stream);
+}
+
+extern "C" int pg_argmax_parts_embed(const float* am_val, const int* am_idx, int am_ld, int n_part, int B,
+                                     void* workspace, int64_t* out_ids, int64_t* hist, int hist_rows, int* step,
+                                     int* pos, int* kv_len, const void* embed, int V_embed, const float* feat, int n_feat, int H,
+                                     long image_id, long pad_id, float img_scale, float normalizer, float* res,
+                                     hipStream_t stream) {
+  PG_REQUIRE(embed != nullptr && res != nullptr && V_embed > 0 && H > 0 && H % 4 == 0 && (n_feat == 0 || feat));
+  const AmEmbArgs ea{(const bf16_t*)embed, V_embed, n_feat, H, feat, (int64_t)image_id, (int64_t)pad_id,
+                     img_scale, normalizer, res};
+  return argmax_parts_launch(am_val, am_idx, am_ld, n_part, B, workspace, out_ids, hist, hist_rows, step, pos, kv_len,
+                             ea, stream);
+}
+
 __global__ __launch_bounds__(1024) void topp_kernel(const float* __restrict__ logits, long ld, int V, float inv_temp,
                                                     float top_p, const float* __restrict__ uniforms,
                                                     int64_t* __restrict__ out_ids, int64_t* __restrict__ hist, int hist_rows,
diff --git a/paligemma-multimodal-system_amd/pghip/_lib.py b/paligemma-multimodal-system_amd/pghip/_lib.py
--- a/paligemma-multimodal-system_amd/pghip/_lib.py
+++ b/paligemma-multimodal-system_amd/pghip/_lib.py
@@ -44,6 +44,12 @@
     "pg_argmax": [vp, i64, i32, i32, vp, vp, vp, i32, vp, vp, vp, vp],
     "pg_argmax_embed": [vp, i64, i32, i32, vp, vp, vp, i32, vp, vp, vp, vp, i32, vp, i32, i32, i64, i64, f32, f32, vp,
                         vp],
+    "pg_gemm_fused_argmax": [vp, i32, vp, i32, vp, vp, i32, i32, i32, i32, i32, C.POINTER(PgFusedArgs), i32, vp, vp,
+                             i32, vp],
+    "pg_gemv_argmax_parts": [i32, i32, C.POINTER(C.c_int)],
+    "pg_argmax_parts": [vp, vp, i32, i32, i32, vp, vp, vp, i32, vp, vp, vp, vp],
+    "pg_argmax_parts_embed": [vp, vp, i32, i32, i32, vp, vp, vp, i32, vp, vp, vp, vp, i32, vp, i32, i32, i64, i64,
+                              f32, f32, vp, vp],
     "pg_argmax_pairs": [vp, i64, i32, i32, i32, vp, vp, vp],
     "pg_argmax_merge": [vp, i32, i32, vp, vp, i32, vp, vp, vp, vp],
     "pg_topp_sample": [vp, i64, i32, i32, f32, f32, vp, vp, vp, i32, vp, vp, vp, vp, vp],
diff --git a/paligemma-multimodal-system_amd/pghip/engine.py b/paligemma-multimodal-system_amd/pghip/engine.py
--- a/paligemma-multimodal-system_amd/pghip/engine.py
+++ b/paligemma-multimodal-system_amd/pghip/engine.py
@@ -105,6 +105,7 @@
         self._rope = None
         self._rope_n = 0
         self._ws = {}
+        self._lm_am = None
         self.graphs = {}
 
     def _validate_splits(self):
@@ -443,7 +444,30 @@
             x8, xs = self._x8(rows, xf.shape[1])
             ops.quant_fp8(xf, x8, xs, M=rows)
             return ops.gemm8(x8, xs, w.lm_w8f, w.lm_s8, out, epi=ops.EPI_F32, M=rows, bias=w.lm_bias, frag=True)
+        if self.tp == 1 and rows <= self.LM_ARGMAX_MAX_ROWS and xf.shape[0] == rows:
+            return self._lm_gemv_argmax(xf, rows, out)
         return ops.gemm(xf, w.lm_w, out, epi=ops.EPI_F32 | w.wflag, bias=w.lm_bias)
+
+    LM_ARGMAX_MAX_ROWS = 4
+
+    def _lm_gemv_argmax(self, xf: Optional[torch.Tensor], rows: int, out: torch.Tensor, fa=None):
+        w = self.w
+        ld = _rup(ops.argmax_parts(rows, w.lm_w.shape[0]), 4)
+        val = self._buf("lm_am_val", (rows, ld), torch.float32)
+        idx = self._buf("lm_am_idx", (rows, ld), torch.int32)
+        self._lm_am = None
+        n_part = ops.gemm_argmax(xf, w.lm_w, out, val, idx, am_n=w.vocab, fa=fa, epi=ops.EPI_F32 | w.wflag, M=rows,
+                                 bias=w.lm_bias)
+        self._lm_am = SimpleNamespace(out=out, version=out._version, rows=rows, val=val, idx=idx, n_part=n_part)
+        return out
+
+    def _lm_parts_of(self, logits: torch.Tensor):
+        am = getattr(self, "_lm_am", None)
+        if (am is None or logits.dim() != 2 or logits.data_ptr() != am.out.data_ptr()
+                or tuple(logits.shape) != (am.rows, self.w.vocab) or logits.stride() != (am.out.stride(0), 1)
+                or logits._version != am.version or am.out._version != am.version):
+            return None
+        return am
 
     def _chain_ok(self, sampler) -> bool:
         return self.CHAIN_EMBED and self.tp == 1 and sampler is not None and not sampler.get("do_sample")
@@ -509,7 +533,10 @@
             xq, ss, tiles, n_ss = self._decode_layers_fin(st, cache, ws)
             logits = self._buf("d_logits", (B, w.vocab_local_pad), torch.float32)
             fa = ops.fused_args(pro_mode=ops.PRO_X_RSTD, ss_in=ss, ss_ld=tiles, ss_n=n_ss, eps=1e-6)
-            ops.gemm_fused(xq, w.lm_w, logits, fa, epi=ops.EPI_F32 | w.wflag, M=B, bias=w.lm_bias)
+            if B <= self.LM_ARGMAX_MAX_ROWS:
+                self._lm_gemv_argmax(xq, B, logits, fa)
+            else:
+                ops.gemm_fused(xq, w.lm_w, logits, fa, epi=ops.EPI_F32 | w.wflag, M=B, bias=w.lm_bias)
             logits = logits[:, :w.vocab]
         else:
             layers = self._decode_layers_fused if ws.route == "fused" else self._decode_layers_unfused
@@ -751,14 +778,24 @@
         kw = dict(hist=st["hist"], step=st["step"])
         if advance:
             kw.update(pos=st["pos"], kv_len=st["kv_len"])
+        am = None if sampler.get("do_sample") else self._lm_parts_of(logits)
+        if am is not None and am.rows != st["ids"].numel():
+            am = None
         if st.get("chain") and self._chain_ok(sampler):
             w = self.w
             B = st["ids"].numel()
-            ops.argmax_embed(logits, st["ids"], st["ws"], w.embed, feats, feats.shape[0] if feats is not None else 0,
-                             self._buf("d_res_a", (B, w.hidden), torch.float32), **self._embed_kw(), **kw)
+            emb = (w.embed, feats, feats.shape[0] if feats is not None else 0,
+                   self._buf("d_res_a", (B, w.hidden), torch.float32))
+            if am is not None:
+                ops.argmax_embed_from_parts(am.val, am.idx, am.n_part, st["ids"], st["ws"], *emb, **self._embed_kw(),
+                                            **kw)
+            else:
+                ops.argmax_embed(logits, st["ids"], st["ws"], *emb, **self._embed_kw(), **kw)
         elif sampler.get("do_sample"):
             ops.topp_sample(logits, st["ids"], sampler["uniforms"], temperature=sampler["temperature"],
                             top_p=sampler["top_p"], **kw)
+        elif am is not None:
+            ops.argmax_from_parts(am.val, am.idx, am.n_part, st["ids"], st["ws"], **kw)
         else:
             ops.argmax(logits, st["ids"], st["ws"], **kw)
 
diff --git a/paligemma-multimodal-system_amd/pghip/ops.py b/paligemma-multimodal-system_amd/pghip/ops.py
--- a/paligemma-multimodal-system_amd/pghip/ops.py
+++ b/paligemma-multimodal-system_amd/pghip/ops.py
@@ -375,6 +375,80 @@
               int(pad_id), float(img_scale), float(normalizer), _p(res), _s())
 
 
+def argmax_parts(M: int, N: int) -> int:
+    n = _lib.C.c_int(0)
+    _lib.call("pg_gemv_argmax_parts", int(M), int(N), _lib.C.byref(n))
+    return n.value
+
+
+def argmax_workspace(M: int, N: int, device):
+    ld = (argmax_parts(M, N) + 3) // 4 * 4
+    return (torch.empty(M, ld, dtype=torch.float32, device=device),
+            torch.empty(M, ld, dtype=torch.int32, device=device))
+
+
+def gemm_argmax(A: Optional[torch.Tensor], W: torch.Tensor, out: torch.Tensor, am_val: torch.Tensor,
+                am_idx: torch.Tensor, *, am_n: int, fa=None, epi: int = EPI_F32, M: int,
+                bias: Optional[torch.Tensor] = None, N: Optional[int] = None) -> int:
+    _chk(W, torch.bfloat16, "W")
+    _chk_frag(W, epi)
+    _chk(out, torch.float32, "out")
+    _chk(am_val, torch.float32, "am_val")
+    _chk(am_idx, torch.int32, "am_idx")
+    if bias is not None:
+        _chk(bias, torch.float32, "bias")
+    N = W.shape[0] if N is None else N
+    K = W.shape[1]
+    if (epi & 0xFF) != EPI_F32 or not 0 < M <= 16 or not 0 < am_n <= N:
+        raise ValueError("pghip.gemm_argmax: EPI_F32 on 1..16 rows, 0 < am_n <= N")
+    if A is not None:
+        _chk(A, torch.bfloat16, "A")
+        if A.stride(1) != 1 or A.shape[1] < K or A.shape[0] < M:
+            raise ValueError(f"pghip.gemm_argmax: A must hold [{M}][{K}] contiguous rows")
+    ldc = out.stride(-2) if out.dim() >= 2 else out.shape[-1]
+    if out.stride(-1) != 1 or out.storage_offset() + (M - 1) * ldc + N > \
+            out.untyped_storage().nbytes() // out.element_size():
+        raise ValueError("pghip.gemm_argmax: output too small")
+    n_part = argmax_parts(M, N)
+    ld = am_val.stride(0)
+    if (am_val.dim() != 2 or am_val.shape != am_idx.shape or am_val.shape[0] < M or am_val.shape[1] < n_part
+            or am_val.stride(1) != 1 or am_idx.stride(1) != 1 or am_idx.stride(0) != ld):
+        raise ValueError(f"pghip.gemm_argmax: am_val / am_idx must be [>= {M}][>= {n_part}] with equal row strides")
+    _lib.call("pg_gemm_fused_argmax", _p(A), A.stride(0) if A is not None else K, _p(W), W.stride(0), _p(bias),
+              _p(out), ldc, M, N, K, epi, None if fa is None else _lib.C.byref(fa), int(am_n), _p(am_val), _p(am_idx),
+              ld, _s())
+    return n_part
+
+
+def _chk_parts(am_val, am_idx, n_part: int, B: int, workspace, who: str):
+    _chk(am_val, torch.float32, "am_val")
+    _chk(am_idx, torch.int32, "am_idx")
+    if am_val.shape[0] < B or am_idx.shape[0] < B or am_idx.stride(0) != am_val.stride(0) or am_val.shape[1] < n_part:
+        raise ValueError(f"pghip.{who}: partials do not cover the rows")
+    if B > 4 and (workspace is None or workspace.numel() * workspace.element_size() < B * 64 * 8):
+        raise ValueError(f"pghip.{who}: more than 4 rows need a workspace of B * 512 bytes (as argmax)")
+
+
+def argmax_from_parts(am_val, am_idx, n_part: int, out_ids, workspace=None, *, hist=None, step=None, pos=None,
+                      kv_len=None):
+    B = out_ids.numel()
+    _chk_parts(am_val, am_idx, n_part, B, workspace, "argmax_from_parts")
+    _lib.call("pg_argmax_parts", _p(am_val), _p(am_idx), am_val.stride(0), int(n_part), B, _p(workspace), _p(out_ids),
+              _p(hist), _rows(hist, B), _p(step), _p(pos), _p(kv_len), _s())
+
+
+def argmax_embed_from_parts(am_val, am_idx, n_part: int, out_ids, workspace, embed, feat, n_feat, res, *, image_id,
+                            pad_id, img_scale, normalizer, hist=None, step=None, pos=None, kv_len=None):
+    _chk(res, torch.float32, "res")
+    B = out_ids.numel()
+    Ve, H = embed.shape
+    assert res.is_contiguous() and res.numel() >= B * H
+    _chk_parts(am_val, am_idx, n_part, B, workspace, "argmax_embed_from_parts")
+    _lib.call("pg_argmax_parts_embed", _p(am_val), _p(am_idx), am_val.stride(0), int(n_part), B, _p(workspace),
+              _p(out_ids), _p(hist), _rows(hist, B), _p(step), _p(pos), _p(kv_len), _p(embed), Ve, _p(feat), int(n_feat),
+              H, int(image_id), int(pad_id), float(img_scale), float(normalizer), _p(res), _s())
+
+
 def argmax_pairs(logits, workspace, pairs, *, vocab_offset: int):
     _chk(logits, torch.float32, "logits")
     B, V = logits.shape
```

After: 941.7 tokens/s. Within noise of the previous version (-0.1%).
